# XingqunQi-lab/EmotionGestures

Hardware: AMD Instinct MI355X
Metric: gesture clips/sec (34 frames, 43 joints) (higher is better)
Workload: dtype bf16x3; 1 GPU; TED clips: 4 s 16 kHz audio -> mel(128x124) -> CVAE sample -> generator -> 34x126 pose; global_batch=64, variant=Models_spatial_memory, parallelism=clip-sharded x1, no data-path collective, launch=hipGraph replay, 4 step(s) in flight, branch_streams=False, fold_affine=False

## Files before the change

emotiongestures_amd/_lib.py:

```python
from __future__ import annotations

import ctypes as C
import os

_HERE = os.path.dirname(os.path.abspath(__file__))
LIB_PATH = os.path.join(_HERE, "libemogest_hip.so")

EG_PREC_F32, EG_PREC_BF16X3, EG_PREC_BF16 = 0, 1, 2
PRECISIONS = {"f32": EG_PREC_F32, "fp32": EG_PREC_F32, "bf16x3": EG_PREC_BF16X3, "bf16": EG_PREC_BF16}

(PACK_RAW, PACK_LINEAR, PACK_VEC_PAD, PACK_CONV3X3, PACK_BN_SCALE, PACK_BN_SHIFT, PACK_CONV1X1, PACK_STEM,
 PACK_WN_TAP, PACK_CONV1D, PACK_POS_TABLE, PACK_LINEAR_T, PACK_LINEAR_FOLD, PACK_BIAS_FOLD, PACK_CONV1X1_BF16, PACK_WN_TAPS) = range(16)


class EgError(RuntimeError):
    pass


class EgWeightEntry(C.Structure):
    _fields_ = [("key", C.c_char * 192), ("kind", C.c_int32), ("dims", C.c_int32 * 4),
                ("offset", C.c_int64), ("numel", C.c_int64)]


class EgGeneratorConfig(C.Structure):
    _fields_ = [(n, C.c_int32) for n in (
        "frames", "pose_dim", "prior_frames", "chunk", "d_model", "d_inner", "n_layers", "n_head", "d_k",
        "n_mels", "spec_len", "text_len", "n_words", "embed_dim", "tcn_hidden", "tcn_layers", "variant",
        "precision", "n_position")] + [("reserved", C.c_int32 * 5)]


class EgCvaeConfig(C.Structure):
    _fields_ = [("frames", C.c_int32), ("d_model", C.c_int32), ("latent", C.c_int32), ("n_classes", C.c_int32),
                ("reserved", C.c_int32 * 4)]


_P = C.c_void_p
_I = C.c_int32
_L = C.c_int64


class EgLinearArgs(C.Structure):
    _fields_ = [(n, _P) for n in ("x", "w", "bias", "res1", "res2", "y", "gate_src", "drop_epoch", "partial", "x_images", "y_images")] + \
               [("drop_offset", C.c_uint64)] + \
               [(n, _I) for n in ("lda", "ldw", "ldr", "ldc", "ldg", "m", "n", "k", "relu", "precision", "splits", "k_x", "y_k")] + \
               [("drop_seed", C.c_uint32), ("drop_p", C.c_float)]


class EgResamplePlan(C.Structure):
    _fields_ = [(n, C.c_int32) for n in ("L", "M", "half", "K", "D", "Hs", "pitch", "bank_floats")]


EG_RESAMPLE_TILE, EG_RESAMPLE_MAX_FACTOR = 1024, 640
EG_SKELETON_MAX_BONES, EG_SKELETON_MAX_FACTOR, EG_SKELETON_TILE_FRAMES = 63, 64, 32
EG_SKELETON_SPACE_LOCAL, EG_SKELETON_SPACE_GLOBAL = 0, 1

SIGNATURES = {
    "eg_last_error": (C.c_char_p, []),
    "eg_launch_count": (_L, []),
    "eg_launch_histogram": (_L, [C.c_char_p, _L, C.c_int32]),
    "eg_version": (C.c_char_p, []),
    "eg_set_default_precision": (C.c_int, [C.c_int]),
    "eg_get_default_precision": (C.c_int, []),
    "eg_generator_default_config": (C.c_int, [C.POINTER(EgGeneratorConfig)]),
    "eg_generator_create": (C.c_int, [C.POINTER(EgGeneratorConfig), C.POINTER(_P)]),
    "eg_generator_destroy": (None, [_P]),
    "eg_generator_arena_floats": (_L, [_P]),
    "eg_generator_num_weights": (_I, [_P]),
    "eg_generator_weight_entry": (C.c_int, [_P, _I, C.POINTER(EgWeightEntry)]),
    "eg_generator_workspace_bytes": (_L, [_P, _I]),
    "eg_generator_forward": (C.c_int, [_P, _P, _I, _P, _P, _P, _P, _P, _P, _P, _P, _P, _P, _L, _P]),
    "eg_generator_forward_draws": (C.c_int, [_P, _P, _I, _I, _P, _P, _P, _P, _P, _L, _P]),
    "eg_generator_draws_workspace_bytes": (_L, [_P, _I, _I]),
    "eg_generator_forward_rollout": (C.c_int, [_P, _P, _I, _I, _P, _P, _P, _P, _P, _P, _P, _P, _P, _P, _P, _P, _L, _P]),
    "eg_generator_rollout_workspace_bytes": (_L, [_P, _I, _I]),
    "eg_generator_forward_rollout_draws": (C.c_int, [_P, _P, _I, _I, _I, _P, _P, _P, _P, _P, _P, _P, _P, _P, _P, _P, _P, _L, _P]),
    "eg_generator_rollout_draws_workspace_bytes": (_L, [_P, _I, _I, _I]),
    "eg_rows_by_table": (C.c_int, [_P, _P, _P, _I, _L, _I, _P]),
    "eg_rollout_ragged_plan_ints": (_L, [_I, _L]),
    "eg_rollout_ragged_plan": (C.c_int, [_P, _I, _P, _P, _P, _P]),
    "eg_generator_forward_rollout_ragged": (C.c_int, [_P, _P, _I, _P, _P, _P, _P, _P, _P, _P, _P, _P, _P, _P, _P, _P, _P, _L, _P]),
    "eg_generator_rollout_ragged_workspace_bytes": (_L, [_P, _I, _L]),
    "eg_stream_state_bytes": (_L, [_P, _I, _I, _I]),
    "eg_stream_reset": (C.c_int, [_P, _P, _I, _I, _I, _P, _P, _P]),
    "eg_stream_push": (C.c_int, [_P, _P, _I, _I, _I, _P, _P, _P, _P]),
    "eg_generator_stream_step": (C.c_int, [_P, _P, _P, _I, _I, _I, _P, _P, _P, _P, _P, _P, _P, _P, _P, _L, _P]),
    "eg_stream_tail": (C.c_int, [_P, _P, _I, _I, _I, _P, _P]),
    "eg_generator_tap": (C.c_int, [_P, _I, _P, C.c_char_p, C.POINTER(_P), C.POINTER(_L)]),
    "eg_cvae_default_config": (C.c_int, [C.POINTER(EgCvaeConfig)]),
    "eg_cvae_create": (C.c_int, [C.POINTER(EgCvaeConfig), C.POINTER(_P)]),
    "eg_cvae_destroy": (None, [_P]),
    "eg_cvae_arena_floats": (_L, [_P]),
    "eg_cvae_num_weights": (_I, [_P]),
    "eg_cvae_weight_entry": (C.c_int, [_P, _I, C.POINTER(EgWeightEntry)]),
    "eg_cvae_workspace_bytes": (_L, [_P, _I]),
    "eg_cvae_sample": (C.c_int, [_P, _P, _I, _P, _P, _P, _P, _L, _P]),
    "eg_cvae_forward": (C.c_int, [_P, _P, _I, _P, _P, _P, _P, _P, _P, _P, _L, _P]),
    "eg_mel_tables": (C.c_int, [_P, _P, _P, _P]),
    "eg_mel_workspace_bytes": (_L, [_I, _I]),
    "eg_melspectrogram": (C.c_int, [_P, _I, _I, _P, _P, _P, _P, _P, _I, _P, _L, _P]),
    "eg_window_gather": (C.c_int, [_P, _I, _L, _I, _L, _I, _P, _P]),
    "eg_window_gather_ragged": (C.c_int, [_P, _I, _L, _P, _P, _L, _I, _P, _P]),
    "eg_resample_plan": (C.c_int, [_I, _I, C.POINTER(EgResamplePlan)]),
    "eg_resample_out_length": (_L, [_L, _I, _I]),
    "eg_resample_filter": (C.c_int, [_I, _I, _P, _P]),
    "eg_resample": (C.c_int, [_P, _I, _L, _P, _P, _I, _I, _P, _L, _P, _L, _P]),
    "eg_resample_stream_state_bytes": (_L, [_I, _I, _I]),
    "eg_resample_stream_reset": (C.c_int, [_P, _I, _I, _I, _P, _P]),
    "eg_resample_stream_push": (C.c_int, [_P, _I, _I, _I, _P, _P, _I, _P, _P, _I, _P]),
    "eg_skeleton_check": (C.c_int, [_P, _P, _P, _I]),
    "eg_skeleton_out_frames": (_L, [_L, _I, _I]),
    "eg_skeleton_tile_frames": (_I, []),
    "eg_skeleton_joints": (C.c_int, [_P, _I, _I, _P, _P, _P, _I, _P, _P, _I, _I, _P, _I, _I, _I, _P, _L, _P]),
    "eg_skeleton_dir_vec": (C.c_int, [_P, _I, _I, _P, _P, _P, _I, _P, _P, _I, _I, _P, _P, _P]),
    "eg_skeleton_rest_check": (C.c_int, [_P, _I]),
    "eg_skeleton_levels": (C.c_int, [_P, _P, _P, _I, _P, _P]),
    "eg_skeleton_rotations": (C.c_int, [_P, _I, _I, _P, _P, _P, _I, _P, _P, _P, _I, _I, _P, _I, _I, _I, _P, _L, _P]),
    "eg_beat_tables": (C.c_int, [_P, _P, _P, _P]),
    "eg_beat_workspace_bytes": (_L, [_I, _I]),
    "eg_beat_align": (C.c_int, [_P, _I, _I, _P, _I, _I, _I, _I, _I, C.c_double, _I, _P, _P, _P, _P, _P, _L, _P, _P, _P, _P, _P, _P, _P]),
    "eg_beat_tracks_meta_ints": (_L, [_I]),
    "eg_beat_tracks_meta": (C.c_int, [_P, _P, _P, _I, _I, _P]),
    "eg_beat_tracks_workspace_bytes": (_L, [_P, _P, _I, _I, _I]),
    "eg_beat_align_tracks": (C.c_int, [_P, _I, _L, _P, _P, _P, _I, _I, _I, _P, _I, _I, _P, C.c_double, _I, _P, _P, _P, _P, _P, _L, _P, _P, _P,
                                       _P, _P, _P, _P]),
    "eg_beat_tracks_scan": (C.c_int, [_P, _P, _I, _P, _P, _L, _P, _P, _P]),
    "eg_take_meta_ints": (_L, [_I]),
    "eg_take_meta": (C.c_int, [_P, _I, _P]),
    "eg_track_rows_pack": (C.c_int, [_P, _I, _I, _I, _I, _P, _P, _P, _P]),
    "eg_take_distance_workspace_bytes": (_L, [_P, _I, _I]),
    "eg_take_distance": (C.c_int, [_P, _I, _I, _I, _P, _P, _I, _P, _L, _P, _P, _P]),
    "eg_conv3x3": (C.c_int, [_P, _P, _P, _P, _P, _P, _P, _I, _I, _I, _I, _I, _I, _I, _I, _I, _P]),
    "eg_conv3x3_se": (C.c_int, [_P, _P, _P, _P, _P, _P, _P, _P, _P, _I, _I, _I, _I, _I, _I, _I, _I, _I, _P]),
    "eg_se_gate_pre": (C.c_int, [_P, _P, _I, _P, _P, _P, _P, _P, _P, _P, _P, _I, _I, _I, _I, _P]),
    "eg_se_block_fused": (C.c_int, [_P] * 19 + [_I] * 7 + [_P]),
    "eg_conv3x3_gap_tiles": (_I, [_I, _I, _I, _I, _I]),
    "eg_conv3x3_channel_split": (_I, [_I, _I, _I, _I, _I, _I, _I]),
    "eg_stem_conv": (C.c_int, [_P, _P, _P, _P, _P, _P, _I, _I, _I, _I, _P]),
    "eg_se_gate": (C.c_int, [_P, _I, _P, _P, _P, _P, _P, _I, _I, _I, _P]),
    "eg_se_residual_relu": (C.c_int, [_P, _P, _P, _P, _P, _P, _P, _I, _I, _I, _I, _I, _I, _I, _I, _P]),
    "eg_linear": (C.c_int, [_P, _I, _P, _I, _P, _P, _P, _I, _P, _I, _I, _I, _I, _I, _I, _I, _I, _P]),
    "eg_split_tiles": (C.c_int, [_P, _I, _I, _I, _P, _P]),
    "eg_linear_presplit": (C.c_int, [_P, _I, _P, _I, _P, _P, _P, _I, _P, _I, _I, _I, _I, _I, _I, _P]),
    "eg_linear_presplit_causal": (C.c_int, [_P, _I, _P, _P, _I, _P, _P, _I, _P, _I, _P, _I, _I, _I, _I, _I, _I, _I, _I, _P]),
    "eg_linear_splitk": (C.c_int, [_P, _I, _P, _I, _P, _P, _I, _I, _I, _I, _I, _I, _P, _I, _P]),
    "eg_layernorm": (C.c_int, [_P, _P, _P, _P, _I, _I, C.c_float, _P]),
    "eg_attention": (C.c_int, [_P, _I, _P, _I, _P, _I, _P, _I, _P, _I, _I, _I, _I, _I, _I, _P]),
    "eg_attention_masked": (C.c_int, [_P, _I, _P, _I, _P, _I, _P, _L, _I, _P, _I, _P, _I, _I, _I, _I, _I, _I, _P]),
    "eg_mha_workspace_bytes": (_L, [_I, _I, _I, _I, _I]),
    "eg_multi_head_attention": (C.c_int, [_P, _P, _P, _P, _P, _P, _P, _P, _P, _P, _I, _I, _I, _I, _I, _I, _P, _L, _P]),
    "eg_ffn_workspace_bytes": (_L, [_I, _I, _I]),
    "eg_positionwise_ffn": (C.c_int, [_P, _P, _P, _P, _P, _P, _P, _P, _I, _I, _I, _I, _P, _L, _P]),
    "eg_tcn_forward": (C.c_int, [_P, _P, _P, _I, _I, _I, _I, _I, _P, _L, _P]),
    "eg_add_rows": (C.c_int, [_P, _P, _P, _L, _I, _I, _P]),
    "eg_add_rows_split": (C.c_int, [_P, _P, _P, _P, _L, _I, _I, _P]),
    "eg_conv3x3_packed_floats": (_L, [_I, _I]),
    "eg_profile_enable": (C.c_int, [_I]),
    "eg_profile_disable": (C.c_int, []),
    "eg_profile_read": (_I, [_P, _P, _P, _I]),
    "eg_profile_read_workgroups": (_I, [_P, _I]),
    "eg_reparameterize": (C.c_int, [_P, _P, _P, _P, _L, _P]),
    "eg_conv1d": (C.c_int, [_P, _P, _P, _P, _P, _P, _I, _I, _I, _I, _I, _I, _I, _I, _P]),
    "eg_contrastive_workspace_bytes": (C.c_int64, [_I]),
    "eg_contrastive_loss": (C.c_int, [_P, _P, _I, _I, _P, _P, _P, _P, _L, _P]),
    "eg_contrastive_backward_workspace_bytes": (_L, [_I]),
    "eg_contrastive_loss_backward": (C.c_int, [_P, _P, _I, _I, _P, _P, _P, _L, _P]),
    "eg_transpose": (C.c_int, [_P, _I, _I, _I, _P, _I, _P]),
    "eg_gemm_tn_workspace_floats": (_L, [_I, _I, _L]),
    "eg_gemm_tn": (C.c_int, [_P, _I, _P, _I, _P, _I, _I, _I, _L, _P, _L, _I, _P]),
    "eg_conv3x3_wgrad": (C.c_int, [_P, _P, _P, _I, _I, _I, _I, _I, _I, _P, _L, _P]),
    "eg_im2col3x3": (C.c_int, [_P, _P, _I, _I, _I, _I, _I, _I, _P]),
    "eg_subsample": (C.c_int, [_P, _P, _I, _I, _I, _I, _I, _I, _P]),
    "eg_conv1d_cl_forward": (C.c_int, [_P, _P, _P, _P] + [_I] * 9 + [_P]),
    "eg_conv1d_cl_backward_input": (C.c_int, [_P, _P, _P, _P] + [_I] * 9 + [_P]),
    "eg_conv1d_cl_backward_weight_workspace_floats": (_L, [_I] * 7),
    "eg_conv1d_cl_backward_weight": (C.c_int, [_P, _P, _P, _P, _P] + [_I] * 9 + [_P, _L, _P]),
    "eg_pad_cols": (C.c_int, [_P, _P, _L, _I, _I, _P]),
    "eg_colreduce_workspace_floats": (_L, [_I]),
    "eg_bn_train_forward": (C.c_int, [_P, _P, _P, _P, _P, _P, _P, _P, _L, _I, C.c_float, C.c_float, _P, _P]),
    "eg_bn_train_backward": (C.c_int, [_P, _P, _P, _P, _P, _P, _P, _P, _L, _I, _I, _P, _P]),
    "eg_bn_train_forward_gap": (C.c_int, [_P, _P, _I, _I, _P, _P, _P, _P, _P, _P, _P, _P, _L, _I, C.c_float, C.c_float, _P, _P]),
    "eg_bn_train_forward_sq": (C.c_int, [_P, _P, _P, _I, _I, _P, _P, _P, _P, _P, _P, _P, _P, _L, _I, C.c_float, C.c_float, _P, _P]),
    "eg_conv3x3_sq": (C.c_int, [_P, _P, _P, _P, _P, _P] + [_I] * 8 + [_P]),
    "eg_se_gate_train_forward": (C.c_int, [_P] * 12 + [_I, _I, _I, _P]),
    "eg_se_tail_forward": (C.c_int, [_P] * 9 + [_I, _I, _I, _P]),
    "eg_se_tail_backward_reduce": (C.c_int, [_P] * 7 + [_I, _I, _I, _P, _P]),
    "eg_se_gate_train_backward": (C.c_int, [_P] * 16 + [_I, _I, _I, _P]),
    "eg_se_tail_backward_finish": (C.c_int, [_P] * 14 + [_I, _I, _I, _P]),
    "eg_se_tail_backward_apply": (C.c_int, [_P] * 13 + [_I, _I, _I, _P]),
    "eg_colsum": (C.c_int, [_P, _P, _P, _P, _L, _I, _P, _P]),
    "eg_elementwise": (C.c_int, [_P, _P, _P, _L, _I, C.c_float, _P]),
    "eg_conv3x3_wgrad_mfma_workspace_floats": (_L, [_I, _I, _I, _I, _I]),
    "eg_conv3x3_wgrad_mfma": (C.c_int, [_P, _P, _P, _I, _I, _I, _I, _I, _P, _L, _P]),
    "eg_conv3x3_wgrad_mfma_oihw": (C.c_int, [_P, _P, _P, _I, _I, _I, _I, _I, _P, _L, _P]),
    "eg_conv3x3_wgrad_gather_mfma": (C.c_int, [_P, _P, _P, _I, _I, _I, _I, _I, _I, _P, _L, _P]),
    "eg_conv3x3_dgrad_s2": (C.c_int, [_P, _P, _P, _P, _I, _I, _I, _I, _I, _I, _P]),
    "eg_conv3x3_res_masked": (C.c_int, [_P, _P, _P, _P, _P, _I, _I, _I, _I, _I, _I, _P]),
    "eg_conv3x3_wgrad_mfma_oihw_in_affine": (C.c_int, [_P, _P, _P, _P, _P, _I, _I, _I, _I, _I, _P, _L, _P]),
    "eg_conv3x3_sq_in_affine": (C.c_int, [_P, _P, _P, _P, _P, _P, _P, _P, _I, _I, _I, _I, _I, _I, _I, _I, _P]),
    "eg_bn_train_stats_sq": (C.c_int, [_P, _P, _I, _I, _P, _P, _P, _P, _P, _P, _P, _P, _L, _I, C.c_float, C.c_float, _P, _P]),
    "eg_pack_conv3x3_device": (C.c_int, [_P, _I, _I, _I, _P, _P]),
    "eg_linear_packed_floats": (_L, [_I, _I]),
    "eg_pack_linear_device": (C.c_int, [_P, _I, _I, _I, _I, _P, _P]),
    "eg_pack_table_blocks": (_I, [_I, _I, _I, _I]),
    "eg_pack_table": (C.c_int, [_P, _I, _I, _P]),
    "eg_dropout": (C.c_int, [_P, _P, _L, C.c_float, C.c_uint32, C.c_uint64, _P]),
    "eg_dropout_dev": (C.c_int, [_P, _P, _L, C.c_float, C.c_uint32, C.c_uint64, _P, _P]),
    "eg_seg_mean": (C.c_int, [_P, _P, _I, _I, _I, C.c_float, _P, _P]),
    "eg_seg_dot": (C.c_int, [_P, _P, _P, _I, _I, _I, _P, _P]),
    "eg_se_scale": (C.c_int, [_P, _P, _P, _P, _I, _I, _I, _P]),
    "eg_layernorm_backward": (C.c_int, [_P, _P, _P, _P, _P, _I, _I, C.c_float, _P]),
    "eg_attention_train": (C.c_int, [_P, _I, _P, _I, _P, _I, _P, _I, _P, _I, _I, _I, _I, _I, C.c_float, C.c_uint32, C.c_uint64, _P, _P]),
    "eg_attention_backward_train": (C.c_int, [_P, _I, _P, _I, _P, _I, _P, _P, _I, _P, _I, _P, _I, _P, _I, _I, _I, _I, _I, _I, C.c_float, C.c_uint32,
                                              C.c_uint64, _P, _P]),
    "eg_smooth_l1": (C.c_int, [_P, _P, _P, _P, _L, C.c_float, C.c_float, _P, _P]),
    "eg_cross_entropy": (C.c_int, [_P, _P, _P, C.c_float, C.c_float, _P, _P, _I, _I, _P, _P]),
    "eg_kld": (C.c_int, [_P, _P, _P, _P, _P, _I, _I, C.c_float, _P]),
    "eg_adam_step": (C.c_int, [_P, _P, _P, _P, _L, C.c_float, C.c_float, C.c_float, C.c_float, C.c_float, _I, _P]),
    "eg_adam_step_dev": (C.c_int, [_P, _P, _P, _P, _L, C.c_float, C.c_float, C.c_float, C.c_float, C.c_float, _P, _P]),
    "eg_counter_add": (C.c_int, [_P, _I, _P]),
    "eg_sp_gate_forward": (C.c_int, [_P, _P, _P, _P, _I, _I, _I, _I, _P]),
    "eg_sp_gate_backward": (C.c_int, [_P, _P, _P, _P, _P, _P, _I, _I, _I, _I, _P]),
    "eg_tm_scale_forward": (C.c_int, [_P, _P, _P, _P, _I, _I, _I, _I, _P]),
    "eg_tm_scale_backward": (C.c_int, [_P, _P, _P, _P, _P, _I, _I, _I, _I, _P]),
    "eg_linear_wgrad_mfma_workspace_floats": (_L, [_I, _I, _I]),
    "eg_linear_wgrad_mfma": (C.c_int, [_P, _I, _P, _I, _P, _I, _P, _I, _I, _I, _P, _L, _P]),
# ... 44 lines not shown
```

emotiongestures_amd/csrc/common.h:

```cpp
#pragma once
#include <hip/hip_runtime.h>
#include <stdint.h>
#include <stdio.h>
#include <stdarg.h>
#include <atomic>
#include "emogest.h"


typedef float f4 __attribute__((ext_vector_type(4)));
typedef short bf8 __attribute__((ext_vector_type(8)));

#define EG_WAVE 64

void eg_set_error(const char* fmt, ...);

#define EG_REQUIRE(cond, code, ...)                      \
    do {                                                 \
        if (!(cond)) {                                   \
            eg_set_error(__VA_ARGS__);                   \
            return (code);                               \
        }                                                \
    } while (0)

extern std::atomic<long long> g_eg_launches;
// ... 41 lines not shown
}
__device__ __forceinline__ float row16_sum(float s) {
    s += dpp_move<0xB1>(s);
    s += dpp_move<0x4E>(s);
    s += dpp_move<0x141>(s);
    s += dpp_move<0x140>(s);
    return s;
}
__device__ __forceinline__ float wave_max(float v) {
#pragma unroll
    for (int o = 32; o > 0; o >>= 1) v = fmaxf(v, __shfl_xor(v, o, 64));
    return v;
}

__device__ __forceinline__ unsigned short f32_to_bf16_rne(float x) {
    unsigned int u = __float_as_uint(x);
    u += 0x7FFFu + ((u >> 16) & 1u);
    return (unsigned short)(u >> 16);
}
__device__ __forceinline__ float bf16_to_f32(unsigned short h) { return __uint_as_float(((unsigned int)h) << 16); }

typedef __bf16 bf16x2_t __attribute__((ext_vector_type(2)));
typedef float f32x2_t __attribute__((ext_vector_type(2)));
typedef unsigned int u32x4_t __attribute__((ext_vector_type(4)));
template <bool WANT_LO>
__device__ __forceinline__ void split_octet(const f4& v0, const f4& v1, bf8& hi, bf8& lo) {
    u32x4_t h, l;
#pragma unroll
    for (int p = 0; p < 4; ++p) {
        const f32x2_t x = {p < 2 ? v0[2 * p] : v1[2 * p - 4], p < 2 ? v0[2 * p + 1] : v1[2 * p - 3]};
        const unsigned hu = __builtin_bit_cast(unsigned, __builtin_convertvector(x, bf16x2_t));
        h[p] = hu;
        if (WANT_LO) {
            const f32x2_t r = {x[0] - __uint_as_float(hu << 16), x[1] - __uint_as_float(hu & 0xffff0000u)};
            l[p] = __builtin_bit_cast(unsigned, __builtin_convertvector(r, bf16x2_t));
        }
    }
    hi = __builtin_bit_cast(bf8, h);
    if (WANT_LO) lo = __builtin_bit_cast(bf8, l);
}

__device__ __forceinline__ unsigned int mix32(unsigned int h) {
    h ^= h >> 16; h *= 0x85EBCA6Bu; h ^= h >> 13; h *= 0xC2B2AE35u; h ^= h >> 16;
    return h;
}
__device__ __forceinline__ unsigned int dropout_seed(unsigned int seed, const int* __restrict__ epoch) {
    return epoch ? seed ^ mix32((unsigned int)*epoch * 0x9E3779B9u + 0x7F4A7C15u) : seed;
}
__device__ __forceinline__ bool dropout_keep(unsigned int seed, unsigned long long ctr, unsigned int thr) {
    return mix32(mix32((unsigned int)ctr ^ seed) + (unsigned int)(ctr >> 32) * 0x9E3779B9u + 0x6A09E667u) >= thr;
}
struct EgDropout {
    unsigned int thr = 0, seed = 0;
    float inv_keep = 1.f;
    unsigned long long offset = 0;
    const int* epoch = nullptr;
};

__device__ __forceinline__ void xcd_tile(int& bx, int& by) {
    const int gx = gridDim.x, gy = gridDim.y, total = gx * gy;
    const int lin = blockIdx.y * gx + blockIdx.x;
    const int xcd = lin & 7, idx = lin >> 3;
    const int q = total >> 3, r = total & 7;
    const int log = xcd * q + (xcd < r ? xcd : r) + idx;
    bx = log / gy;
    by = log - bx * gy;
}

template <int N> __device__ __forceinline__ void wait_vmcnt_imm() {
    __builtin_amdgcn_s_waitcnt((N & 15) | 0x70 | 0xF00 | ((N >> 4) << 14));
}
__device__ __forceinline__ void wait_lgkmcnt0() { __builtin_amdgcn_s_waitcnt(0xC07F); }
__device__ __forceinline__ void wg_barrier() {
    asm volatile("" ::: "memory");
    __builtin_amdgcn_s_barrier();
    asm volatile("" ::: "memory");
}

struct EgProfScope {
    int slot;
    hipStream_t st;
    EgProfScope(int64_t tag, double flops, hipStream_t s);
    void workgroups(int n);
    ~EgProfScope();
};

struct EgiCvaeFused {
    const float *y = nullptr, *z = nullptr;
    const float *lin_w[4] = {}, *lin_b[4] = {};
    const float *t_w[2] = {}, *t_b[2] = {}, *t_s[2] = {}, *t_t[2] = {};
    const float *c_w[3] = {}, *c_b[3] = {}, *c_s[2] = {}, *c_t[2] = {};
    float* out = nullptr;
    int F = 0, L = 0, T = 0;
};

struct EgiLinear {
    const float* x = nullptr; int lda = 0;
    const void* ximg = nullptr; int xK = 0, xk0 = 0;
    const float* w = nullptr; int ldw = 0; const float* bias = nullptr;
    const float* res1 = nullptr; const float* res2 = nullptr; int ldr = 0;
    float* y = nullptr; int ldc = 0;
    void* yimg = nullptr; int yK = 0, yk0 = 0;
    int m = 0, n = 0, k = 0, relu = 0, a_shift = 0, a_seq = 1, precision = 0;
    int shared_chip = 0;
    int xs_shift = 0, xs_period = 1; const void* xzero = nullptr;
    int splits = 0; float* partial = nullptr;
};
```

emotiongestures_amd/csrc/gemm.hip:

```cpp
#include "common.h"
#include <stdlib.h>
#include <string.h>

namespace {

struct GemmArgs {
    const float* x; const float* w; const float* bias; const float* res1; const float* res2; float* y;
    const unsigned short* whi; const unsigned short* wlo;
    int lda, ldw, ldr, ldc, M, N, K, relu, a_shift, a_seq, k_per_split;
    float* partial;
    unsigned short* yimg = nullptr;
    int yKO = 0, yoct0 = 0;
    int xoct0 = 0;
    int xs_steps = 0, xs_shift = 0, xs_period = 1;
    const bf8* xzero = nullptr;
    const float* gate = nullptr; int ldg = 0;
    EgDropout drop;
};

__device__ __forceinline__ float epi_masks(const GemmArgs& a, float v, int m, int n, unsigned int dseed) {
    if (a.gate && !(a.gate[(size_t)m * a.ldg + n] > 0.f)) v = 0.f;
    if (a.drop.thr) v = dropout_keep(dseed, a.drop.offset + (unsigned long long)m * a.N + n, a.drop.thr) ? v * a.drop.inv_keep : 0.f;
    return v;
}
// ... 316 lines not shown
        const int k0 = kbeg + step * 32;
        f4* X = lds + slot * SLOT;
#pragma unroll
        for (int p = 0; p < 2; ++p) {
            const int k = min(k0 + xq[p], klast);
            __builtin_amdgcn_global_load_lds((const __attribute__((address_space(1))) void*)(xsrc[p] + k),
                                             (__attribute__((address_space(3))) void*)(X + (p * 4 + wave) * 64), 16, 0, 0);
        }
        bf8* W = reinterpret_cast<bf8*>(X + XS);
#pragma unroll
        for (int t = 0; t < TN; ++t) {
            const size_t gbase = ((size_t)min(by * TN + t, nt_last) * KO + (k0 >> 3)) * 64 + wave * 64 + lane;
            __builtin_amdgcn_global_load_lds((const __attribute__((address_space(1))) void*)(reinterpret_cast<const bf8*>(a.whi) + gbase),
                                             (__attribute__((address_space(3))) void*)(W + t * NIMG * WIMG + wave * 64), 16, 0, 0);
            if (TERMS == 3)
                __builtin_amdgcn_global_load_lds((const __attribute__((address_space(1))) void*)(reinterpret_cast<const bf8*>(a.wlo) + gbase),
                                                 (__attribute__((address_space(3))) void*)(W + t * NIMG * WIMG + WIMG + wave * 64), 16, 0, 0);
        }
    };
    auto wait_groups = [&](int groups_in_flight) {
        if (groups_in_flight >= 2) wait_vmcnt_imm<2 * G>();
        else if (groups_in_flight == 1) wait_vmcnt_imm<G>();
        else wait_vmcnt_imm<0>();
    };

    f4 acc[2][WN];
#pragma unroll
    for (int t = 0; t < 2; ++t)
#pragma unroll
        for (int n = 0; n < WN; ++n) acc[t][n] = (f4){0.f, 0.f, 0.f, 0.f};

    const int pre = min(nsteps, RING - 1);
    for (int s = 0; s < pre; ++s) issue(s, s);
    wait_groups(pre - 1);
    wg_barrier();
    const int fsw = (li ^ (li >> 1)) & 7;
#pragma unroll 1
    for (int s = 0; s < nsteps; ++s) {
        if (s + RING - 1 < nsteps) issue(s + RING - 1, (s + RING - 1) % RING);
        const f4* X = lds + (s % RING) * SLOT;
        const bf8* W = reinterpret_cast<const bf8*>(X + XS);
        bf8 xh[2], xl[2], wh[WN], wl[WN];
#pragma unroll
        for (int t = 0; t < 2; ++t) {
            const f4* xr = X + (wm + t * 16 + li) * 8;
            const f4 q0 = xr[(2 * kq) ^ fsw], q1 = xr[(2 * kq + 1) ^ fsw];
            split_octet<TERMS == 3>(q0, q1, xh[t], xl[t]);
        }
#pragma unroll
        for (int n = 0; n < WN; ++n) {
            const int col = wn + n * 16, tile = col >> 6, r = (col & 63) + li;
            wh[n] = W[tile * NIMG * WIMG + kq * 64 + r];
            if (TERMS == 3) wl[n] = W[tile * NIMG * WIMG + WIMG + kq * 64 + r];
        }
#pragma unroll
        for (int t = 0; t < 2; ++t)
#pragma unroll
            for (int n = 0; n < WN; ++n) {
                if (TERMS == 3) {
                    acc[t][n] = __builtin_amdgcn_mfma_f32_16x16x32_bf16(wl[n], xh[t], acc[t][n], 0, 0, 0);
                    acc[t][n] = __builtin_amdgcn_mfma_f32_16x16x32_bf16(wh[n], xl[t], acc[t][n], 0, 0, 0);
                }
                acc[t][n] = __builtin_amdgcn_mfma_f32_16x16x32_bf16(wh[n], xh[t], acc[t][n], 0, 0, 0);
            }
        const int newest = min(s + RING - 1, nsteps - 1);
        wait_groups(max(0, newest - (s + 1)));
        __builtin_amdgcn_s_waitcnt(0xC07F);
        wg_barrier();
    }
    gemm_epilogue<2, WN, true>(a, acc, m0 + wm + li, n0 + wn + kq * 4);
}

template <int TERMS, int WN>
int launch_glds(const GemmArgs& a, int splits, hipStream_t st) {
    constexpr int NIMG = (TERMS == 3) ? 2 : 1, TN = WN / 2, RING = (WN == 2) ? 4 : 3;
    constexpr size_t LDS_BYTES = (size_t)RING * (64 * 8 + TN * NIMG * 4 * 64) * 16;
    auto kern = gemm_glds_kernel<TERMS, WN>;
    if (int rc = eg_ensure_dynamic_lds(reinterpret_cast<const void*>(kern), LDS_BYTES, "gemm_glds")) return rc;
    dim3 grid(eg_cdiv(a.M, 64), eg_cdiv(a.N, 64 * TN), splits);
    hipLaunchKernelGGL(kern, grid, dim3(256), LDS_BYTES, st, a);
    return eg_check_launch("gemm_glds");
}


template <int TERMS, bool TRAIN = false, bool SHIFT = false>
__global__ __launch_bounds__(256, 2) void gemm_presplit_kernel(GemmArgs a, const bf8* __restrict__ xhi, const bf8* __restrict__ xlo, int xKO) {
    constexpr int BK = 32;
    constexpr int RING = 4;
    constexpr int WM = 2;
    constexpr int NIMG = (TERMS == 3) ? 2 : 1;
    constexpr int IMG = 256;
    constexpr int XO = NIMG * IMG, SLOT = XO + NIMG * IMG;
    constexpr int G = 2 * NIMG;
    extern __shared__ __attribute__((aligned(16))) bf8 lds[];
    const int tid = threadIdx.x, lane = tid & 63, li = lane & 15, kq = lane >> 4;
    const int wave = __builtin_amdgcn_readfirstlane(tid >> 6);
    int bx, by;
    xcd_tile(bx, by);
    const int m0 = bx * 64, n0 = by * 64;
    const int wm = (wave >> 1) * 32, wn = (wave & 1) * 32;
    const int kbeg = blockIdx.z * a.k_per_split;
    const int kend = min(a.K, kbeg + a.k_per_split);
    const int nsteps = (kend - kbeg + BK - 1) / BK;
    const int KO = a.ldw >> 3;
    const bf8 *sxh = nullptr, *sxl = nullptr;
    if constexpr (SHIFT) {
        const int m = bx * 64 + lane, ms = m - a.xs_shift;
        const bool ok = (m % a.xs_period) >= a.xs_shift;
        const size_t gs = ((size_t)(ms >> 6) * xKO + a.xoct0 + wave) * 64 + (ms & 63);
        sxh = ok ? xhi + gs : a.xzero + wave * 64 + lane;
        sxl = ok ? xlo + gs : a.xzero + wave * 64 + lane;
    }
    auto issue = [&](int step, int slot) {
        const int ko = (kbeg + step * BK) >> 3;
        bf8* S = lds + slot * SLOT;
        const int d = wave * 64;
        const int xo = (SHIFT && step >= a.xs_steps) ? ko - a.xs_steps * 4 : ko;
        const size_t gx = ((size_t)bx * xKO + a.xoct0 + xo + wave) * 64 + lane;
        const bf8* ph = xhi + gx;
        const bf8* pl = xlo + gx;
        if (SHIFT && step < a.xs_steps) { ph = sxh + (size_t)step * 256; pl = sxl + (size_t)step * 256; }
        __builtin_amdgcn_global_load_lds((const __attribute__((address_space(1))) void*)ph, (__attribute__((address_space(3))) void*)(S + d), 16, 0, 0);
        if (TERMS == 3)
            __builtin_amdgcn_global_load_lds((const __attribute__((address_space(1))) void*)pl, (__attribute__((address_space(3))) void*)(S + IMG + d), 16, 0, 0);
        const size_t gw = ((size_t)by * KO + ko + wave) * 64 + lane;
        __builtin_amdgcn_global_load_lds((const __attribute__((address_space(1))) void*)(reinterpret_cast<const bf8*>(a.whi) + gw),
                                         (__attribute__((address_space(3))) void*)(S + XO + d), 16, 0, 0);
        if (TERMS == 3)
            __builtin_amdgcn_global_load_lds((const __attribute__((address_space(1))) void*)(reinterpret_cast<const bf8*>(a.wlo) + gw),
                                             (__attribute__((address_space(3))) void*)(S + XO + IMG + d), 16, 0, 0);
    };
    static_assert(RING == 4, "a step group must land within two steps: at most one younger group stays in flight across a barrier");
    auto wait_groups = [&](int n) {
        if (n == 0) wait_vmcnt_imm<0>(); else wait_vmcnt_imm<G>();
    };
    struct Frags { bf8 xh[WM], xl[WM], wh[2], wl[2]; };
    auto read_frags = [&](Frags& f, int slot) {
        const bf8* S = lds + slot * SLOT + li;
        const int o = kq * 64;
#pragma unroll
        for (int t = 0; t < WM; ++t) {
            f.xh[t] = S[o + wm + t * 16];
            if (TERMS == 3) f.xl[t] = S[IMG + o + wm + t * 16];
        }
#pragma unroll
        for (int n = 0; n < 2; ++n) {
            f.wh[n] = S[XO + o + wn + n * 16];
            if (TERMS == 3) f.wl[n] = S[XO + IMG + o + wn + n * 16];
        }
    };
    f4 acc[WM][2];
#pragma unroll
    for (int t = 0; t < WM; ++t)
#pragma unroll
        for (int n = 0; n < 2; ++n) acc[t][n] = (f4){0.f, 0.f, 0.f, 0.f};
    auto mfma_step = [&](const Frags& f) {
#pragma unroll
        for (int t = 0; t < WM; ++t)
#pragma unroll
            for (int n = 0; n < 2; ++n) {
                if (TERMS == 3) {
                    acc[t][n] = __builtin_amdgcn_mfma_f32_16x16x32_bf16(f.wl[n], f.xh[t], acc[t][n], 0, 0, 0);
                    acc[t][n] = __builtin_amdgcn_mfma_f32_16x16x32_bf16(f.wh[n], f.xl[t], acc[t][n], 0, 0, 0);
                }
                acc[t][n] = __builtin_amdgcn_mfma_f32_16x16x32_bf16(f.wh[n], f.xh[t], acc[t][n], 0, 0, 0);
            }
    };

    const int pre = min(nsteps, RING - 1);
    for (int s = 0; s < pre; ++s) issue(s, s);
    wait_groups(max(0, pre - 2));
    wg_barrier();
    Frags fa, fb;
    read_frags(fa, 0);
    __builtin_amdgcn_s_waitcnt(0xC07F);
    auto step = [&](int s, Frags& cur, Frags& nxt) {
        if (s + RING - 1 < nsteps) issue(s + RING - 1, (s + RING - 1) % RING);
        if (s + 1 < nsteps) read_frags(nxt, (s + 1) % RING);
        mfma_step(cur);
        const int newest = min(s + RING - 1, nsteps - 1);
        wait_groups(max(0, min(RING - 3, newest - (s + 2))));
        __builtin_amdgcn_s_waitcnt(0xC07F);
        wg_barrier();
    };
    int s0 = 0;
    if constexpr (!SHIFT) {
        constexpr int AHEAD = (RING - 1) * 4;
        const size_t xoff = (size_t)(a.xoct0 + (kbeg >> 3) + AHEAD + wave) * 64 + lane;
        const bf8* px = xhi + (size_t)bx * xKO * 64 + xoff;
        const bf8* pxl = xlo + (size_t)bx * xKO * 64 + xoff;
        const bf8* pw = reinterpret_cast<const bf8*>(a.whi) + ((size_t)by * KO + (kbeg >> 3) + AHEAD + wave) * 64 + lane;
        const bf8* pwl = reinterpret_cast<const bf8*>(a.wlo) + ((size_t)by * KO + (kbeg >> 3) + AHEAD + wave) * 64 + lane;
        auto fast = [&](const int j, Frags& cur, Frags& nxt) {
            bf8* S = lds + ((j + RING - 1) % RING) * SLOT + wave * 64;
            __builtin_amdgcn_global_load_lds((const __attribute__((address_space(1))) void*)px, (__attribute__((address_space(3))) void*)S, 16, 0, 0);
            if (TERMS == 3)
                __builtin_amdgcn_global_load_lds((const __attribute__((address_space(1))) void*)pxl, (__attribute__((address_space(3))) void*)(S + IMG), 16, 0, 0);
            __builtin_amdgcn_global_load_lds((const __attribute__((address_space(1))) void*)pw, (__attribute__((address_space(3))) void*)(S + XO), 16, 0, 0);
            if (TERMS == 3)
                __builtin_amdgcn_global_load_lds((const __attribute__((address_space(1))) void*)pwl, (__attribute__((address_space(3))) void*)(S + XO + IMG), 16, 0, 0);
            px += 256; pxl += 256; pw += 256; pwl += 256;
            read_frags(nxt, (j + 1) % RING);
            mfma_step(cur);
            wait_vmcnt_imm<(RING - 3) * G>();
            wait_lgkmcnt0();
            wg_barrier();
        };
#pragma unroll 1
        for (; s0 + 2 * RING - 1 <= nsteps; s0 += RING) {
#pragma unroll
            for (int j = 0; j < RING; j += 2) {
                fast(j, fa, fb);
                fast(j + 1, fb, fa);
            }
        }
    }
#pragma unroll 1
    for (int s = s0; s < nsteps; s += 2) {
        step(s, fa, fb);
        if (s + 1 < nsteps) step(s + 1, fb, fa);
    }
    gemm_epilogue<WM, 2, TRAIN>(a, acc, m0 + wm + li, n0 + wn + kq * 4);
}

template <int TERMS, bool TRAIN = false, bool SHIFT = false>
int launch_presplit(const GemmArgs& a, const bf8* xhi, const bf8* xlo, int xko, dim3 grid, hipStream_t st) {
    constexpr int NIMG = (TERMS == 3) ? 2 : 1;
    constexpr size_t LDS_BYTES = (size_t)4 * 2 * NIMG * 4 * 64 * 16;
    auto kern = gemm_presplit_kernel<TERMS, TRAIN, SHIFT>;
    if (int rc = eg_ensure_dynamic_lds(reinterpret_cast<const void*>(kern), LDS_BYTES, "gemm_presplit")) return rc;
    hipLaunchKernelGGL(kern, grid, dim3(256), LDS_BYTES, st, a, xhi, xlo, xko);
    return eg_check_launch("gemm_presplit");
}

template <int TERMS, bool TRAIN = false, bool SHIFT = false>
__global__ __launch_bounds__(512, 1) void gemm_presplit128_kernel(GemmArgs a, const bf8* __restrict__ xhi, const bf8* __restrict__ xlo, int xKO,
                                                                  int m_tiles, int n_tiles) {
    constexpr int RING = 3;
    constexpr int NIMG = (TERMS == 3) ? 2 : 1;
    constexpr int OPI = 8 * 64;
    constexpr int OP = NIMG * OPI, SLOT = 2 * OP;
    constexpr int G = 2 * NIMG;
    extern __shared__ __attribute__((aligned(16))) bf8 lds[];
    const int tid = threadIdx.x, lane = tid & 63, li = lane & 15, kq = lane >> 4;
    const int wave = __builtin_amdgcn_readfirstlane(tid >> 6);
    int bx, by;
    xcd_tile(bx, by);
    const int m0 = bx * 128, n0 = by * 128;
    const int wm = wave >> 2, wn = wave & 3;
    const int nsteps = (a.K + 31) / 32;
    const int KO = a.ldw >> 3;
    const int pt = wave >> 2, po = wave & 3;
    const int xtile = min(bx * 2 + pt, m_tiles - 1);
    const size_t gx = ((size_t)xtile * xKO + a.xoct0 + po) * 64 + lane;
    const bf8 *sxh = nullptr, *sxl = nullptr;
    if constexpr (SHIFT) {
        const int m = xtile * 64 + lane, ms = m - a.xs_shift;
        const bool ok = (m % a.xs_period) >= a.xs_shift;
        const size_t gs = ((size_t)(ms >> 6) * xKO + a.xoct0 + po) * 64 + (ms & 63);
        sxh = ok ? xhi + gs : a.xzero + po * 64 + lane;
        sxl = ok ? xlo + gs : a.xzero + po * 64 + lane;
    }
    const size_t gw = ((size_t)min(by * 2 + pt, n_tiles - 1) * KO + po) * 64 + lane;
    const bf8* whi = reinterpret_cast<const bf8*>(a.whi);
    const bf8* wlo = reinterpret_cast<const bf8*>(a.wlo);
    auto issue = [&](int step, int slot) {
        bf8* S = lds + slot * SLOT + wave * 64;
        const size_t o = (size_t)step * 4 * 64;
        const bf8* ph = xhi + gx + o;
        const bf8* pl = xlo + gx + o;
        if constexpr (SHIFT) {
            if (step < a.xs_steps) { ph = sxh + o; pl = sxl + o; }
            else { ph -= (size_t)a.xs_steps * 256; pl -= (size_t)a.xs_steps * 256; }
        }
        __builtin_amdgcn_global_load_lds((const __attribute__((address_space(1))) void*)ph, (__attribute__((address_space(3))) void*)S, 16, 0, 0);
        if (TERMS == 3)
            __builtin_amdgcn_global_load_lds((const __attribute__((address_space(1))) void*)pl, (__attribute__((address_space(3))) void*)(S + OPI), 16, 0, 0);
        __builtin_amdgcn_global_load_lds((const __attribute__((address_space(1))) void*)(whi + gw + o), (__attribute__((address_space(3))) void*)(S + OP), 16, 0, 0);
        if (TERMS == 3)
            __builtin_amdgcn_global_load_lds((const __attribute__((address_space(1))) void*)(wlo + gw + o), (__attribute__((address_space(3))) void*)(S + OP + OPI), 16, 0, 0);
    };
    struct Frags { bf8 xh[4], xl[4], wh[2], wl[2]; };
    auto read_frags = [&](Frags& f, int slot) {
        const bf8* X = lds + slot * SLOT + (wm * 4 + kq) * 64 + li;
        const bf8* W = lds + slot * SLOT + OP + ((wn >> 1) * 4 + kq) * 64 + (wn & 1) * 32 + li;
#pragma unroll
        for (int t = 0; t < 4; ++t) {
            f.xh[t] = X[t * 16];
            if (TERMS == 3) f.xl[t] = X[OPI + t * 16];
        }
#pragma unroll
        for (int n = 0; n < 2; ++n) {
            f.wh[n] = W[n * 16];
            if (TERMS == 3) f.wl[n] = W[OPI + n * 16];
        }
    };
    f4 acc[4][2];
#pragma unroll
    for (int t = 0; t < 4; ++t)
#pragma unroll
        for (int n = 0; n < 2; ++n) acc[t][n] = (f4){0.f, 0.f, 0.f, 0.f};
    auto mfma_half = [&](const Frags& f, int half) {
#pragma unroll
        for (int t = half * 2; t < half * 2 + 2; ++t)
#pragma unroll
            for (int n = 0; n < 2; ++n) {
                if (TERMS == 3) {
                    acc[t][n] = __builtin_amdgcn_mfma_f32_16x16x32_bf16(f.wl[n], f.xh[t], acc[t][n], 0, 0, 0);
                    acc[t][n] = __builtin_amdgcn_mfma_f32_16x16x32_bf16(f.wh[n], f.xl[t], acc[t][n], 0, 0, 0);
                }
                acc[t][n] = __builtin_amdgcn_mfma_f32_16x16x32_bf16(f.wh[n], f.xh[t], acc[t][n], 0, 0, 0);
            }
    };
    auto wait_younger = [&](int n) {
        if (n <= 0) wait_vmcnt_imm<0>();
        else if (n == 1) wait_vmcnt_imm<G>();
        else wait_vmcnt_imm<2 * G>();
    };
    const int pre = min(nsteps, RING - 1);
    for (int s = 0; s < pre; ++s) issue(s, s);
    wait_younger(pre - 1);
    wg_barrier();
    Frags fa, fb;
    read_frags(fa, 0);
    auto step = [&](int s, Frags& cur, Frags& nxt) {
        if (s + RING - 1 < nsteps) issue(s + RING - 1, (s + RING - 1) % RING);
        mfma_half(cur, 0);
        __builtin_amdgcn_sched_barrier(0);
        wait_younger(min(s + RING - 1, nsteps - 1) - (s + 1));
        wait_lgkmcnt0();
        wg_barrier();
        if (s + 1 < nsteps) read_frags(nxt, (s + 1) % RING);
        mfma_half(cur, 1);
    };
#pragma unroll 1
    for (int s = 0; s < nsteps; s += 2) {
        step(s, fa, fb);
        if (s + 1 < nsteps) step(s + 1, fb, fa);
    }
    gemm_epilogue<4, 2, TRAIN>(a, acc, m0 + wm * 64 + li, n0 + wn * 32 + kq * 4);
}

template <int TERMS, bool TRAIN = false, bool SHIFT = false>
int launch_presplit128(const GemmArgs& a, const bf8* xhi, const bf8* xlo, int xko, int m_tiles, int n_tiles, hipStream_t st) {
    constexpr int NIMG = (TERMS == 3) ? 2 : 1;
    constexpr size_t LDS_BYTES = (size_t)3 * 2 * NIMG * 8 * 64 * 16;
    static_assert(LDS_BYTES <= 160 * 1024, "LDS");
    auto kern = gemm_presplit128_kernel<TERMS, TRAIN, SHIFT>;
    if (int rc = eg_ensure_dynamic_lds(reinterpret_cast<const void*>(kern), LDS_BYTES, "gemm_presplit128")) return rc;
    dim3 grid(eg_cdiv(m_tiles, 2), eg_cdiv(n_tiles, 2), 1);
    hipLaunchKernelGGL(kern, grid, dim3(512), LDS_BYTES, st, a, xhi, xlo, xko, m_tiles, n_tiles);
    return eg_check_launch("gemm_presplit128");
}

enum PresplitTile { TILE_64 = 0, TILE_128 = 1, TILE_AUTO = -1, TILE_BAD = -2 };
int presplit_tile_override() {
    const char* e = getenv("EG_GEMM_TILE");
    if (!e || !e[0]) return TILE_AUTO;
    if (!strcmp(e, "64")) return TILE_64;
    if (!strcmp(e, "128")) return TILE_128;
    return TILE_BAD;
}
int presplit_tile_default(int m, int n, int shared_chip) {
    const long wgs = (long)eg_cdiv(m, 128) * eg_cdiv(n, 128);
    if (wgs >= (shared_chip ? 64 : 1024)) return TILE_128;
    return TILE_64;
}
int dispatch_presplit(const GemmArgs& a, const bf8* xhi, const bf8* xlo, int xko, int precision, hipStream_t st, EgProfScope* prof = nullptr, int shared_chip = 0) {
    const int mt = eg_cdiv(a.M, 64), nt = eg_cdiv(a.N, 64);
    int tile = presplit_tile_override();
    if (tile == TILE_BAD) {
        eg_set_error("EG_GEMM_TILE=\"%s\": accepted values are \"64\" and \"128\" (unset or empty: automatic); the retired tile variants are in tools/experiments/README.md",
                     getenv("EG_GEMM_TILE"));
        return EG_ERR_BAD_ARG;
    }
    if (tile == TILE_AUTO) tile = presplit_tile_default(a.M, a.N, shared_chip);
    if (prof) prof->workgroups(tile == TILE_128 ? eg_cdiv(mt, 2) * eg_cdiv(nt, 2) : mt * nt);
    const bool x3 = precision == EG_PREC_BF16X3;
    dim3 grid(mt, nt, 1);
    if (a.xs_steps) {
        if (a.gate || a.drop.thr) { eg_set_error("shifted pre-split product: no training epilogue"); return EG_ERR_UNSUPPORTED; }
        if (tile == TILE_128)
            return x3 ? launch_presplit128<3, false, true>(a, xhi, xlo, xko, mt, nt, st) : launch_presplit128<1, false, true>(a, xhi, xlo, xko, mt, nt, st);
        return x3 ? launch_presplit<3, false, true>(a, xhi, xlo, xko, grid, st) : launch_presplit<1, false, true>(a, xhi, xlo, xko, grid, st);
    }
    if (a.gate || a.drop.thr) {
        if (!x3) { eg_set_error("pre-split product with a training epilogue: bf16x3 only"); return EG_ERR_UNSUPPORTED; }
        if (tile == TILE_128) return launch_presplit128<3, true>(a, xhi, xlo, xko, mt, nt, st);
        return launch_presplit<3, true>(a, xhi, xlo, xko, grid, st);
    }
    if (tile == TILE_128) return x3 ? launch_presplit128<3>(a, xhi, xlo, xko, mt, nt, st) : launch_presplit128<1>(a, xhi, xlo, xko, mt, nt, st);
    return x3 ? launch_presplit<3>(a, xhi, xlo, xko, grid, st) : launch_presplit<1>(a, xhi, xlo, xko, grid, st);
}

template <int RT, bool XF32, bool TRAIN>
__global__ __launch_bounds__(256) void gemm_skinny_kernel(GemmArgs a, const bf8* __restrict__ xhi, const bf8* __restrict__ xlo, int xKO) {
    constexpr int B = 4;
    __shared__ f4 red[4][RT][64];
    const int tid = threadIdx.x, lane = tid & 63, li = lane & 15, kq = lane >> 4;
    const int wave = __builtin_amdgcn_readfirstlane(tid >> 6);
    const int n0 = blockIdx.x * 16, m0 = blockIdx.y * 64, KO = a.ldw >> 3;
    const int nsteps = (a.K + 31) >> 5;
    const bf8* __restrict__ wh = reinterpret_cast<const bf8*>(a.whi) + ((size_t)(n0 >> 6) * KO) * 64 + (n0 & 63) + li;
    const bf8* __restrict__ wl = reinterpret_cast<const bf8*>(a.wlo) + ((size_t)(n0 >> 6) * KO) * 64 + (n0 & 63) + li;
    const size_t xtile = (size_t)blockIdx.y * xKO * 64;
    struct Frag { bf8 wh, wl, xh[RT], xl[RT]; };
    auto load = [&](Frag& f, int step) {
        const int ko = step * 4 + kq;
        f.wh = wh[(size_t)ko * 64];
        f.wl = wl[(size_t)ko * 64];
#pragma unroll
        for (int t = 0; t < RT; ++t) {
            if constexpr (XF32) {
                const int m = m0 + t * 16 + li, k = ko * 8;
                split_octet<true>(load_x_quad(a, m, k, a.K), load_x_quad(a, m, k + 4, a.K), f.xh[t], f.xl[t]);
            } else {
                const size_t gx = xtile + (size_t)(a.xoct0 + ko) * 64 + t * 16 + li;
                f.xh[t] = xhi[gx];
                f.xl[t] = xlo[gx];
            }
        }
    };
    f4 acc[RT];
#pragma unroll
    for (int t = 0; t < RT; ++t) acc[t] = (f4){0.f, 0.f, 0.f, 0.f};
    auto mfma = [&](const Frag& f) {
#pragma unroll
        for (int t = 0; t < RT; ++t) {
            acc[t] = __builtin_amdgcn_mfma_f32_16x16x32_bf16(f.wl, f.xh[t], acc[t], 0, 0, 0);
            acc[t] = __builtin_amdgcn_mfma_f32_16x16x32_bf16(f.wh, f.xl[t], acc[t], 0, 0, 0);
            acc[t] = __builtin_amdgcn_mfma_f32_16x16x32_bf16(f.wh, f.xh[t], acc[t], 0, 0, 0);
        }
    };
    const int mine = (nsteps - wave + 3) >> 2;
    Frag fa[B], fb[B];
    auto load_batch = [&](Frag (&f)[B], int first) {
#pragma unroll
        for (int j = 0; j < B; ++j)
            if (first + j < mine) load(f[j], wave + 4 * (first + j));
    };
    auto mfma_batch = [&](const Frag (&f)[B], int first) {
#pragma unroll
        for (int j = 0; j < B; ++j)
            if (first + j < mine) mfma(f[j]);
    };
    load_batch(fa, 0);
#pragma unroll 1
    for (int s = 0; s < mine; s += 2 * B) {
        if (s + B < mine) load_batch(fb, s + B);
        mfma_batch(fa, s);
        if (s + 2 * B < mine) load_batch(fa, s + 2 * B);
        mfma_batch(fb, s + B);
    }
#pragma unroll
    for (int t = 0; t < RT; ++t) red[wave][t][lane] = acc[t];
    __syncthreads();
    if (wave < RT) {
        f4 v[1][1];
        v[0][0] = (red[0][wave][lane] + red[1][wave][lane]) + (red[2][wave][lane] + red[3][wave][lane]);
        gemm_epilogue<1, 1, TRAIN>(a, v, m0 + wave * 16 + li, n0 + kq * 4);
    }
}
template <bool XF32, bool TRAIN>
int launch_skinny_t(const GemmArgs& a, const bf8* xhi, const bf8* xlo, int xko, hipStream_t st) {
    const dim3 grid(eg_cdiv(a.N, 16), eg_cdiv(a.M, 64)), block(256);
    switch (a.M > 64 ? 4 : eg_cdiv(a.M, 16)) {
        case 1: hipLaunchKernelGGL((gemm_skinny_kernel<1, XF32, TRAIN>), grid, block, 0, st, a, xhi, xlo, xko); break;
        case 2: hipLaunchKernelGGL((gemm_skinny_kernel<2, XF32, TRAIN>), grid, block, 0, st, a, xhi, xlo, xko); break;
        case 3: hipLaunchKernelGGL((gemm_skinny_kernel<3, XF32, TRAIN>), grid, block, 0, st, a, xhi, xlo, xko); break;
        default: hipLaunchKernelGGL((gemm_skinny_kernel<4, XF32, TRAIN>), grid, block, 0, st, a, xhi, xlo, xko); break;
    }
    return eg_check_launch("gemm (few rows)");
}
template <bool XF32>
int launch_skinny(const GemmArgs& a, const bf8* xhi, const bf8* xlo, int xko, hipStream_t st) {
// ... 2 lines not shown
}
constexpr int SKINNY_ROWS = 64;
bool skinny_ok(const GemmArgs& a, int precision) {
    if (precision != EG_PREC_BF16X3 || a.partial) return false;
    int limit = SKINNY_ROWS;
    if (const char* e = getenv("EG_GEMM_SKINNY")) { if (e[0] == '0') limit = 0; }
    return a.M <= limit;
}

__global__ __launch_bounds__(256) void split_tile_kernel(const float* __restrict__ x, int lda, int M, int K, int KO,
                                                         bf8* __restrict__ hi, bf8* __restrict__ lo) {
    const size_t total = (size_t)gridDim.y * 64 * KO;
    const int mt = blockIdx.y;
    for (int i = blockIdx.x * 256 + threadIdx.x; i < 64 * KO; i += gridDim.x * 256) {
        const int o = i >> 6, r = i & 63, m = mt * 64 + r, k = o * 8;
        f4 v0 = (f4){0.f, 0.f, 0.f, 0.f}, v1 = v0;
        if (m < M) {
            if (k < K) v0 = *reinterpret_cast<const f4*>(x + (size_t)m * lda + k);
            if (k + 4 < K) v1 = *reinterpret_cast<const f4*>(x + (size_t)m * lda + k + 4);
        }
        bf8 h, l;
        split_octet<true>(v0, v1, h, l);
        hi[((size_t)mt * KO + o) * 64 + r] = h;
        lo[((size_t)mt * KO + o) * 64 + r] = l;
    }
    (void)total;
}

__global__ __launch_bounds__(256) void splitk_reduce_kernel(GemmArgs a, int splits) {
    const int i = blockIdx.x * 256 + threadIdx.x;
    if (i >= a.M * a.N) return;
    const int m = i / a.N, n = i - m * a.N;
    float s = a.bias ? a.bias[n] : 0.f;
    for (int z = 0; z < splits; ++z) s += a.partial[(size_t)z * a.M * a.N + i];
    if (a.gate || a.drop.thr) s = epi_masks(a, s, m, n, a.drop.thr ? dropout_seed(a.drop.seed, a.drop.epoch) : 0u);
    if (a.res1) s += a.res1[(size_t)m * a.ldr + n];
    if (a.relu) s = fmaxf(s, 0.f);
    if (a.res2) s = fmaxf(s + a.res2[(size_t)m * a.ldr + n], 0.f);
    a.y[(size_t)m * a.ldc + n] = s;
}

int launch_gemm(GemmArgs& a, int splits, int precision, hipStream_t st) {
    dim3 grid(eg_cdiv(a.M, 64), eg_cdiv(a.N, 64), splits), block(256);
    if (precision == EG_PREC_F32) hipLaunchKernelGGL((gemm_kernel<EG_PREC_F32>), grid, block, 0, st, a);
    else if (a.a_shift) {
        if (precision == EG_PREC_BF16X3) hipLaunchKernelGGL((gemm_bf16_kernel<3>), grid, block, 0, st, a);
        else hipLaunchKernelGGL((gemm_bf16_kernel<1>), grid, block, 0, st, a);
    } else {
        bool wide = (long)eg_cdiv(a.M, 64) * eg_cdiv(a.N, 128) * splits >= 256;
        if (const char* e = getenv("EG_GLDS_TILE")) wide = e[0] == '1';
        if (precision == EG_PREC_BF16X3) return wide ? launch_glds<3, 4>(a, splits, st) : launch_glds<3, 2>(a, splits, st);
        return wide ? launch_glds<1, 4>(a, splits, st) : launch_glds<1, 2>(a, splits, st);
    }
    return eg_check_launch("gemm");
}

int launch_splitk(GemmArgs& a, int splits, int precision, hipStream_t st) {
    a.k_per_split = (int)eg_round_up(eg_cdiv(a.K, splits), 64);
    const int nsplit = eg_cdiv(a.K, a.k_per_split);
    if (int rc = launch_gemm(a, nsplit, precision, st)) return rc;
    hipLaunchKernelGGL(splitk_reduce_kernel, dim3(eg_cdiv(a.M * a.N, 256)), dim3(256), 0, st, a, nsplit);
    return eg_check_launch("splitk_reduce");
}

int fill_common(GemmArgs& a, const float* x, int lda, const float* w, int ldw, int m, int n, int k, int precision,
                const char* who) {
    EG_REQUIRE(x && w && m > 0 && n > 0 && k > 0, EG_ERR_BAD_ARG, "%s: null pointer or empty shape", who);
    EG_REQUIRE(eg_aligned16(x) && eg_aligned16(w), EG_ERR_ALIGN, "%s: X and W must be 16-byte aligned", who);
    EG_REQUIRE((k & 3) == 0 && (lda & 3) == 0 && (ldw & 3) == 0, EG_ERR_ALIGN, "%s: K, lda, ldw must be multiples of 4 (K=%d lda=%d ldw=%d)", who, k, lda, ldw);
    EG_REQUIRE(precision >= 0 && precision <= 2, EG_ERR_BAD_ARG, "%s: precision %d", who, precision);
    a.x = x; a.w = w; a.lda = lda; a.ldw = ldw; a.M = m; a.N = n; a.K = k;
    a.whi = a.wlo = nullptr;
    if (precision != EG_PREC_F32) {
        EG_REQUIRE((ldw & 63) == 0, EG_ERR_ALIGN, "%s: split-bf16 modes need ldw %% 64 == 0 (EG_PACK_LINEAR weights)", who);
        const size_t rows = (size_t)eg_round_up(n, 64);
        a.whi = reinterpret_cast<const unsigned short*>(w + rows * ldw);
        a.wlo = a.whi + rows * ldw;
    }
    return EG_OK;
}

}

int egi_linear(const EgiLinear& p, hipStream_t st) {
    GemmArgs a;
    EG_REQUIRE((p.x || p.ximg) && p.w && (p.y || p.yimg) && p.m > 0 && p.n > 0 && p.k > 0, EG_ERR_BAD_ARG, "egi_linear: null pointer or empty shape");
    EG_REQUIRE((p.k & 3) == 0 && (p.ldw & 3) == 0, EG_ERR_ALIGN, "egi_linear: K, ldw %% 4");
    a.x = p.x; a.w = p.w; a.lda = p.lda; a.ldw = p.ldw; a.M = p.m; a.N = p.n; a.K = p.k;
    a.whi = a.wlo = nullptr;
    if (p.precision != EG_PREC_F32) {
        EG_REQUIRE((p.ldw & 63) == 0, EG_ERR_ALIGN, "egi_linear: packed weights need ldw %% 64 == 0");
        const size_t rows = (size_t)eg_round_up(p.n, 64);
        a.whi = reinterpret_cast<const unsigned short*>(p.w + rows * p.ldw);
        a.wlo = a.whi + rows * p.ldw;
    }
    a.bias = p.bias; a.res1 = p.res1; a.res2 = p.res2; a.ldr = p.ldr; a.y = p.y; a.ldc = p.ldc; a.relu = p.relu;
    a.a_shift = p.a_shift; a.a_seq = p.a_seq > 0 ? p.a_seq : 1; a.k_per_split = (int)eg_round_up(p.k, 64); a.partial = nullptr;
    if (p.yimg) {
        EG_REQUIRE((p.n & 3) == 0 && (p.yK & 63) == 0 && (p.yk0 & 7) == 0, EG_ERR_ALIGN, "egi_linear: image output alignment");
        a.yimg = reinterpret_cast<unsigned short*>(p.yimg); a.yKO = p.yK >> 3; a.yoct0 = p.yk0 >> 3;
    }
    EgProfScope prof(p.precision == EG_PREC_F32 ? 5 : ((p.ximg) ? 3 : (p.a_shift ? 4 : 2)), 2.0 * p.m * (double)p.n * p.k, st);
    if (p.ximg && p.precision != EG_PREC_F32) {
        EG_REQUIRE((p.xK & 63) == 0 && (p.xk0 & 31) == 0 && (p.k & 31) == 0, EG_ERR_ALIGN, "egi_linear: pre-split X needs K %% 32 == 0");
        const int xko = p.xK >> 3, mt = eg_cdiv(p.m, 64);
        const bf8* xhi = reinterpret_cast<const bf8*>(p.ximg);
        const bf8* xlo = xhi + (size_t)mt * xko * 64;
        a.xoct0 = p.xk0 >> 3;
        if (p.xs_shift > 0) {
            EG_REQUIRE((p.k & 63) == 0 && p.xs_period > 0 && p.xzero && p.splits <= 1, EG_ERR_BAD_ARG, "egi_linear: shifted product needs k %% 64 == 0, a period and a zero line");
            a.xs_steps = p.k >> 6; a.xs_shift = p.xs_shift; a.xs_period = p.xs_period; a.xzero = reinterpret_cast<const bf8*>(p.xzero);
            return dispatch_presplit(a, xhi, xlo, xko, p.precision, st, &prof, p.shared_chip);
        }
        if (skinny_ok(a, p.precision)) {
            prof.workgroups(eg_cdiv(a.N, 16) * eg_cdiv(a.M, 64));
            return launch_skinny<false>(a, xhi, xlo, xko, st);
        }
        if (p.splits > 1) {
            EG_REQUIRE(p.partial && !p.yimg && p.y, EG_ERR_BAD_ARG, "egi_linear: split-K needs a partial buffer and an fp32 output (no image output)");
            a.partial = p.partial;
            a.k_per_split = (int)eg_round_up(eg_cdiv(a.K, p.splits), 64);
            const int nsplit = eg_cdiv(a.K, a.k_per_split);
            prof.workgroups(mt * eg_cdiv(a.N, 64) * nsplit);
            dim3 grid(mt, eg_cdiv(a.N, 64), nsplit);
            const int rc = (p.precision == EG_PREC_BF16X3) ? launch_presplit<3>(a, xhi, xlo, xko, grid, st) : launch_presplit<1>(a, xhi, xlo, xko, grid, st);
            if (rc) return rc;
            hipLaunchKernelGGL(splitk_reduce_kernel, dim3(eg_cdiv(a.M * a.N, 256)), dim3(256), 0, st, a, nsplit);
            return eg_check_launch("splitk_reduce");
        }
        return dispatch_presplit(a, xhi, xlo, xko, p.precision, st, &prof, p.shared_chip);
    }
    EG_REQUIRE(p.x && (p.lda & 3) == 0, EG_ERR_BAD_ARG, "egi_linear: fp32 input missing");
    if (skinny_ok(a, p.precision)) {
        prof.workgroups(eg_cdiv(a.N, 16) * eg_cdiv(a.M, 64));
        return launch_skinny<true>(a, nullptr, nullptr, 0, st);
    }
    prof.workgroups(eg_cdiv(p.m, 64) * eg_cdiv(p.n, 64));
    return launch_gemm(a, 1, p.precision, st);
}
int egi_split_tiles(const float* x, int lda, int m, int k, void* images, hipStream_t st) { return eg_split_tiles(x, lda, m, k, images, st); }

extern "C" int eg_linear(const float* x, int32_t lda, const float* w, int32_t ldw, const float* bias,
                         const float* res1, const float* res2, int32_t ldr, float* y, int32_t ldc,
                         int32_t m, int32_t n, int32_t k, int32_t relu, int32_t a_shift, int32_t a_seq,
                         int32_t precision, void* stream) {
    GemmArgs a;
    int rc = fill_common(a, x, lda, w, ldw, m, n, k, precision, "eg_linear");
    if (rc) return rc;
    EG_REQUIRE(y, EG_ERR_BAD_ARG, "eg_linear: null output");
    EG_REQUIRE(a_shift == 0 || a_seq > 0, EG_ERR_BAD_ARG, "eg_linear: a_seq must be positive when a_shift is set");
    a.bias = bias; a.res1 = res1; a.res2 = res2; a.ldr = ldr; a.y = y; a.ldc = ldc; a.relu = relu;
    a.a_shift = a_shift; a.a_seq = a_seq > 0 ? a_seq : 1; a.k_per_split = (int)eg_round_up(k, 64); a.partial = nullptr;
    EgProfScope prof(precision == EG_PREC_F32 ? 5 : (a_shift ? 4 : 2), 2.0 * m * (double)n * k, (hipStream_t)stream);
    if (skinny_ok(a, precision)) return launch_skinny<true>(a, nullptr, nullptr, 0, (hipStream_t)stream);
    return launch_gemm(a, 1, precision, (hipStream_t)stream);
}

extern "C" int eg_linear_splitk(const float* x, int32_t lda, const float* w, int32_t ldw, const float* bias, float* y,
                                int32_t ldc, int32_t m, int32_t n, int32_t k, int32_t relu, int32_t splits,
                                float* partial, int32_t precision, void* stream) {
    GemmArgs a;
    int rc = fill_common(a, x, lda, w, ldw, m, n, k, precision, "eg_linear_splitk");
    if (rc) return rc;
    EG_REQUIRE(y && partial && splits > 0, EG_ERR_BAD_ARG, "eg_linear_splitk: null output/partial");
    a.bias = bias; a.res1 = a.res2 = nullptr; a.ldr = 0; a.y = y; a.ldc = ldc; a.relu = relu;
    a.a_shift = 0; a.a_seq = 1; a.partial = partial;
    return launch_splitk(a, splits, precision, (hipStream_t)stream);
}

extern "C" int eg_linear_ex(const EgLinearArgs* p, void* stream) {
    EG_REQUIRE(p, EG_ERR_BAD_ARG, "eg_linear_ex: null argument block");
    GemmArgs a;
    int rc = fill_common(a, p->x_images ? reinterpret_cast<const float*>(p->x_images) : p->x, p->x_images ? 4 : p->lda, p->w, p->ldw, p->m, p->n, p->k, p->precision,
                         "eg_linear_ex");
    if (rc) return rc;
    if (p->x_images) a.x = nullptr;
    EG_REQUIRE(p->y, EG_ERR_BAD_ARG, "eg_linear_ex: null output");
    EG_REQUIRE(p->drop_p >= 0.f && p->drop_p < 1.f, EG_ERR_BAD_ARG, "eg_linear_ex: drop_p=%f", (double)p->drop_p);
    a.bias = p->bias; a.res1 = p->res1; a.res2 = p->res2; a.ldr = p->ldr; a.y = p->y; a.ldc = p->ldc; a.relu = p->relu;
    a.a_shift = 0; a.a_seq = 1; a.k_per_split = (int)eg_round_up(p->k, 64); a.partial = nullptr;
    a.gate = p->gate_src; a.ldg = p->ldg;
    if (p->drop_p > 0.f) {
        a.drop.thr = (unsigned int)((double)p->drop_p * 4294967296.0);
        a.drop.inv_keep = 1.0f / (1.0f - p->drop_p);
        a.drop.seed = p->drop_seed; a.drop.offset = p->drop_offset; a.drop.epoch = p->drop_epoch;
    }
    if (p->y_images) {
        EG_REQUIRE(p->precision != EG_PREC_F32 && (p->n & 3) == 0 && (p->y_k & 63) == 0 && p->y_k >= p->n && p->splits < 2, EG_ERR_BAD_ARG,
                   "eg_linear_ex: image output needs a bf16 mode, n %% 4 == 0, y_k %% 64 == 0 and no split-K");
        a.yimg = reinterpret_cast<unsigned short*>(p->y_images); a.yKO = p->y_k >> 3; a.yoct0 = 0;
    }
    if (p->splits >= 2) {
        EG_REQUIRE(p->partial && !p->x_images, EG_ERR_BAD_ARG, "eg_linear_ex: split-K needs a partial buffer of splits*M*N floats (and fp32 X)");
        a.partial = p->partial;
        return launch_splitk(a, p->splits, p->precision, (hipStream_t)stream);
    }
    if (p->x_images) {
        EG_REQUIRE(p->precision != EG_PREC_F32 && (p->k_x & 63) == 0 && (p->k & 31) == 0 && p->k <= p->k_x, EG_ERR_BAD_ARG,
                   "eg_linear_ex: pre-split X needs a bf16 mode, k %% 32 == 0 and images of width k_x %% 64 == 0 >= k");
        const int xko = p->k_x >> 3, mt = eg_cdiv(p->m, 64);
        const bf8* xhi = reinterpret_cast<const bf8*>(p->x_images);
        const bf8* xlo = xhi + (size_t)mt * xko * 64;
        a.xoct0 = 0;
        EgProfScope prof(3, 2.0 * p->m * (double)p->n * p->k, (hipStream_t)stream);
        if (skinny_ok(a, p->precision)) return launch_skinny<false>(a, xhi, xlo, xko, (hipStream_t)stream);
        return dispatch_presplit(a, xhi, xlo, xko, p->precision, (hipStream_t)stream, &prof, 0);
    }
    EgProfScope prof(p->precision == EG_PREC_F32 ? 5 : 2, 2.0 * p->m * (double)p->n * p->k, (hipStream_t)stream);
    if (skinny_ok(a, p->precision)) return launch_skinny<true>(a, nullptr, nullptr, 0, (hipStream_t)stream);
    return launch_gemm(a, 1, p->precision, (hipStream_t)stream);
}

extern "C" int eg_split_tiles(const float* x, int32_t lda, int32_t m, int32_t k, void* images, void* stream) {
    EG_REQUIRE(x && images && m > 0 && k > 0 && (k & 3) == 0 && (lda & 3) == 0, EG_ERR_BAD_ARG, "eg_split_tiles: bad argument");
    const int kpad = (int)eg_round_up(k, 64), ko = kpad / 8, mt = eg_cdiv(m, 64);
    bf8* hi = reinterpret_cast<bf8*>(images);
    bf8* lo = hi + (size_t)mt * ko * 64;
    hipLaunchKernelGGL(split_tile_kernel, dim3(eg_cdiv(64 * ko, 256), mt), dim3(256), 0, (hipStream_t)stream, x, lda, m, k, ko, hi, lo);
    return eg_check_launch("split_tiles");
}

extern "C" int eg_linear_presplit(const void* x_images, int32_t k_x, const float* w, int32_t ldw, const float* bias,
                                  const float* res1, const float* res2, int32_t ldr, float* y, int32_t ldc,
                                  int32_t m, int32_t n, int32_t k, int32_t relu, int32_t precision, void* stream) {
    GemmArgs a;
    EG_REQUIRE(x_images && w && y && m > 0 && n > 0 && k > 0, EG_ERR_BAD_ARG, "eg_linear_presplit: null pointer or empty shape");
    EG_REQUIRE(precision == EG_PREC_BF16X3 || precision == EG_PREC_BF16, EG_ERR_BAD_ARG, "eg_linear_presplit: bf16 modes only");
    EG_REQUIRE((ldw & 63) == 0, EG_ERR_ALIGN, "eg_linear_presplit: ldw %% 64");
    a.x = nullptr; a.w = w; a.lda = 0; a.ldw = ldw; a.M = m; a.N = n; a.K = k;
    const size_t rows = (size_t)eg_round_up(n, 64);
    a.whi = reinterpret_cast<const unsigned short*>(w + rows * ldw);
    a.wlo = a.whi + rows * ldw;
    a.bias = bias; a.res1 = res1; a.res2 = res2; a.ldr = ldr; a.y = y; a.ldc = ldc; a.relu = relu;
    a.a_shift = 0; a.a_seq = 1; a.k_per_split = (int)eg_round_up(k, 64); a.partial = nullptr;
    const int xko = (int)eg_round_up(k_x, 64) / 8, mt = eg_cdiv(m, 64);
    const bf8* xhi = reinterpret_cast<const bf8*>(x_images);
    const bf8* xlo = xhi + (size_t)mt * xko * 64;
    EgProfScope prof(3, 2.0 * m * (double)n * k, (hipStream_t)stream);
    return dispatch_presplit(a, xhi, xlo, xko, precision, (hipStream_t)stream, &prof);
}

extern "C" int eg_linear_presplit_causal(const void* x_images, int32_t k_x, const void* zero_line, const float* w, int32_t ldw, const float* bias,
                                         const float* res2, int32_t ldr, float* y, int32_t ldc, void* y_images, int32_t y_k, int32_t m, int32_t n,
                                         int32_t k_tap, int32_t relu, int32_t shift, int32_t period, int32_t precision, void* stream) {
    EG_REQUIRE(x_images && zero_line && w && (y || y_images) && m > 0 && n > 0 && k_tap > 0, EG_ERR_BAD_ARG, "eg_linear_presplit_causal: null pointer or empty shape");
    EG_REQUIRE(precision == EG_PREC_BF16X3 || precision == EG_PREC_BF16, EG_ERR_BAD_ARG, "eg_linear_presplit_causal: bf16 modes only");
    EG_REQUIRE((k_tap & 31) == 0 && ldw == 2 * k_tap && (ldw & 63) == 0 && (k_x & 63) == 0 && k_x >= k_tap, EG_ERR_ALIGN,
               "eg_linear_presplit_causal: k_tap %% 32, ldw == 2 * k_tap, k_x %% 64");
    EG_REQUIRE(shift > 0 && period > 0, EG_ERR_BAD_ARG, "eg_linear_presplit_causal: shift=%d period=%d", shift, period);
    EgiLinear p;
    p.ximg = x_images; p.xK = k_x; p.xk0 = 0; p.w = w; p.ldw = ldw; p.bias = bias; p.res2 = res2; p.ldr = ldr; p.y = y; p.ldc = ldc;
    p.yimg = y_images; p.yK = y_k; p.m = m; p.n = n; p.k = 2 * k_tap; p.relu = relu; p.precision = precision;
    p.xs_shift = shift; p.xs_period = period; p.xzero = zero_line;
    return egi_linear(p, (hipStream_t)stream);
}
```

emotiongestures_amd/csrc/generator.hip:

```cpp
#include "common.h"
#include <string>
#include <vector>
#include <algorithm>
#include <string.h>
#include <map>
#include <mutex>

static thread_local char g_err[512] = "";
void eg_set_error(const char* fmt, ...) {
    va_list ap;
    va_start(ap, fmt);
    vsnprintf(g_err, sizeof(g_err), fmt, ap);
    va_end(ap);
}
extern "C" const char* eg_last_error(void) { return g_err; }
std::atomic<long long> g_eg_launches{0};
extern "C" int64_t eg_launch_count(void) { return (int64_t)g_eg_launches.load(std::memory_order_relaxed); }
bool g_eg_launch_hist = [] { const char* e = getenv("EG_LAUNCH_HIST"); return e && e[0] == '1'; }();
namespace {
std::mutex g_hist_mu;
std::map<std::string, long long> g_hist;
}
void egi_count_launch(const char* what) {
    std::lock_guard<std::mutex> lk(g_hist_mu);
    ++g_hist[what];
}
extern "C" int64_t eg_launch_histogram(char* buf, int64_t cap, int32_t reset) {
    std::lock_guard<std::mutex> lk(g_hist_mu);
    std::string out;
    for (const auto& kv : g_hist) out += kv.first + " " + std::to_string(kv.second) + "\n";
    if (buf && cap > 0) {
        const size_t n = out.size() < (size_t)cap - 1 ? out.size() : (size_t)cap - 1;
        memcpy(buf, out.data(), n);
        buf[n] = 0;
    }
    if (reset) g_hist.clear();
    return (int64_t)out.size() + 1;
}
extern "C" const char* eg_version(void) { return "emogest-hip 0.1 (gfx950)"; }
static int g_default_precision = EG_PREC_F32;
extern "C" int eg_set_default_precision(int p) {
    EG_REQUIRE(p >= 0 && p <= 2, EG_ERR_BAD_ARG, "eg_set_default_precision: %d", p);
    g_default_precision = p;
    return EG_OK;
}
extern "C" int eg_get_default_precision(void) { return g_default_precision; }

int eg_ensure_dynamic_lds(const void* kernel, size_t bytes, const char* who) {
    if (bytes <= 64 * 1024) return EG_OK;
    static std::mutex mu;
    static std::map<std::pair<const void*, int>, size_t> done;
    int dev = 0;
    EG_HIP_TRY(hipGetDevice(&dev), who);
    std::lock_guard<std::mutex> lk(mu);
    size_t& have = done[std::make_pair(kernel, dev)];
    if (have >= bytes) return EG_OK;
    if (bytes > 160 * 1024) { eg_set_error("%s: needs %zu B of LDS (160 KiB per CU)", who, bytes); return EG_ERR_UNSUPPORTED; }
    hipError_t e = hipFuncSetAttribute(kernel, hipFuncAttributeMaxDynamicSharedMemorySize, (int)bytes);
    if (e != hipSuccess) {
        eg_set_error("%s: cannot reserve %zu B of LDS on device %d: %s", who, bytes, dev, hipGetErrorString(e));
        return EG_ERR_HIP;
    }
    have = bytes;
    return EG_OK;
}

namespace {
struct ProfRec { hipEvent_t a, b; int64_t tag; double flops; bool ok; int wgs; };
std::vector<ProfRec> g_prof;
int g_prof_n = 0;
bool g_prof_on = false;
}
EgProfScope::EgProfScope(int64_t tag, double flops, hipStream_t s) : slot(-1), st(s) {
    if (!g_prof_on || g_prof_n >= (int)g_prof.size()) return;
    slot = g_prof_n++;
    g_prof[slot].tag = tag;
    g_prof[slot].flops = flops;
    g_prof[slot].wgs = 0;
    g_prof[slot].ok = hipEventRecord(g_prof[slot].a, st) == hipSuccess;
}
void EgProfScope::workgroups(int n) {
    if (slot >= 0) g_prof[slot].wgs = n;
}
EgProfScope::~EgProfScope() {
    if (slot >= 0 && hipEventRecord(g_prof[slot].b, st) != hipSuccess) g_prof[slot].ok = false;
}
extern "C" int eg_profile_enable(int32_t max_records) {
    EG_REQUIRE(max_records > 0, EG_ERR_BAD_ARG, "eg_profile_enable: max_records=%d", max_records);
    while ((int)g_prof.size() < max_records) {
        ProfRec r;
        if (hipEventCreate(&r.a) != hipSuccess || hipEventCreate(&r.b) != hipSuccess) { eg_set_error("hipEventCreate failed"); return EG_ERR_HIP; }
        r.tag = 0; r.flops = 0; r.ok = false; r.wgs = 0;
        g_prof.push_back(r);
    }
    g_prof_n = 0;
    g_prof_on = true;
    return EG_OK;
}
extern "C" int eg_profile_disable(void) { g_prof_on = false; return EG_OK; }
extern "C" int32_t eg_profile_read_workgroups(int32_t* workgroups, int32_t capacity) {
    const int n = g_prof_n < capacity ? g_prof_n : capacity;
    for (int i = 0; i < n; ++i) workgroups[i] = g_prof[i].wgs;
    return n;
}
extern "C" int32_t eg_profile_read(int64_t* tags, double* flops, float* ms, int32_t capacity) {
    int n = g_prof_n < capacity ? g_prof_n : capacity;
    for (int i = 0; i < n; ++i) {
        float t = 0.f;
        if (!g_prof[i].ok || hipEventSynchronize(g_prof[i].b) != hipSuccess || hipEventElapsedTime(&t, g_prof[i].a, g_prof[i].b) != hipSuccess) {
            eg_set_error("eg_profile_read: event %d was not recorded / cannot be read", i);
            g_prof_n = 0;
            return EG_ERR_HIP;
        }
        tags[i] = g_prof[i].tag; flops[i] = g_prof[i].flops; ms[i] = t;
    }
    g_prof_n = 0;
    return n;
}

struct EgiPriorW {
    const float *w1, *b1, *s1, *t1, *w2, *b2, *s2, *t2;
    const float *sp_w0, *sp_b0, *sp_w1, *sp_b1, *tc_w0, *tc_b0, *tc_w1, *tc_b1, *tm_w0, *tm_b0, *tm_w1, *tm_b1;
};
int egi_embedding(const int64_t* idx, const float* table, float* out, int rows, int dim, int ld, int n_words, hipStream_t st);
int egi_embedding_img(const int64_t* idx, const float* table, float* out, void* img, void* zero_line, int rows, int dim, int ld, int n_words, hipStream_t st);
int egi_add(const float* a, const float* b, float* out, size_t n, int row_len, int period, hipStream_t st);
int egi_add_img(const float* a, const float* b, float* out, void* img, size_t n, int row_len, int period, hipStream_t st);
int egi_time_linear(const float* x, const float* w, const float* bias, float* y, int batch, int L, int C, int ld, hipStream_t st);
int egi_copy2d(const float* src, int lds_, float* dst, int ldd, int rows, int cols, hipStream_t st);
int egi_linear(const EgiLinear& p, hipStream_t st);
int egi_layernorm(const float* x, const float* gamma, const float* beta, float* y, void* img, int rows, int d, float eps, hipStream_t st);
int egi_attention(const float* q, int ldq, const float* k, int ldk, const float* v, int ldv, float* out, int ldo, float* attn,
                  void* oimg, int batch, int heads, int lq, int lk, int dk, int precision, hipStream_t st);
int egi_add_bcast(const float* a, const float* b, float* out, size_t rows, int row_len, int period, int rep, hipStream_t st);
int egi_prior_encoder(const float* prior, const EgiPriorW& w, float* cat, float* tm_mem, float* tm_pe, float* tm_gram, int batch,
                      int P, int F, int D, int Dpad, int chunk, int variant, hipStream_t st);
int egi_conv1d(const float* x, const float* w, const float* bias, const float* scale, const float* shift, float* y, int n, int cin,
               int cout, int lin, int k, int stride, int pad, int act, hipStream_t st);
int egi_convt1d(const float* x, const float* w, const float* bias, const float* scale, const float* shift, float* y, int n, int cin,
                int cout, int lin, hipStream_t st);
int egi_swap01(const void* in, void* out, int A, int B, size_t inner_words, hipStream_t st);
int egi_rows_by_table(const void* in, void* out, const int32_t* table, int rows, size_t inner_words, bool scatter, hipStream_t st);
int egi_rollout_handoff_ragged(const float* pose, const float* prior_in, const float* alpha, float* track, float* windows, float* prior_out,
                               const int32_t* table, int N, int U, int active, int Wmax, int s, int F, int P, int D, hipStream_t st);
int egi_rollout_handoff(const float* pose, const float* prior_in, const float* alpha, float* track, float* windows, float* prior_out, int U,
                        int W, int w, int F, int P, int D, hipStream_t st);
int egi_small_linear(const float* x, int ldx, const float* w, const float* bias, float* y, int ldy, int n, int in, int out,
                     hipStream_t st);
int egi_cvae_sample_fused(EgiCvaeFused a, int n, hipStream_t st, int* taken);

#define EG_TRY(expr)              \
    do {                          \
        int _rc = (expr);         \
        if (_rc) return _rc;      \
    } while (0)

namespace {

struct Layout {
    std::vector<EgWeightEntry> entries;
    int64_t total = 0;
    int64_t add(const std::string& key, int kind, int d0, int d1, int d2, int d3, int64_t numel) {
        total = eg_round_up(total, 16);
        EgWeightEntry e;
        memset(&e, 0, sizeof(e));
        snprintf(e.key, sizeof(e.key), "%s", key.c_str());
        e.kind = kind; e.dims[0] = d0; e.dims[1] = d1; e.dims[2] = d2; e.dims[3] = d3;
        e.offset = total; e.numel = numel;
        entries.push_back(e);
        total += numel;
        return e.offset;
    }
    int64_t raw(const std::string& key, int64_t numel) { return add(key, EG_PACK_RAW, (int)numel, 0, 0, 0, numel); }
    int64_t vec(const std::string& key, int n, int npad) { return add(key, EG_PACK_VEC_PAD, n, npad, 0, 0, npad); }
};

struct LinW { int64_t w = -1, b = -1; int n = 0, k = 0, npad = 0, kpad = 0; };
struct ConvW { int64_t w = -1, bias = -1, scale = -1, shift = -1; int cin = 0, cout = 0, coutp = 0, stride = 1; };
struct BlockW {
    ConvW c1, c2;
    int64_t se_w1, se_b1, se_w2, se_b2;
    bool ds = false;
    int64_t ds_w = -1, ds_scale = -1, ds_shift = -1;
    int64_t ds_wb = -1;
    int cin, cout, stride;
};
struct MhaW { LinW q, kv, qkv, o; int64_t ln_g, ln_b; };
struct FfnW { LinW w1, w2; int64_t ln_g, ln_b; };

LinW add_linear(Layout& L, const std::string& prefix, int n, int k, bool bias, int kpad_force = 0, int npad_force = 0) {
    LinW w;
    w.n = n; w.k = k;
    w.npad = npad_force ? npad_force : (int)eg_round_up(n, 64);
    w.kpad = kpad_force ? kpad_force : (int)eg_round_up(k, 64);
    w.w = L.add(prefix + ".weight", EG_PACK_LINEAR, n, k, w.npad, w.kpad, (int64_t)w.npad * w.kpad * 2);
    if (bias) w.b = L.vec(prefix + ".bias", n, w.npad);
    return w;
}
ConvW add_conv3(Layout& L, const std::string& key, int cin, int cout, int stride) {
    ConvW c;
    c.cin = cin; c.cout = cout; c.coutp = (int)eg_round_up(cout, 16); c.stride = stride;
    c.w = L.add(key + ".weight", EG_PACK_CONV3X3, cout, cin, c.coutp, 0, (int64_t)9 * cin * c.coutp * 2);
    return c;
}
void add_bn(Layout& L, const std::string& prefix, int n, int npad, int64_t& scale, int64_t& shift) {
    scale = L.add(prefix, EG_PACK_BN_SCALE, n, npad, 0, 0, npad);
    shift = L.add(prefix, EG_PACK_BN_SHIFT, n, npad, 0, 0, npad);
}
LinW add_linear_cat(Layout& L, const std::vector<std::string>& prefixes, int n_each, int k, bool bias) {
    LinW w;
    const int n = n_each * (int)prefixes.size();
    w.n = n; w.k = k; w.npad = (int)eg_round_up(n, 64); w.kpad = (int)eg_round_up(k, 64);
    std::string wk, bk;
// ... 19 lines not shown
    if (self_attn) {
        m.qkv = add_linear_cat(L, {p + ".w_qs", p + ".w_ks", p + ".w_vs"}, d, d, false);
    } else {
        m.q = add_linear(L, p + ".w_qs", d, d, false);
        m.kv = add_linear_cat(L, {p + ".w_ks", p + ".w_vs"}, d, d, false);
    }
    m.o = add_linear(L, p + ".fc", d, d, false);
    m.ln_g = L.raw(p + ".layer_norm.weight", d);
    m.ln_b = L.raw(p + ".layer_norm.bias", d);
    return m;
}
FfnW add_ffn(Layout& L, const std::string& p, int d, int di) {
    FfnW f;
    f.w1 = add_linear(L, p + ".w_1", di, d, true);
    f.w2 = add_linear(L, p + ".w_2", d, di, true);
    f.ln_g = L.raw(p + ".layer_norm.weight", d);
    f.ln_b = L.raw(p + ".layer_norm.bias", d);
    return f;
}

struct Carver {
    int64_t off = 0;
    int64_t take(int64_t floats) {
        const int64_t o = off;
        off = eg_round_up(off + floats * (int64_t)sizeof(float), 256);
        return o;
    }
};

}

struct EgGenerator {
    EgGeneratorConfig cfg;
    Layout L;
    int H1, W1, H2, W2, H3, W3, HW3, Dpad, stages[3] = {3, 4, 6}, filters[3] = {32, 64, 128};
    int64_t stem_w, stem_b, stem_scale, stem_shift;
    std::vector<BlockW> blocks;
    ConvW final_conv;
    LinW a_fc1, a_fc2, emosem0, emo2, sem2, fus0, fus2, cls[4], post[4], prior_h0, prior_h2, txt_dec;
    bool fuse_se = true;
    bool fold = false;
    bool shared_chip = false;
    LinW f_audio, f_emo, f_sem, f_post, f_prior;
    int64_t pos_table;
    std::vector<MhaW> enc_attn, dec_attn;
    std::vector<FfnW> enc_ffn, dec_ffn;
    int64_t pc_w1, pc_b1, pc_s1, pc_t1, pc_w2, pc_b2, pc_s2, pc_t2;
    int64_t sp_w0, sp_b0, sp_w1, sp_b1, tc_w0, tc_b0, tc_w1, tc_b1, tm_w0, tm_b0, tm_w1, tm_b1;
    int64_t emb;
    struct TcnConv { LinW tap0, tap1, taps; int64_t bias; };
    std::vector<TcnConv> tcn;
    int64_t txt_fc1_w, txt_fc1_b;
    int Cpad;
    bool keep_taps = false;
    bool concurrent = false;
    mutable hipStream_t side[2] = {nullptr, nullptr};
    mutable hipEvent_t ev_fork = nullptr, ev_join[2] = {nullptr, nullptr};
    int ensure_streams() const {
        if (side[0]) return EG_OK;
        for (int i = 0; i < 2; ++i) {
            if (hipStreamCreateWithFlags(&side[i], hipStreamNonBlocking) != hipSuccess ||
                hipEventCreateWithFlags(&ev_join[i], hipEventDisableTiming) != hipSuccess) {
                eg_set_error("cannot create side stream/event");
                return EG_ERR_HIP;
            }
        }
        if (hipEventCreateWithFlags(&ev_fork, hipEventDisableTiming) != hipSuccess) { eg_set_error("cannot create event"); return EG_ERR_HIP; }
        return EG_OK;
    }
    ~EgGenerator() {
        for (int i = 0; i < 2; ++i) {
            if (side[i]) (void)hipStreamDestroy(side[i]);
            if (ev_join[i]) (void)hipEventDestroy(ev_join[i]);
        }
        if (ev_fork) (void)hipEventDestroy(ev_fork);
    }
};

namespace {

struct GenWs {
    int64_t act[3], gap, gate, scv, amap, afc1, afeat, emo_t, emo, sem_t, sem, cls_part, cls_h[3], cls_out;
    int64_t fus_in, fus_h, fusion, xa, xb, q, qkv, ao, proj, ffn_h, im_x[2], im_enc, im_h, im_a[3], im_p[2];
    int64_t prior_cat, prior_h, prior_enc, prior_rep, tm_mem, tm_pe, tm_gram, post_a, post_b, post_c, pose;
    int64_t t_emb, t_a, t_b, t_c, t_out, im_t[3], t_zero;
    int64_t tap_stem, tap_l[3];
    int64_t total;
};

GenWs carve(const EgGenerator* g, int B, int NB = 0) {
    if (NB <= 0) NB = B;
    const EgGeneratorConfig& c = g->cfg;
    GenWs w;
    Carver cv;
    const int64_t BF = (int64_t)B * c.frames, D = c.d_model, NF = (int64_t)NB * c.frames;
    const int64_t act = (int64_t)B * g->H1 * g->W1 * 32;
    for (int i = 0; i < 3; ++i) w.act[i] = cv.take(act);
    {
        int64_t gap_per_clip = 0;
        int h = g->H1, wd = g->W1;
        for (const BlockW& b : g->blocks) {
            const int ho = (h + 2 - 3) / b.stride + 1, wo = (wd + 2 - 3) / b.stride + 1;
            const int64_t need = (int64_t)eg_conv3x3_gap_tiles(ho, wo, b.cout, b.cout, 1) * b.cout;
            gap_per_clip = need > gap_per_clip ? need : gap_per_clip;
            const int64_t need1 = (int64_t)eg_conv3x3_gap_tiles(h, wd, b.cin, b.cout, b.stride) * b.cout;
            gap_per_clip = need1 > gap_per_clip ? need1 : gap_per_clip;
            h = ho; wd = wo;
        }
        w.gap = cv.take((int64_t)B * gap_per_clip);
    }
    w.gate = cv.take((int64_t)B * 128);
    w.scv = cv.take((int64_t)3 * B * 128);
    w.amap = cv.take(BF * g->HW3);
    w.afc1 = cv.take(BF * D); w.afeat = cv.take(BF * D);
    w.emo_t = cv.take(BF * D * 2); w.emo = cv.take(BF * D); w.sem_t = cv.take(16); w.sem = cv.take(BF * D);
    w.cls_part = cv.take((int64_t)(c.frames > 64 ? c.frames : 64) * B * D);
    w.cls_h[0] = cv.take((int64_t)B * D); w.cls_h[1] = cv.take((int64_t)B * 256); w.cls_h[2] = cv.take((int64_t)B * 64);
    w.cls_out = cv.take((int64_t)B * 16);
    w.fus_in = cv.take(NF * D); w.fus_h = cv.take(NF * D); w.fusion = cv.take(NF * D);
    w.xa = cv.take(NF * D); w.xb = cv.take(NF * D);
    w.q = cv.take(NF * D); w.qkv = cv.take(NF * D * 3); w.ao = cv.take(NF * D); w.proj = cv.take(NF * D);
    w.ffn_h = cv.take(NF * c.d_inner);
    {
        const int64_t N64 = eg_round_up(NF, 64), B64 = eg_round_up(BF, 64), KX = D > g->Dpad ? D : g->Dpad;
        w.im_x[0] = cv.take(N64 * KX); w.im_x[1] = cv.take(N64 * KX); w.im_enc = cv.take(N64 * D); w.im_h = cv.take(N64 * c.d_inner);
        w.im_a[0] = cv.take(B64 * D); w.im_a[1] = cv.take(B64 * D); w.im_a[2] = cv.take(B64 * D * 2);
        w.im_p[0] = cv.take(B64 * D); w.im_p[1] = cv.take(B64 * D);
    }
    w.prior_cat = cv.take(BF * g->Dpad); w.prior_h = cv.take(BF * D); w.prior_enc = cv.take(BF * D);
    w.prior_rep = cv.take(NB > B ? NF * D : 16);
    w.tm_mem = cv.take((int64_t)B * c.pose_dim); w.tm_pe = cv.take((int64_t)B * c.chunk + 16); w.tm_gram = cv.take((int64_t)c.pose_dim * c.chunk);
    w.post_a = cv.take(NF * D * 4); w.post_b = cv.take(NF * D); w.post_c = cv.take(NF * g->Dpad); w.pose = cv.take(NF * c.pose_dim);
    const int64_t BT = (int64_t)B * c.text_len;
    w.t_emb = cv.take(BT * g->Cpad); w.t_a = cv.take(BT * g->Cpad); w.t_b = cv.take(BT * g->Cpad); w.t_c = cv.take(BT * g->Cpad);
    w.t_out = cv.take(BT * 512);
    for (int i = 0; i < 3; ++i) w.im_t[i] = cv.take(eg_round_up(BT, 64) * g->Cpad);
    w.t_zero = cv.take((int64_t)g->Cpad * 32);
    w.tap_stem = w.tap_l[0] = w.tap_l[1] = w.tap_l[2] = -1;
    if (g->keep_taps) {
        w.tap_stem = cv.take(act);
        w.tap_l[0] = cv.take(act);
        w.tap_l[1] = cv.take((int64_t)B * g->H2 * g->W2 * 64);
        w.tap_l[2] = cv.take((int64_t)B * g->H3 * g->W3 * 128);
    }
    w.total = cv.off;
    return w;
}

inline float* P(void* ws, int64_t off) { return reinterpret_cast<float*>(reinterpret_cast<char*>(ws) + off); }

int run_linear(const float* arena, const LinW& w, const float* x, int lda, float* y, int ldc, int m, int relu, const float* res1,
               int ldr, int prec, hipStream_t st, int n_override = 0) {
    return eg_linear(x, lda, arena + w.w, w.kpad, w.b >= 0 ? arena + w.b : nullptr, res1, nullptr, ldr, y, ldc, m,
                     n_override ? n_override : w.n, w.kpad <= lda ? w.kpad : w.k, relu, 0, 0, prec, st);
}

int run_conv(const float* arena, const ConvW& c, const float* x, float* y, float* gap, int B, int h, int w, int relu, int nchw,
             int prec, hipStream_t st) {
    return eg_conv3x3(x, arena + c.w, c.bias >= 0 ? arena + c.bias : nullptr, c.scale >= 0 ? arena + c.scale : nullptr,
                      c.shift >= 0 ? arena + c.shift : nullptr, y, gap, B, h, w, c.cin, c.cout, c.stride, relu, nchw, prec, st);
}

struct Act { float* f = nullptr; int ld = 0; void* img = nullptr; int kimg = 0; };
inline Act act(float* f, int ld, void* img = nullptr, int kimg = 0) { Act a; a.f = f; a.ld = ld; a.img = img; a.kimg = kimg; return a; }

int lin(const EgGenerator* g, const float* arena, const LinW& w, const Act& x, int xk0, const Act& y, bool want_f32, int m, int relu,
        const float* res1, int ldr, hipStream_t st, int n_override = 0, int splits = 0, float* partial = nullptr) {
    const bool img_ok = g->cfg.precision != EG_PREC_F32;
    EgiLinear p;
    p.w = arena + w.w; p.ldw = w.kpad; p.bias = w.b >= 0 ? arena + w.b : nullptr;
    p.res1 = res1; p.ldr = ldr; p.m = m; p.n = n_override ? n_override : w.n; p.relu = relu; p.precision = g->cfg.precision;
    p.shared_chip = g->shared_chip ? 1 : 0;
    if (img_ok && x.img) {
        p.ximg = x.img; p.xK = x.kimg; p.xk0 = xk0; p.k = w.kpad;
    } else {
        p.x = x.f + xk0; p.lda = x.ld; p.k = (w.kpad <= x.ld - xk0 || w.kpad <= x.ld) && (x.ld >= w.kpad) ? w.kpad : w.k;
    }
    const bool yimg = img_ok && y.img;
    if (yimg) { p.yimg = y.img; p.yK = y.kimg; }
    if (want_f32 || !yimg) { p.y = y.f; p.ldc = y.ld; }
    if (splits > 1 && img_ok && x.img && !yimg) { p.splits = splits; p.partial = partial; }
    return egi_linear(p, st);
}

int run_mha(const EgGenerator* g, const float* arena, const MhaW& m, const Act& xq, const Act& xkv, const Act& out, const GenWs& w,
            void* ws, int B, int Lq, int Lk, hipStream_t st) {
    const int D = g->cfg.d_model;
    float *qkv = P(ws, w.qkv), *ao = P(ws, w.ao), *pr = P(ws, w.proj);
    void* aimg = g->cfg.precision != EG_PREC_F32 ? P(ws, w.im_h) : nullptr;
    if (!xkv.f) {
        EG_TRY(lin(g, arena, m.qkv, xq, 0, act(qkv, 3 * D), true, B * Lq, 0, nullptr, 0, st));
        EG_TRY(egi_attention(qkv, 3 * D, qkv + D, 3 * D, qkv + 2 * D, 3 * D, ao, D, nullptr, aimg, B, g->cfg.n_head, Lq, Lk, g->cfg.d_k, g->cfg.precision, st));
    } else {
        float* q = P(ws, w.q);
        EG_TRY(lin(g, arena, m.q, xq, 0, act(q, D), true, B * Lq, 0, nullptr, 0, st));
        EG_TRY(lin(g, arena, m.kv, xkv, 0, act(qkv, 2 * D), true, B * Lk, 0, nullptr, 0, st));
        EG_TRY(egi_attention(q, D, qkv, 2 * D, qkv + D, 2 * D, ao, D, nullptr, aimg, B, g->cfg.n_head, Lq, Lk, g->cfg.d_k, g->cfg.precision, st));
    }
    EG_TRY(lin(g, arena, m.o, act(ao, D, aimg, D), 0, act(pr, D), true, B * Lq, 0, xq.f, D, st));
    return egi_layernorm(pr, arena + m.ln_g, arena + m.ln_b, out.f, g->cfg.precision != EG_PREC_F32 ? out.img : nullptr, B * Lq, D, 1e-6f, st);
}

int run_mha_kv(const EgGenerator* g, const float* arena, const MhaW& m, const Act& xq, const float* kv, const Act& out, const GenWs& w,
               void* ws, int B, int Lq, int Lk, hipStream_t st) {
    const int D = g->cfg.d_model;
    float *q = P(ws, w.q), *ao = P(ws, w.ao), *pr = P(ws, w.proj);
    void* aimg = g->cfg.precision != EG_PREC_F32 ? P(ws, w.im_h) : nullptr;
    EG_TRY(lin(g, arena, m.q, xq, 0, act(q, D), true, B * Lq, 0, nullptr, 0, st));
    EG_TRY(egi_attention(q, D, kv, 2 * D, kv + D, 2 * D, ao, D, nullptr, aimg, B, g->cfg.n_head, Lq, Lk, g->cfg.d_k, g->cfg.precision, st));
    EG_TRY(lin(g, arena, m.o, act(ao, D, aimg, D), 0, act(pr, D), true, B * Lq, 0, xq.f, D, st));
    return egi_layernorm(pr, arena + m.ln_g, arena + m.ln_b, out.f, g->cfg.precision != EG_PREC_F32 ? out.img : nullptr, B * Lq, D, 1e-6f, st);
}

int run_ffn(const EgGenerator* g, const float* arena, const FfnW& f, const Act& x, const Act& out, const GenWs& w, void* ws, int rows,
            hipStream_t st) {
    const int D = g->cfg.d_model, DI = g->cfg.d_inner;
    float *h = P(ws, w.ffn_h), *pr = P(ws, w.proj);
    const Act hid = act(h, DI, P(ws, w.im_h), DI);
    EG_TRY(lin(g, arena, f.w1, x, 0, hid, false, rows, 1, nullptr, 0, st));
    const int sp = (g->cfg.precision != EG_PREC_F32 && rows <= 64 && DI >= 2048 && 4 * D <= DI) ? 4 : 0;
    EG_TRY(lin(g, arena, f.w2, hid, 0, act(pr, D), true, rows, 0, x.f, D, st, 0, sp, h));
    return egi_layernorm(pr, arena + f.ln_g, arena + f.ln_b, out.f, g->cfg.precision != EG_PREC_F32 ? out.img : nullptr, rows, D, 1e-6f, st);
}


int run_audio_tower(const EgGenerator* g, const float* arena, const float* spec, const GenWs& w, void* ws, int B, hipStream_t st) {
    const int prec = g->cfg.precision, F = g->cfg.frames, D = g->cfg.d_model;
    float* bufs[3] = {P(ws, w.act[0]), P(ws, w.act[1]), P(ws, w.act[2])};
    float *gap = P(ws, w.gap), *gate = P(ws, w.gate);
    int xi = 0, h = g->H1, wd = g->W1, bi = 0;
    EG_TRY(eg_stem_conv(spec, arena + g->stem_w, arena + g->stem_b, arena + g->stem_scale, arena + g->stem_shift, bufs[0], B, g->H1,
                        g->W1, 32, st));
    if (g->keep_taps)
        EG_HIP_TRY(hipMemcpyAsync(P(ws, w.tap_stem), bufs[0], sizeof(float) * (size_t)B * g->H1 * g->W1 * 32, hipMemcpyDeviceToDevice, st), "tap copy");
    for (int s = 0; s < 3; ++s) {
        for (int j = 0; j < g->stages[s]; ++j, ++bi) {
            const BlockW& bw = g->blocks[bi];
            const int t1 = (xi + 1) % 3, t2 = (xi + 2) % 3;
            const int ho = (h + 2 - 3) / bw.stride + 1, wo = (wd + 2 - 3) / bw.stride + 1;
            if (g->fuse_se && (!bw.ds || prec != EG_PREC_F32)) {
                EG_TRY(eg_se_block_fused(bufs[xi], arena + bw.c1.w, arena + bw.c1.scale, arena + bw.c1.shift, arena + bw.c2.w, arena + bw.c2.scale,
                                         arena + bw.c2.shift, arena + bw.se_w1, arena + bw.se_b1, arena + bw.se_w2, arena + bw.se_b2,
                                         bw.ds ? arena + bw.ds_wb : nullptr, bw.ds ? arena + bw.ds_scale : nullptr, bw.ds ? arena + bw.ds_shift : nullptr,
                                         bufs[t1], bufs[t2], gap, gate, P(ws, w.scv), B, h, wd, bw.cin, bw.cout, bw.stride, prec, st));
                xi = t2; h = ho; wd = wo;
                continue;
            }
            EG_TRY(run_conv(arena, bw.c1, bufs[xi], bufs[t1], nullptr, B, h, wd, 1, 0, prec, st));
            EG_TRY(run_conv(arena, bw.c2, bufs[t1], bufs[t2], gap, B, ho, wo, 0, 0, prec, st));
            const int tiles = eg_conv3x3_gap_tiles(ho, wo, bw.cout, bw.cout, 1);
            EG_TRY(eg_se_gate(gap, tiles, arena + bw.se_w1, arena + bw.se_b1, arena + bw.se_w2, arena + bw.se_b2, gate, B, bw.cout,
                              ho * wo, st));
            EG_TRY(eg_se_residual_relu(bufs[t2], gate, bufs[xi], bw.ds ? arena + bw.ds_w : nullptr, bw.ds ? arena + bw.ds_scale : nullptr,
                                       bw.ds ? arena + bw.ds_shift : nullptr, bufs[t1], B, ho, wo, bw.cout, h, wd, bw.cin, bw.stride, st));
            xi = t1; h = ho; wd = wo;
        }
        if (g->keep_taps)
            EG_HIP_TRY(hipMemcpyAsync(P(ws, w.tap_l[s]), bufs[xi], sizeof(float) * (size_t)B * h * wd * g->filters[s], hipMemcpyDeviceToDevice, st), "tap copy");
    }
    float* amap = P(ws, w.amap);
    EG_TRY(run_conv(arena, g->final_conv, bufs[xi], amap, nullptr, B, h, wd, 0, 1, prec, st));
    if (g->fold) return lin(g, arena, g->f_audio, act(amap, g->HW3), 0, act(P(ws, w.afeat), D, P(ws, w.im_a[1]), D), true, B * F, 0, nullptr, 0, st);
    const Act h1 = act(P(ws, w.afc1), D, P(ws, w.im_a[0]), D);
    EG_TRY(lin(g, arena, g->a_fc1, act(amap, g->HW3), 0, h1, false, B * F, 0, nullptr, 0, st));
    return lin(g, arena, g->a_fc2, h1, 0, act(P(ws, w.afeat), D, P(ws, w.im_a[1]), D), true, B * F, 0, nullptr, 0, st);
}

int causal_conv(const EgGenerator* g, const float* arena, const EgGenerator::TcnConv& cv, void* ximg, const void* zero, float* y, void* yimg,
                const float* res2, int rows, int d, int L, hipStream_t st) {
    EgiLinear p;
    p.ximg = ximg; p.xK = g->Cpad; p.w = arena + cv.taps.w; p.ldw = cv.taps.kpad; p.bias = arena + cv.bias; p.res2 = res2; p.ldr = g->Cpad;
    p.y = y; p.ldc = g->Cpad; p.yimg = yimg; p.yK = g->Cpad; p.m = rows; p.n = g->Cpad; p.k = cv.taps.kpad; p.relu = 1;
    p.precision = g->cfg.precision; p.shared_chip = g->shared_chip ? 1 : 0;
    p.xs_shift = d; p.xs_period = L; p.xzero = zero;
    return egi_linear(p, st);
}

bool text_one_launch(const EgGenerator* g) {
    if (g->cfg.precision == EG_PREC_F32 || g->cfg.embed_dim != g->cfg.tcn_hidden || g->Cpad != (int)eg_round_up(g->cfg.tcn_hidden, 64)) return false;
    const char* e = getenv("EG_TEXT_TAPS");
    return !(e && e[0] == '2');
}

int run_text(const EgGenerator* g, const float* arena, const int64_t* text, float* out, const GenWs& w, void* ws, int B, hipStream_t st) {
    const EgGeneratorConfig& c = g->cfg;
    const int L = c.text_len, C = c.tcn_hidden, ld = g->Cpad, rows = B * L, prec = c.precision;
    float *x = P(ws, w.t_emb), *h1 = P(ws, w.t_a), *h2 = P(ws, w.t_b), *y = P(ws, w.t_c);
    if (text_one_launch(g)) {
        void *xi = P(ws, w.im_t[0]), *hi = P(ws, w.im_t[1]), *yi = P(ws, w.im_t[2]), *zero = P(ws, w.t_zero);
        EG_TRY(egi_embedding_img(text, arena + g->emb, x, xi, zero, rows, c.embed_dim, ld, c.n_words, st));
        for (int i = 0; i < c.tcn_layers; ++i) {
            const bool last = i + 1 == c.tcn_layers;
            EG_TRY(causal_conv(g, arena, g->tcn[2 * i], xi, zero, nullptr, hi, nullptr, rows, 1 << i, L, st));
            EG_TRY(causal_conv(g, arena, g->tcn[2 * i + 1], hi, zero, y, last ? nullptr : yi, x, rows, 1 << i, L, st));
            float* t = x; x = y; y = t;
            void* ti = xi; xi = yi; yi = ti;
        }
        EG_TRY(egi_time_linear(x, arena + g->txt_fc1_w, arena + g->txt_fc1_b, h1, B, L, C, ld, st));
        return eg_linear(h1, ld, arena + g->txt_dec.w, g->txt_dec.kpad, arena + g->txt_dec.b, nullptr, nullptr, 0, out, 512, rows, 512, C, 0,
                         0, 0, prec, st);
    }
    EG_TRY(egi_embedding(text, arena + g->emb, x, rows, c.embed_dim, ld, c.n_words, st));
    for (int i = 0; i < c.tcn_layers; ++i) {
        const int d = 1 << i;
        const EgGenerator::TcnConv& c1 = g->tcn[2 * i];
        const EgGenerator::TcnConv& c2 = g->tcn[2 * i + 1];
        EG_TRY(eg_linear(x, ld, arena + c1.tap0.w, c1.tap0.kpad, arena + c1.bias, nullptr, nullptr, 0, h1, ld, rows, C, C, 0, d, L, prec, st));
        EG_TRY(eg_linear(x, ld, arena + c1.tap1.w, c1.tap1.kpad, nullptr, h1, nullptr, ld, h1, ld, rows, C, C, 1, 0, 0, prec, st));
        EG_TRY(eg_linear(h1, ld, arena + c2.tap0.w, c2.tap0.kpad, arena + c2.bias, nullptr, nullptr, 0, h2, ld, rows, C, C, 0, d, L, prec, st));
        EG_TRY(eg_linear(h1, ld, arena + c2.tap1.w, c2.tap1.kpad, nullptr, h2, x, ld, y, ld, rows, C, C, 1, 0, 0, prec, st));
        float* t = x; x = y; y = t;
    }
    EG_TRY(egi_time_linear(x, arena + g->txt_fc1_w, arena + g->txt_fc1_b, h1, B, L, C, ld, st));
    return eg_linear(h1, ld, arena + g->txt_dec.w, g->txt_dec.kpad, arena + g->txt_dec.b, nullptr, nullptr, 0, out, 512, rows, 512, C, 0,
                     0, 0, prec, st);
}

int run_prior(const EgGenerator* g, const float* arena, const float* prior, const GenWs& w, void* ws, int B, hipStream_t st) {
    const EgGeneratorConfig& c = g->cfg;
    EgiPriorW pw;
    memset(&pw, 0, sizeof(pw));
    pw.w1 = arena + g->pc_w1; pw.b1 = arena + g->pc_b1; pw.s1 = arena + g->pc_s1; pw.t1 = arena + g->pc_t1;
    pw.w2 = arena + g->pc_w2; pw.b2 = arena + g->pc_b2; pw.s2 = arena + g->pc_s2; pw.t2 = arena + g->pc_t2;
    if (c.variant == 1) {
        pw.sp_w0 = arena + g->sp_w0; pw.sp_b0 = arena + g->sp_b0; pw.sp_w1 = arena + g->sp_w1; pw.sp_b1 = arena + g->sp_b1;
        pw.tc_w0 = arena + g->tc_w0; pw.tc_b0 = arena + g->tc_b0; pw.tc_w1 = arena + g->tc_w1; pw.tc_b1 = arena + g->tc_b1;
        pw.tm_w0 = arena + g->tm_w0; pw.tm_b0 = arena + g->tm_b0; pw.tm_w1 = arena + g->tm_w1; pw.tm_b1 = arena + g->tm_b1;
    }
    EG_TRY(egi_prior_encoder(prior, pw, P(ws, w.prior_cat), P(ws, w.tm_mem), P(ws, w.tm_pe), P(ws, w.tm_gram), B, c.prior_frames, c.frames,
                             c.pose_dim, g->Dpad, c.chunk, c.variant, st));
    const int rows = B * c.frames;
    if (g->fold)
        return lin(g, arena, g->f_prior, act(P(ws, w.prior_cat), g->Dpad), 0, act(P(ws, w.prior_enc), c.d_model, P(ws, w.im_p[1]), c.d_model), true, rows, 0,
                   nullptr, 0, st);
    const Act ph = act(P(ws, w.prior_h), c.d_model, P(ws, w.im_p[0]), c.d_model);
    EG_TRY(lin(g, arena, g->prior_h0, act(P(ws, w.prior_cat), g->Dpad), 0, ph, false, rows, 0, nullptr, 0, st));
    return lin(g, arena, g->prior_h2, ph, 0, act(P(ws, w.prior_enc), c.d_model, P(ws, w.im_p[1]), c.d_model), true, rows, 0, nullptr, 0, st);
}

bool add_images(const EgGenerator* g) {
    if (g->cfg.precision == EG_PREC_F32) return false;
    const char* e = getenv("EG_ADD_IMAGES");
    return !(e && e[0] == '0');
}
Act fusion_act(const EgGenerator* g, const GenWs& w, void* ws) {
    const int D = g->cfg.d_model;
    return act(P(ws, w.fus_in), D, add_images(g) ? P(ws, w.im_x[1]) : nullptr, D);
}

int run_encoder(const EgGenerator* g, const float* arena, const Act& fusion_in, Act& enc_out, const GenWs& w, void* ws, int NB,
                hipStream_t st) {
    const EgGeneratorConfig& c = g->cfg;
    const int F = c.frames, D = c.d_model, rows = NB * F;
    void *im0 = P(ws, w.im_x[0]), *im1 = P(ws, w.im_x[1]), *ime = P(ws, w.im_enc);
    const Act fh = act(P(ws, w.fus_h), D, im0, D);
    EG_TRY(lin(g, arena, g->fus0, fusion_in, 0, fh, false, rows, 1, nullptr, 0, st));
    EG_TRY(lin(g, arena, g->fus2, fh, 0, act(P(ws, w.fusion), D), true, rows, 0, nullptr, 0, st));
    float *xa = P(ws, w.xa), *xb = P(ws, w.xb);
    void* xa_img = add_images(g) ? im1 : nullptr;
    EG_TRY(egi_add_img(P(ws, w.fusion), arena + g->pos_table, xa, xa_img, (size_t)rows * D, D, F, st));
    Act x = act(xa, D, xa_img, D);
    for (int l = 0; l < c.n_layers; ++l) {
        const Act mid = act(xb, D, im0, D);
        const Act nxt = act(xa, D, l + 1 < c.n_layers ? im1 : ime, D);
        EG_TRY(run_mha(g, arena, g->enc_attn[l], x, Act(), mid, w, ws, NB, F, F, st));
        EG_TRY(run_ffn(g, arena, g->enc_ffn[l], mid, nxt, w, ws, rows, st));
        x = nxt;
    }
    enc_out = x;
    return EG_OK;
}

int run_post(const EgGenerator* g, const float* arena, const Act& dx, float* pose, const GenWs& w, void* ws, int rows, hipStream_t st) {
    const EgGeneratorConfig& c = g->cfg;
    const int D = c.d_model;
    void *im0 = P(ws, w.im_x[0]), *im1 = P(ws, w.im_x[1]), *imh = P(ws, w.im_h);
    if (g->fold) return lin(g, arena, g->f_post, dx, 0, act(pose, c.pose_dim), true, rows, 0, nullptr, 0, st);
    const Act pa = act(P(ws, w.post_a), D * 4, imh, D * 4), pb = act(P(ws, w.post_b), D, im0, D), pc = act(P(ws, w.post_c), g->Dpad, im1, g->Dpad);
    EG_TRY(lin(g, arena, g->post[0], dx, 0, pa, false, rows, 0, nullptr, 0, st));
    EG_TRY(lin(g, arena, g->post[1], pa, 0, pb, false, rows, 0, nullptr, 0, st));
    EG_TRY(lin(g, arena, g->post[2], pb, 0, pc, false, rows, 0, nullptr, 0, st, g->Dpad));
    return lin(g, arena, g->post[3], pc, 0, act(pose, c.pose_dim), true, rows, 0, nullptr, 0, st);
}

int run_decoder(const EgGenerator* g, const float* arena, const Act& prior_enc, const Act& enc_out, float* const* kv, float* pose,
                const GenWs& w, void* ws, int NB, hipStream_t st) {
    const EgGeneratorConfig& c = g->cfg;
    const int F = c.frames, D = c.d_model, rows = NB * F;
    void *im0 = P(ws, w.im_x[0]), *im1 = P(ws, w.im_x[1]);
    float *xb = P(ws, w.xb), *da = P(ws, w.fus_h);
    Act dx = prior_enc;
    for (int l = 0; l < c.n_layers; ++l) {
        const Act mid = act(xb, D, im0, D);
        const Act nxt = act(da, D, im1, D);
        if (kv) EG_TRY(run_mha_kv(g, arena, g->dec_attn[l], dx, kv[l], mid, w, ws, NB, F, F, st));
        else EG_TRY(run_mha(g, arena, g->dec_attn[l], dx, enc_out, mid, w, ws, NB, F, F, st));
        EG_TRY(run_ffn(g, arena, g->dec_ffn[l], mid, nxt, w, ws, rows, st));
        dx = nxt;
    }
    return run_post(g, arena, dx, pose, w, ws, rows, st);
}

int run_transformer(const EgGenerator* g, const float* arena, const Act& fusion_in, const Act& prior_enc, float* pose, const GenWs& w,
                    void* ws, int NB, hipStream_t st) {
    Act enc_out;
    EG_TRY(run_encoder(g, arena, fusion_in, enc_out, w, ws, NB, st));
    return run_decoder(g, arena, prior_enc, enc_out, nullptr, pose, w, ws, NB, st);
}

int run_heads(const EgGenerator* g, const float* arena, float* emo, float* sem, float* pred, const GenWs& w, void* ws, int B, hipStream_t st) {
    const EgGeneratorConfig& c = g->cfg;
    const int F = c.frames, D = c.d_model, rows = B * F, prec = c.precision;
    const Act afeat = act(P(ws, w.afeat), D, P(ws, w.im_a[1]), D), es = act(P(ws, w.emo_t), 2 * D, P(ws, w.im_a[2]), 2 * D);
    if (g->fold) {
        EG_TRY(lin(g, arena, g->f_emo, afeat, 0, act(emo, D), true, rows, 0, nullptr, 0, st));
        EG_TRY(lin(g, arena, g->f_sem, afeat, 0, act(sem, D), true, rows, 0, nullptr, 0, st));
    } else {
        EG_TRY(lin(g, arena, g->emosem0, afeat, 0, es, false, rows, 0, nullptr, 0, st));
        EG_TRY(lin(g, arena, g->emo2, es, 0, act(emo, D), true, rows, 0, nullptr, 0, st));
        EG_TRY(lin(g, arena, g->sem2, es, D, act(sem, D), true, rows, 0, nullptr, 0, st));
    }
    const int K0 = F * D;
    EG_TRY(eg_linear_splitk(emo, K0, arena + g->cls[0].w, g->cls[0].kpad, arena + g->cls[0].b, P(ws, w.cls_h[0]), D, B, D, K0, 1,
                            F, P(ws, w.cls_part), prec, st));
    EG_TRY(run_linear(arena, g->cls[1], P(ws, w.cls_h[0]), D, P(ws, w.cls_h[1]), 256, B, 1, nullptr, 0, prec, st));
    EG_TRY(run_linear(arena, g->cls[2], P(ws, w.cls_h[1]), 256, P(ws, w.cls_h[2]), 64, B, 1, nullptr, 0, prec, st));
    return run_linear(arena, g->cls[3], P(ws, w.cls_h[2]), 64, pred, 8, B, 0, nullptr, 0, prec, st);
}

int validate_cfg(const EgGeneratorConfig& c) {
    EG_REQUIRE(c.frames > c.prior_frames && c.prior_frames >= c.chunk && c.chunk > 0, EG_ERR_BAD_ARG, "config: frames/prior/chunk inconsistent");
    EG_REQUIRE(c.d_model % 64 == 0 && c.d_model >= 64 && c.d_model <= 2048, EG_ERR_UNSUPPORTED, "config: d_model=%d", c.d_model);
    EG_REQUIRE(c.d_k == 64 && c.n_head * c.d_k == c.d_model, EG_ERR_UNSUPPORTED, "config: heads*d_k must equal d_model with d_k=64");
    EG_REQUIRE(c.n_mels % 16 == 0 && c.n_mels <= 512 && c.spec_len >= 4, EG_ERR_UNSUPPORTED, "config: spectrogram %dx%d", c.n_mels, c.spec_len);
    EG_REQUIRE(c.frames <= 128, EG_ERR_UNSUPPORTED, "config: frames=%d > 128 (final conv width)", c.frames);
    EG_REQUIRE(c.embed_dim == c.tcn_hidden && c.embed_dim % 4 == 0, EG_ERR_UNSUPPORTED, "config: TCN needs embed_dim == hidden, %%4");
    EG_REQUIRE(c.variant == 0 || c.variant == 1, EG_ERR_BAD_ARG, "config: variant=%d", c.variant);
    EG_REQUIRE(c.precision >= 0 && c.precision <= 2, EG_ERR_BAD_ARG, "config: precision=%d", c.precision);
    EG_REQUIRE(c.n_position >= c.frames, EG_ERR_BAD_ARG, "config: n_position < frames");
    EG_REQUIRE(c.pose_dim > 0 && c.pose_dim <= 1024 && c.n_words > 0 && c.text_len > 0 && c.text_len <= 128, EG_ERR_BAD_ARG, "config: sizes");
    return EG_OK;
}

}

extern "C" int eg_generator_default_config(EgGeneratorConfig* c) {
    EG_REQUIRE(c, EG_ERR_BAD_ARG, "null config");
    memset(c, 0, sizeof(*c));
    c->frames = 34; c->pose_dim = 126; c->prior_frames = 4; c->chunk = 4; c->d_model = 512; c->d_inner = 2048; c->n_layers = 3;
    c->n_head = 8; c->d_k = 64; c->n_mels = 128; c->spec_len = 124; c->text_len = 60; c->n_words = 200; c->embed_dim = 300;
    c->tcn_hidden = 300; c->tcn_layers = 3; c->variant = 0; c->precision = g_default_precision; c->n_position = 60;
    return EG_OK;
}

extern "C" int eg_generator_create(const EgGeneratorConfig* cfg, EgGenerator** out) {
    EG_REQUIRE(cfg && out, EG_ERR_BAD_ARG, "eg_generator_create: null pointer");
    EG_TRY(validate_cfg(*cfg));
    EgGenerator* g = new EgGenerator();
    g->cfg = *cfg;
    g->keep_taps = cfg->reserved[0] != 0;
    g->concurrent = cfg->reserved[1] != 0;
    g->fold = cfg->reserved[2] != 0;
    g->fuse_se = cfg->reserved[3] == 0;
    g->shared_chip = cfg->reserved[4] != 0;
    const EgGeneratorConfig& c = g->cfg;
    g->H1 = c.n_mels; g->W1 = c.spec_len;
    g->H2 = (g->H1 - 1) / 2 + 1; g->W2 = (g->W1 - 1) / 2 + 1;
    g->H3 = (g->H2 - 1) / 2 + 1; g->W3 = (g->W2 - 1) / 2 + 1;
    g->HW3 = g->H3 * g->W3;
    if (g->HW3 % 8 != 0) { delete g; eg_set_error("config: final map %dx%d not a multiple of 8", g->H3, g->W3); return EG_ERR_UNSUPPORTED; }
    g->Dpad = (int)eg_round_up(c.pose_dim, 64);
    g->Cpad = (int)eg_round_up(c.tcn_hidden, 64);
    Layout& L = g->L;
    const int D = c.d_model, F = c.frames, P_ = c.prior_frames, PL = F - P_, PD = c.pose_dim;
    const std::string fe = "audio_encoder.feat_extractor";
    g->stem_w = L.add(fe + ".conv1.weight", EG_PACK_STEM, 32, 0, 0, 0, 9 * 32);
    g->stem_b = L.raw(fe + ".conv1.bias", 32);
    add_bn(L, fe + ".bn1", 32, 32, g->stem_scale, g->stem_shift);
    int inpl = 32;
    for (int s = 0; s < 3; ++s) {
        const int planes = g->filters[s];
        for (int j = 0; j < g->stages[s]; ++j) {
            BlockW b;
            const std::string p = fe + ".layer" + std::to_string(s + 1) + "." + std::to_string(j);
            b.stride = (s > 0 && j == 0) ? 2 : 1;
            b.cin = inpl; b.cout = planes;
            b.c1 = add_conv3(L, p + ".conv1", inpl, planes, b.stride);
            add_bn(L, p + ".bn1", planes, planes, b.c1.scale, b.c1.shift);
            b.c2 = add_conv3(L, p + ".conv2", planes, planes, 1);
            add_bn(L, p + ".bn2", planes, planes, b.c2.scale, b.c2.shift);
            b.se_w1 = L.raw(p + ".se.fc.0.weight", planes / 8 * planes);
            b.se_b1 = L.raw(p + ".se.fc.0.bias", planes / 8);
            b.se_w2 = L.raw(p + ".se.fc.2.weight", planes * (planes / 8));
            b.se_b2 = L.raw(p + ".se.fc.2.bias", planes);
            b.ds = (b.stride != 1 || inpl != planes);
            if (b.ds) {
                b.ds_w = L.add(p + ".downsample.0.weight", EG_PACK_CONV1X1, planes, inpl, 0, 0, (int64_t)inpl * planes);
                b.ds_wb = L.add(p + ".downsample.0.weight", EG_PACK_CONV1X1_BF16, planes, inpl, 0, 0, (int64_t)inpl * planes);
                add_bn(L, p + ".downsample.1", planes, planes, b.ds_scale, b.ds_shift);
            }
            g->blocks.push_back(b);
            inpl = planes;
        }
// ... 39 lines not shown
    g->pc_w1 = L.raw(pp + ".pred_conv.0.weight", (int64_t)PL * P_ * 3); g->pc_b1 = L.raw(pp + ".pred_conv.0.bias", PL);
    add_bn(L, pp + ".pred_conv.2", PL, PL, g->pc_s1, g->pc_t1);
    g->pc_w2 = L.raw(pp + ".pred_conv.3.weight", (int64_t)PL * PL * 3); g->pc_b2 = L.raw(pp + ".pred_conv.3.bias", PL);
    add_bn(L, pp + ".pred_conv.5", PL, PL, g->pc_s2, g->pc_t2);
    if (c.variant == 1) {
        const int CD = c.chunk * PD;
        const std::string sp = pp + ".spatial_memory.spatial_chunk_encoder", tm = pp + ".temporal_memory";
        g->sp_w0 = L.raw(sp + ".0.weight", (int64_t)PD * CD); g->sp_b0 = L.raw(sp + ".0.bias", PD);
        g->sp_w1 = L.raw(sp + ".2.weight", (int64_t)PD * PD); g->sp_b1 = L.raw(sp + ".2.bias", PD);
        g->tc_w0 = L.raw(tm + ".temporal_chunk_encoder.0.weight", (int64_t)PD * CD); g->tc_b0 = L.raw(tm + ".temporal_chunk_encoder.0.bias", PD);
        g->tc_w1 = L.raw(tm + ".temporal_chunk_encoder.2.weight", (int64_t)PD * PD); g->tc_b1 = L.raw(tm + ".temporal_chunk_encoder.2.bias", PD);
        g->tm_w0 = L.raw(tm + ".temporal_memory_encoder.0.weight", (int64_t)c.chunk * CD); g->tm_b0 = L.raw(tm + ".temporal_memory_encoder.0.bias", c.chunk);
        g->tm_w1 = L.raw(tm + ".temporal_memory_encoder.2.weight", (int64_t)c.chunk * c.chunk); g->tm_b1 = L.raw(tm + ".temporal_memory_encoder.2.bias", c.chunk);
    }
    g->pos_table = L.add("encoder.position_enc.pos_table", EG_PACK_POS_TABLE, F, D, 0, 0, (int64_t)F * D);
    for (int l = 0; l < c.n_layers; ++l) {
        const std::string e = "encoder.layer_stack." + std::to_string(l), d = "decoder.layer_stack." + std::to_string(l);
        g->enc_attn.push_back(add_mha(L, e + ".slf_attn", D, true));
        g->enc_ffn.push_back(add_ffn(L, e + ".pos_ffn", D, c.d_inner));
        g->dec_attn.push_back(add_mha(L, d + ".enc_attn", D, false));
        g->dec_ffn.push_back(add_ffn(L, d + ".pos_ffn", D, c.d_inner));
    }
    g->emb = L.raw("text_encoder.embedding.weight", (int64_t)c.n_words * c.embed_dim);
    for (int i = 0; i < c.tcn_layers; ++i)
        for (int j = 1; j <= 2; ++j) {
            EgGenerator::TcnConv tc;
            const std::string p = "text_encoder.tcn.network." + std::to_string(i) + ".conv" + std::to_string(j);
            const int C = c.tcn_hidden, npad = (int)eg_round_up(C, 64);
            for (int tap = 0; tap < 2; ++tap) {
                LinW w;
                w.n = C; w.k = C; w.npad = npad; w.kpad = g->Cpad;
                w.w = L.add(p, EG_PACK_WN_TAP, C, C, tap, g->Cpad, (int64_t)npad * g->Cpad * 2);
                (tap == 0 ? tc.tap0 : tc.tap1) = w;
            }
            tc.taps.n = C; tc.taps.k = 2 * g->Cpad; tc.taps.npad = npad; tc.taps.kpad = 2 * g->Cpad;
            tc.taps.w = L.add(p + ".weight_g|" + p + ".weight_v", EG_PACK_WN_TAPS, C, C, npad, g->Cpad, (int64_t)npad * g->Cpad * 4);
            tc.bias = L.vec(p + ".bias", C, npad);
            g->tcn.push_back(tc);
        }
    g->txt_fc1_w = L.raw("text_encoder.fc1.0.weight", (int64_t)c.text_len * c.text_len);
    g->txt_fc1_b = L.raw("text_encoder.fc1.0.bias", c.text_len);
    g->txt_dec = add_linear(L, "text_encoder.decoder", 512, c.tcn_hidden, true, g->Cpad, 0);
    L.total = eg_round_up(L.total, 16);
    *out = g;
    return EG_OK;
}

extern "C" void eg_generator_destroy(EgGenerator* g) { delete g; }
extern "C" int64_t eg_generator_arena_floats(const EgGenerator* g) { return g ? g->L.total : 0; }
extern "C" int32_t eg_generator_num_weights(const EgGenerator* g) { return g ? (int32_t)g->L.entries.size() : 0; }
extern "C" int eg_generator_weight_entry(const EgGenerator* g, int32_t i, EgWeightEntry* out) {
    EG_REQUIRE(g && out && i >= 0 && i < (int)g->L.entries.size(), EG_ERR_BAD_ARG, "eg_generator_weight_entry: index %d", i);
    *out = g->L.entries[i];
    return EG_OK;
}
extern "C" int64_t eg_generator_workspace_bytes(const EgGenerator* g, int32_t batch) {
    if (!g || batch <= 0) return 0;
    return carve(g, batch).total;
}

extern "C" int eg_generator_forward(const EgGenerator* g, const float* arena, int32_t B, const float* spec, const int64_t* text,
                                    const float* prior, const float* sampled, float* pose, float* emotion_feature,
                                    float* semantic_feature, float* emotion_prediction, float* text_embedding, void* ws,
                                    int64_t ws_bytes, void* stream) {
    EG_REQUIRE(g && arena && spec && text && prior && ws, EG_ERR_BAD_ARG, "eg_generator_forward: null pointer");
    EG_REQUIRE(B > 0, EG_ERR_BAD_ARG, "eg_generator_forward: batch=%d", B);
    const GenWs w = carve(g, B);
    EG_REQUIRE(ws_bytes >= w.total, EG_ERR_WORKSPACE, "eg_generator_forward: workspace %lld < %lld bytes", (long long)ws_bytes, (long long)w.total);
    EG_REQUIRE(eg_aligned16(ws) && eg_aligned16(arena) && eg_aligned16(spec), EG_ERR_ALIGN, "eg_generator_forward: 16-byte alignment");
    hipStream_t st = (hipStream_t)stream;
    const EgGeneratorConfig& c = g->cfg;
    const int F = c.frames, D = c.d_model, rows = B * F;

    float* txt = text_embedding ? text_embedding : P(ws, w.t_out);
    hipStream_t s_text = st, s_prior = st;
    if (g->concurrent) {
        EG_TRY(g->ensure_streams());
        s_text = g->side[0]; s_prior = g->side[1];
        EG_HIP_TRY(hipEventRecord(g->ev_fork, st), "branch fork");
        EG_HIP_TRY(hipStreamWaitEvent(s_text, g->ev_fork, 0), "branch fork");
        EG_HIP_TRY(hipStreamWaitEvent(s_prior, g->ev_fork, 0), "branch fork");
    }
    EG_TRY(run_text(g, arena, text, txt, w, ws, B, s_text));
    EG_TRY(run_prior(g, arena, prior, w, ws, B, s_prior));
    if (g->concurrent) {
        EG_HIP_TRY(hipEventRecord(g->ev_join[0], s_text), "branch join");
        EG_HIP_TRY(hipEventRecord(g->ev_join[1], s_prior), "branch join");
    }
    EG_TRY(run_audio_tower(g, arena, spec, w, ws, B, st));
    float* emo = emotion_feature ? emotion_feature : P(ws, w.emo);
    float* sem = semantic_feature ? semantic_feature : P(ws, w.sem);
    EG_TRY(run_heads(g, arena, emo, sem, emotion_prediction ? emotion_prediction : P(ws, w.cls_out), w, ws, B, st));
    const Act fus_in = fusion_act(g, w, ws);
    EG_TRY(egi_add_img(sampled ? sampled : emo, sem, fus_in.f, fus_in.img, (size_t)rows * D, D, 0, st));
    float* pose_out = pose ? pose : P(ws, w.pose);
    if (g->concurrent) {
        EG_HIP_TRY(hipStreamWaitEvent(st, g->ev_join[1], 0), "branch join");
        EG_HIP_TRY(hipStreamWaitEvent(st, g->ev_join[0], 0), "branch join");
    }
    return run_transformer(g, arena, fus_in, act(P(ws, w.prior_enc), D, P(ws, w.im_p[1]), D), pose_out, w, ws, B, st);
}

extern "C" int64_t eg_generator_draws_workspace_bytes(const EgGenerator* g, int32_t batch, int32_t draws) {
    if (!g || batch <= 0 || draws <= 0) return 0;
    return carve(g, batch, batch * draws).total;
}

extern "C" int eg_generator_forward_draws(const EgGenerator* g, const float* arena, int32_t B, int32_t R, const float* spec,
                                          const float* prior, const float* sampled, float* pose, void* ws, int64_t ws_bytes,
                                          void* stream) {
    EG_REQUIRE(g && arena && spec && prior && sampled && pose && ws, EG_ERR_BAD_ARG, "eg_generator_forward_draws: null pointer");
    EG_REQUIRE(B > 0 && R > 0, EG_ERR_BAD_ARG, "eg_generator_forward_draws: batch=%d draws=%d", B, R);
    const GenWs w = carve(g, B, B * R);
    EG_REQUIRE(ws_bytes >= w.total, EG_ERR_WORKSPACE, "eg_generator_forward_draws: workspace %lld < %lld bytes", (long long)ws_bytes, (long long)w.total);
    hipStream_t st = (hipStream_t)stream;
    const EgGeneratorConfig& c = g->cfg;
    const int F = c.frames, D = c.d_model, rows = B * F, prec = c.precision;
    EG_TRY(run_audio_tower(g, arena, spec, w, ws, B, st));
    EG_TRY(run_prior(g, arena, prior, w, ws, B, st));
    const Act afeat = act(P(ws, w.afeat), D, P(ws, w.im_a[1]), D), es = act(P(ws, w.emo_t), 2 * D, P(ws, w.im_a[2]), 2 * D);
    if (g->fold) {
        EG_TRY(lin(g, arena, g->f_sem, afeat, 0, act(P(ws, w.sem), D), true, rows, 0, nullptr, 0, st));
    } else {
        EG_TRY(lin(g, arena, g->emosem0, afeat, 0, es, false, rows, 0, nullptr, 0, st));
        EG_TRY(lin(g, arena, g->sem2, es, D, act(P(ws, w.sem), D), true, rows, 0, nullptr, 0, st));
    }
    EG_TRY(egi_add_bcast(sampled, P(ws, w.sem), P(ws, w.fus_in), (size_t)B * R * F, D, F, R, st));
    EG_TRY(egi_add_bcast(nullptr, P(ws, w.prior_enc), P(ws, w.prior_rep), (size_t)B * R * F, D, F, R, st));
    return run_transformer(g, arena, act(P(ws, w.fus_in), D), act(P(ws, w.prior_rep), D), pose, w, ws, B * R, st);
}

int egi_draws_fusion(const float* sampled, const float* semantic, float* fus_in, int U, int W, int R, size_t clip_floats, hipStream_t st);
int egi_draws_seed(const float* seed, float* prior, int U, int R, int PD, hipStream_t st);
namespace {
struct RollPlan {
    int U, R, N, steps;
    const int32_t* plan;
    const int32_t* windows_per;
    const int32_t* order;
    bool same_order;
    bool seed_in_order;
};

struct RollWs { GenWs a; int64_t kv[8], prior[2], spec, text, sampled, total; };
RollWs carve_rollout(const EgGenerator* g, int U, int64_t N, int R) {
    const EgGeneratorConfig& c = g->cfg;
    RollWs r;
    r.a = carve(g, (int)N, (int)(N * R));
    GenWs& w = r.a;
    Carver cv;
    cv.off = w.total;
    const int64_t UR = (int64_t)U * R, D = c.d_model;
    if (UR > N) {
        const int64_t BF = UR * c.frames, B64 = eg_round_up(BF, 64);
        w.prior_cat = cv.take(BF * g->Dpad); w.prior_h = cv.take(BF * D); w.prior_enc = cv.take(BF * D);
        w.im_p[0] = cv.take(B64 * D); w.im_p[1] = cv.take(B64 * D);
        w.tm_mem = cv.take(UR * c.pose_dim); w.tm_pe = cv.take(UR * c.chunk + 16);
    }
    for (int l = 0; l < c.n_layers; ++l) r.kv[l] = cv.take(N * R * c.frames * 2 * D);
    r.prior[0] = cv.take(UR * c.prior_frames * c.pose_dim);
    r.prior[1] = cv.take(UR * c.prior_frames * c.pose_dim);
    r.spec = cv.take(N * c.n_mels * c.spec_len);
    r.text = cv.take(N * c.text_len * 2);
    r.sampled = R == 1 ? cv.take(N * c.frames * D) : -1;
    r.total = cv.off;
    return r;
}

int roll_rows(const RollPlan& p, const void* in, void* out, size_t words, bool back, hipStream_t st) {
    if (p.plan) return egi_rows_by_table(in, out, p.plan, p.N, words, back, st);
    return back ? egi_swap01(in, out, p.steps, p.U, words, st) : egi_swap01(in, out, p.U, p.steps, words, st);
}

int rollout_phase_a(const EgGenerator* g, const float* arena, const RollPlan& p, const RollWs& r, void* ws, const float* spec,
                    const int64_t* text, const float* sampled, float* emotion_prediction, float* emotion_feature, float* semantic_feature,
                    float* text_embedding, float** kv, hipStream_t st) {
    const EgGeneratorConfig& c = g->cfg;
    const GenWs& w = r.a;
    const int F = c.frames, D = c.d_model, N = p.N, NR = p.N * p.R;
    const bool move = !p.same_order;
    if (move) {
        EG_TRY(roll_rows(p, spec, P(ws, r.spec), (size_t)c.n_mels * c.spec_len, false, st));
        spec = P(ws, r.spec);
        if (text_embedding) {
            EG_TRY(roll_rows(p, text, P(ws, r.text), (size_t)c.text_len * 2, false, st));
            text = reinterpret_cast<const int64_t*>(P(ws, r.text));
        }
        if (sampled && p.R == 1) {
            EG_TRY(roll_rows(p, sampled, P(ws, r.sampled), (size_t)F * D, false, st));
            sampled = P(ws, r.sampled);
        }
    }
    float* txt = move ? P(ws, w.t_out) : text_embedding;
    float* emo = move || !emotion_feature ? P(ws, w.emo) : emotion_feature;
    float* sem = move || !semantic_feature ? P(ws, w.sem) : semantic_feature;
    float* pred = move || !emotion_prediction ? P(ws, w.cls_out) : emotion_prediction;
    if (text_embedding) EG_TRY(run_text(g, arena, text, txt, w, ws, N, st));
    EG_TRY(run_audio_tower(g, arena, spec, w, ws, N, st));
    EG_TRY(run_heads(g, arena, emo, sem, pred, w, ws, N, st));
    Act fus_in = act(P(ws, w.fus_in), D);
    if (p.R == 1) {
        fus_in = fusion_act(g, w, ws);
        EG_TRY(egi_add_img(sampled ? sampled : emo, sem, fus_in.f, fus_in.img, (size_t)N * F * D, D, 0, st));
    } else EG_TRY(egi_draws_fusion(sampled, sem, fus_in.f, p.U, p.steps, p.R, (size_t)F * D, st));
    Act enc_out;
    EG_TRY(run_encoder(g, arena, fus_in, enc_out, w, ws, NR, st));
    for (int l = 0; l < c.n_layers; ++l) {
        kv[l] = P(ws, r.kv[l]);
        EG_TRY(lin(g, arena, g->dec_attn[l].kv, enc_out, 0, act(kv[l], 2 * D), true, NR * F, 0, nullptr, 0, st));
    }
    if (move) {
        if (text_embedding) EG_TRY(roll_rows(p, txt, text_embedding, (size_t)c.text_len * 512, true, st));
        if (emotion_feature) EG_TRY(roll_rows(p, emo, emotion_feature, (size_t)F * D, true, st));
        if (semantic_feature) EG_TRY(roll_rows(p, sem, semantic_feature, (size_t)F * D, true, st));
        if (emotion_prediction) EG_TRY(roll_rows(p, pred, emotion_prediction, 8, true, st));
    }
    return EG_OK;
}

int rollout_phase_b(const EgGenerator* g, const float* arena, const RollPlan& p, const RollWs& r, void* ws, float* const* kv,
                    const float* seed_pose, const float* alpha, float* track, float* windows, hipStream_t st) {
    const EgGeneratorConfig& c = g->cfg;
    const GenWs& w = r.a;
    const int F = c.frames, D = c.d_model, P_ = c.prior_frames, PD = c.pose_dim;
    const float* prior = seed_pose;
    if (p.R > 1) {
        EG_TRY(egi_draws_seed(seed_pose, P(ws, r.prior[1]), p.U, p.R, P_ * PD, st));
        prior = P(ws, r.prior[1]);
    } else if (!p.seed_in_order) {
        EG_TRY(egi_rows_by_table(seed_pose, P(ws, r.prior[1]), p.plan + p.N, p.U, (size_t)P_ * PD, false, st));
        prior = P(ws, r.prior[1]);
    }
    const Act prior_enc = act(P(ws, w.prior_enc), D, P(ws, w.im_p[1]), D);
    int batch = p.U * p.R;
    size_t slot = 0;
    for (int s = 0; s < p.steps; ++s) {
        if (p.plan)
            while (batch > 0 && p.windows_per[p.order[batch - 1]] <= s) --batch;
        EG_TRY(run_prior(g, arena, prior, w, ws, batch, st));
        float* step_kv[8];
        for (int l = 0; l < c.n_layers; ++l) step_kv[l] = kv[l] + slot * F * 2 * D;
        EG_TRY(run_decoder(g, arena, prior_enc, Act(), step_kv, P(ws, w.pose), w, ws, batch, st));
        float* next = P(ws, r.prior[s & 1]);
        if (p.plan)
            EG_TRY(egi_rollout_handoff_ragged(P(ws, w.pose), prior, alpha, track, windows, next, p.plan, p.N, p.U, batch, p.steps, s, F, P_, PD, st));
        else
            EG_TRY(egi_rollout_handoff(P(ws, w.pose), prior, alpha, track, windows, next, batch, p.steps, s, F, P_, PD, st));
        prior = next;
        slot += (size_t)batch;
    }
    return EG_OK;
}
}

extern "C" int64_t eg_generator_rollout_workspace_bytes(const EgGenerator* g, int32_t utterances, int32_t windows) {
    if (!g || utterances <= 0 || windows <= 0 || g->cfg.n_layers > 8 || (int64_t)utterances * windows > (1 << 20)) return 0;
    return carve_rollout(g, utterances, (int64_t)utterances * windows, 1).total;
}

extern "C" int eg_generator_forward_rollout(const EgGenerator* g, const float* arena, int32_t U, int32_t W, const float* spec,
                                            const int64_t* text, const float* seed_pose, const float* sampled, const float* alpha,
                                            float* track, float* windows, float* emotion_prediction, float* emotion_feature,
                                            float* semantic_feature, float* text_embedding, void* ws, int64_t ws_bytes, void* stream) {
    EG_REQUIRE(g && arena && spec && seed_pose && track && ws, EG_ERR_BAD_ARG, "eg_generator_forward_rollout: null pointer");
    EG_REQUIRE(U >= 1, EG_ERR_BAD_ARG, "eg_generator_forward_rollout: utterances=%d (need >= 1)", U);
    EG_REQUIRE(W >= 1, EG_ERR_BAD_ARG, "eg_generator_forward_rollout: windows=%d (need >= 1)", W);
    EG_REQUIRE((int64_t)U * W <= (1 << 20), EG_ERR_UNSUPPORTED, "eg_generator_forward_rollout: utterances*windows=%lld", (long long)U * W);
    EG_REQUIRE(text || !text_embedding, EG_ERR_BAD_ARG, "eg_generator_forward_rollout: text_embedding wanted without text");
    EG_REQUIRE(g->cfg.n_layers <= 8, EG_ERR_UNSUPPORTED, "eg_generator_forward_rollout: n_layers=%d > 8", g->cfg.n_layers);
    const RollWs r = carve_rollout(g, U, (int64_t)U * W, 1);
    EG_REQUIRE(ws_bytes >= r.total, EG_ERR_WORKSPACE, "eg_generator_forward_rollout: workspace %lld < %lld bytes", (long long)ws_bytes, (long long)r.total);
    EG_REQUIRE(eg_aligned16(ws) && eg_aligned16(arena) && eg_aligned16(spec), EG_ERR_ALIGN, "eg_generator_forward_rollout: 16-byte alignment");
    const bool same = U == 1 || W == 1;
    const RollPlan p = {U, 1, U * W, W, nullptr, nullptr, nullptr, same, true};
    hipStream_t st = (hipStream_t)stream;
    float* kv[8];
    EG_TRY(rollout_phase_a(g, arena, p, r, ws, spec, text, sampled, emotion_prediction, emotion_feature, semantic_feature, text_embedding, kv, st));
    return rollout_phase_b(g, arena, p, r, ws, kv, seed_pose, alpha, track, windows, st);
}

extern "C" int64_t eg_generator_rollout_draws_workspace_bytes(const EgGenerator* g, int32_t utterances, int32_t windows, int32_t draws) {
    if (!g || utterances <= 0 || windows <= 0 || draws <= 0 || g->cfg.n_layers > 8) return 0;
    const int64_t N = (int64_t)utterances * windows;
    if (N > (1 << 20) || N * draws > (1 << 20)) return 0;
    return carve_rollout(g, utterances, N, draws).total;
}

extern "C" int eg_generator_forward_rollout_draws(const EgGenerator* g, const float* arena, int32_t U, int32_t W, int32_t R, const float* spec,
                                                  const int64_t* text, const float* seed_pose, const float* sampled, const float* alpha,
                                                  float* track, float* windows, float* emotion_prediction, float* emotion_feature,
                                                  float* semantic_feature, float* text_embedding, void* ws, int64_t ws_bytes, void* stream) {
    EG_REQUIRE(g && arena && spec && seed_pose && sampled && track && ws, EG_ERR_BAD_ARG, "eg_generator_forward_rollout_draws: null pointer");
    EG_REQUIRE(U >= 1, EG_ERR_BAD_ARG, "eg_generator_forward_rollout_draws: utterances=%d (need >= 1)", U);
// ... 58 lines not shown
}

int egi_stream_reset(float* ring, float* prior, int64_t* ctr, const int32_t* mask, const float* seed, int U, int64_t ring_len, int PD,
                     hipStream_t st);
int egi_stream_push(float* ring, int64_t* ctr, const float* chunk, const int32_t* ends, float* clips, int U, int64_t hop, int n, int lag,
                    hipStream_t st);
int egi_stream_handoff(const float* pose, float* prior, int64_t* ctr, const float* alpha, float* rows_out, int32_t* valid_out,
                       float* window_out, int U, int F, int P, int D, hipStream_t st);
namespace {
struct StreamState { int64_t ring, prior, ctr, total, ring_len; int lag; };
int64_t stream_lag(int hop, int n) { return ((int64_t)n + hop - 1) / hop; }
bool stream_geometry_ok(const EgGenerator* g, int U, int hop, int n) {
    if (!g || U < 1 || U > (1 << 20) || hop < 1 || n < 1) return false;
    const int64_t per = stream_lag(hop, n) * hop + n;
    return per < ((int64_t)1 << 31) && (int64_t)U * per < ((int64_t)1 << 40);
}
StreamState carve_stream(const EgGenerator* g, int U, int hop, int n) {
    StreamState s;
    s.lag = (int)stream_lag(hop, n);
    s.ring_len = (int64_t)s.lag * hop;
    Carver cv;
    s.ring = cv.take((int64_t)U * s.ring_len);
    s.prior = cv.take((int64_t)U * g->cfg.prior_frames * g->cfg.pose_dim);
    s.ctr = cv.take((int64_t)U * 4 * 2);
    s.total = cv.off;
    return s;
}
inline int64_t* stream_ctr(void* state, const StreamState& s) { return reinterpret_cast<int64_t*>(reinterpret_cast<char*>(state) + s.ctr); }
}

extern "C" int64_t eg_stream_state_bytes(const EgGenerator* g, int32_t rows, int32_t hop_samples, int32_t n_samples) {
    if (!stream_geometry_ok(g, rows, hop_samples, n_samples)) return 0;
    return carve_stream(g, rows, hop_samples, n_samples).total;
}

extern "C" int eg_stream_reset(const EgGenerator* g, void* state, int32_t rows, int32_t hop_samples, int32_t n_samples,
                               const int32_t* row_mask, const float* seed_pose, void* stream) {
    EG_REQUIRE(g && state && seed_pose, EG_ERR_BAD_ARG, "eg_stream_reset: null pointer");
    EG_REQUIRE(stream_geometry_ok(g, rows, hop_samples, n_samples), EG_ERR_BAD_ARG, "eg_stream_reset: rows=%d hop_samples=%d n_samples=%d", rows,
               hop_samples, n_samples);
    EG_REQUIRE(eg_aligned16(state), EG_ERR_ALIGN, "eg_stream_reset: 16-byte alignment");
    const StreamState s = carve_stream(g, rows, hop_samples, n_samples);
    return egi_stream_reset(P(state, s.ring), P(state, s.prior), stream_ctr(state, s), row_mask, seed_pose, rows, s.ring_len,
                            g->cfg.prior_frames * g->cfg.pose_dim, (hipStream_t)stream);
}

extern "C" int eg_stream_push(const EgGenerator* g, void* state, int32_t rows, int32_t hop_samples, int32_t n_samples, const float* chunk,
                              const int32_t* ends, float* clips, void* stream) {
    EG_REQUIRE(g && state && chunk && clips, EG_ERR_BAD_ARG, "eg_stream_push: null pointer");
    EG_REQUIRE(stream_geometry_ok(g, rows, hop_samples, n_samples), EG_ERR_BAD_ARG, "eg_stream_push: rows=%d hop_samples=%d n_samples=%d", rows,
               hop_samples, n_samples);
    EG_REQUIRE(eg_aligned16(state), EG_ERR_ALIGN, "eg_stream_push: 16-byte alignment");
    const StreamState s = carve_stream(g, rows, hop_samples, n_samples);
    return egi_stream_push(P(state, s.ring), stream_ctr(state, s), chunk, ends, clips, rows, hop_samples, n_samples, s.lag, (hipStream_t)stream);
}

extern "C" int eg_stream_tail(const EgGenerator* g, const void* state, int32_t rows, int32_t hop_samples, int32_t n_samples, float* out,
                              void* stream) {
    EG_REQUIRE(g && state && out, EG_ERR_BAD_ARG, "eg_stream_tail: null pointer");
    EG_REQUIRE(stream_geometry_ok(g, rows, hop_samples, n_samples), EG_ERR_BAD_ARG, "eg_stream_tail: rows=%d hop_samples=%d n_samples=%d", rows,
               hop_samples, n_samples);
    const StreamState s = carve_stream(g, rows, hop_samples, n_samples);
    const int PD = g->cfg.prior_frames * g->cfg.pose_dim;
    return egi_copy2d(P(const_cast<void*>(state), s.prior), PD, out, PD, rows, PD, (hipStream_t)stream);
}

extern "C" int eg_generator_stream_step(const EgGenerator* g, const float* arena, void* state, int32_t U, int32_t hop_samples,
                                        int32_t n_samples, const float* spec, const int64_t* text, const float* sampled, const float* alpha,
                                        float* rows_out, int32_t* valid_out, float* window_out, float* emotion_prediction, void* ws,
                                        int64_t ws_bytes, void* stream) {
    EG_REQUIRE(g && arena && state && spec && rows_out && valid_out && ws, EG_ERR_BAD_ARG, "eg_generator_stream_step: null pointer");
    EG_REQUIRE(stream_geometry_ok(g, U, hop_samples, n_samples), EG_ERR_BAD_ARG, "eg_generator_stream_step: rows=%d hop_samples=%d n_samples=%d", U,
               hop_samples, n_samples);
    const GenWs w = carve(g, U);
    EG_REQUIRE(ws_bytes >= w.total, EG_ERR_WORKSPACE, "eg_generator_stream_step: workspace %lld < %lld bytes", (long long)ws_bytes, (long long)w.total);
    EG_REQUIRE(eg_aligned16(ws) && eg_aligned16(arena) && eg_aligned16(spec) && eg_aligned16(state), EG_ERR_ALIGN,
               "eg_generator_stream_step: 16-byte alignment");
    const StreamState s = carve_stream(g, U, hop_samples, n_samples);
    hipStream_t st = (hipStream_t)stream;
    const EgGeneratorConfig& c = g->cfg;
    const int F = c.frames, D = c.d_model, rows = U * F;
    float* prior = P(state, s.prior);
    if (text) EG_TRY(run_text(g, arena, text, P(ws, w.t_out), w, ws, U, st));
    EG_TRY(run_prior(g, arena, prior, w, ws, U, st));
    EG_TRY(run_audio_tower(g, arena, spec, w, ws, U, st));
    EG_TRY(run_heads(g, arena, P(ws, w.emo), P(ws, w.sem), emotion_prediction ? emotion_prediction : P(ws, w.cls_out), w, ws, U, st));
    const Act fus_in = fusion_act(g, w, ws);
    EG_TRY(egi_add_img(sampled ? sampled : P(ws, w.emo), P(ws, w.sem), fus_in.f, fus_in.img, (size_t)rows * D, D, 0, st));
    EG_TRY(run_transformer(g, arena, fus_in, act(P(ws, w.prior_enc), D, P(ws, w.im_p[1]), D), P(ws, w.pose), w, ws, U, st));
    return egi_stream_handoff(P(ws, w.pose), prior, stream_ctr(state, s), alpha, rows_out, valid_out, window_out, U, F, c.prior_frames, c.pose_dim,
                              st);
}

extern "C" int eg_generator_tap(const EgGenerator* g, int32_t batch, void* ws, const char* name, float** d_ptr, int64_t* numel) {
    EG_REQUIRE(g && ws && name && d_ptr && numel && batch > 0, EG_ERR_BAD_ARG, "eg_generator_tap: null pointer");
    const GenWs w = carve(g, batch);
    const EgGeneratorConfig& c = g->cfg;
    const int64_t BFD = (int64_t)batch * c.frames * c.d_model;
    const std::string n(name);
    int64_t off = -1, cnt = 0;
    if (n == "audio_feat") { off = w.afeat; cnt = BFD; }
    else if (n == "prior_enc") { off = w.prior_enc; cnt = BFD; }
    else if (n == "fusion") { off = w.fusion; cnt = BFD; }
    else if (n == "enc_out") { off = w.xa; cnt = BFD; }
    else if (n == "audio_map") { off = w.amap; cnt = (int64_t)batch * c.frames * g->HW3; }
    else if (n == "mha_out") { off = w.xb; cnt = BFD; }
    else if (n == "attn_q") { off = w.q; cnt = BFD; }
    else if (n == "attn_qkv") { off = w.qkv; cnt = 3 * BFD; }
    else if (n == "attn_out") { off = w.ao; cnt = BFD; }
    else if (n == "proj") { off = w.proj; cnt = BFD; }
    else if (n == "dec_out") { off = w.fus_h; cnt = BFD; }
    else if (g->keep_taps && n == "stem") { off = w.tap_stem; cnt = (int64_t)batch * g->H1 * g->W1 * 32; }
    else if (g->keep_taps && n == "layer1") { off = w.tap_l[0]; cnt = (int64_t)batch * g->H1 * g->W1 * 32; }
    else if (g->keep_taps && n == "layer2") { off = w.tap_l[1]; cnt = (int64_t)batch * g->H2 * g->W2 * 64; }
    else if (g->keep_taps && n == "layer3") { off = w.tap_l[2]; cnt = (int64_t)batch * g->H3 * g->W3 * 128; }
    EG_REQUIRE(off >= 0, EG_ERR_BAD_ARG, "eg_generator_tap: unknown or disabled tap '%s'", name);
    *d_ptr = P(ws, off);
    *numel = cnt;
    return EG_OK;
}

struct EgCvae {
    EgCvaeConfig cfg;
    Layout L;
    struct Conv { int64_t w, b, s, t; int cin, cout, k, stride, pad; bool act; };
    Conv enc[4], dec_conv[3];
    struct ConvT { int64_t w, b, s, t; int cin, cout; } dec_t[2];
    struct Lin { int64_t w, b; int in, out; } py0, py2, mu0, mu2, var0, var2, fz0, fz2;
};

namespace {
EgCvae::Lin cvae_lin(Layout& L, const std::string& p, int out, int in) {
    EgCvae::Lin l;
    l.in = in; l.out = out;
    l.w = L.raw(p + ".weight", (int64_t)out * in);
    l.b = L.raw(p + ".bias", out);
    return l;
}
EgCvae::Conv cvae_conv(Layout& L, const std::string& seq, int idx, int cout, int cin, int k, int stride, int pad, bool act) {
    EgCvae::Conv c;
    c.cin = cin; c.cout = cout; c.k = k; c.stride = stride; c.pad = pad; c.act = act; c.s = c.t = -1;
    const std::string p = seq + "." + std::to_string(idx);
    c.w = L.raw(p + ".weight", (int64_t)cout * cin * k);
    c.b = L.raw(p + ".bias", cout);
    if (act) add_bn(L, seq + "." + std::to_string(idx + 2), cout, cout, c.s, c.t);
    return c;
}
struct CvaeWs { int64_t py_h, zy, fz_h, z0, d1, d2, d3, d4, e1, e2, e3, e4, mu_h, var_h, z, total; };
CvaeWs cvae_carve(const EgCvae* c, int n) {
    CvaeWs w;
    Carver cv;
    const int F = c->cfg.frames, D = c->cfg.d_model, Q = D / 4;
    w.py_h = cv.take((int64_t)n * 16); w.zy = cv.take((int64_t)n * 64); w.fz_h = cv.take((int64_t)n * 128); w.z0 = cv.take((int64_t)n * 4 * Q);
    w.d1 = cv.take((int64_t)n * 8 * Q * 2); w.d2 = cv.take((int64_t)n * 16 * D); w.d3 = cv.take((int64_t)n * 32 * D); w.d4 = cv.take((int64_t)n * F * D);
    w.e1 = cv.take((int64_t)n * 32 * D); w.e2 = cv.take((int64_t)n * 16 * D); w.e3 = cv.take((int64_t)n * 8 * D / 2); w.e4 = cv.take((int64_t)n * 4 * Q);
    w.mu_h = cv.take((int64_t)n * 128); w.var_h = cv.take((int64_t)n * 128); w.z = cv.take((int64_t)n * 32);
    w.total = cv.off;
    return w;
}
int cvae_decode(const EgCvae* c, const float* A, const CvaeWs& w, void* ws, int n, float* out, hipStream_t st) {
    const int F = c->cfg.frames, D = c->cfg.d_model, Q = D / 4;
    EG_TRY(egi_small_linear(P(ws, w.zy), 64, A + c->fz0.w, A + c->fz0.b, P(ws, w.fz_h), 128, n, 64, 128, st));
    EG_TRY(egi_small_linear(P(ws, w.fz_h), 128, A + c->fz2.w, A + c->fz2.b, P(ws, w.z0), 4 * Q, n, 128, 4 * Q, st));
    EG_TRY(egi_convt1d(P(ws, w.z0), A + c->dec_t[0].w, A + c->dec_t[0].b, A + c->dec_t[0].s, A + c->dec_t[0].t, P(ws, w.d1), n, 4, 8, Q, st));
    EG_TRY(egi_convt1d(P(ws, w.d1), A + c->dec_t[1].w, A + c->dec_t[1].b, A + c->dec_t[1].s, A + c->dec_t[1].t, P(ws, w.d2), n, 8, 16, 2 * Q, st));
    const EgCvae::Conv* dc = c->dec_conv;
    EG_TRY(egi_conv1d(P(ws, w.d2), A + dc[0].w, A + dc[0].b, A + dc[0].s, A + dc[0].t, P(ws, w.d3), n, 16, 32, D, 3, 1, 1, 1, st));
    EG_TRY(egi_conv1d(P(ws, w.d3), A + dc[1].w, A + dc[1].b, A + dc[1].s, A + dc[1].t, P(ws, w.d4), n, 32, F, D, 3, 1, 1, 1, st));
// ... 103 lines not shown
```

include/emogest.h:

```cpp
#ifndef EMOGEST_H
#define EMOGEST_H

#include <stddef.h>
#include <stdint.h>

#ifdef __cplusplus
extern "C" {
#endif

typedef enum EgStatus {
    EG_OK = 0,
    EG_ERR_BAD_ARG = -1,
    EG_ERR_UNSUPPORTED = -2,
    EG_ERR_WORKSPACE = -3,
    EG_ERR_HIP = -4,
    EG_ERR_ALIGN = -5
} EgStatus;

typedef enum EgPrecision {
    EG_PREC_F32 = 0,
    EG_PREC_BF16X3 = 1,
    EG_PREC_BF16 = 2
} EgPrecision;

// ... 194 lines not shown
                          int32_t bones, const double* rest, const void* d_levels, const int32_t* d_frames, int32_t draws, int32_t frame_unit,
                          const float* d_mean, int32_t space, int32_t L, int32_t M, float* rotations, int64_t out_stride, void* stream);

#define EG_BEAT_MAX_FRAMES 1024
int eg_beat_tables(float* h_melfb_t , float* h_window , float* h_twiddle ,
                   int32_t* h_band );
int64_t eg_beat_workspace_bytes(int32_t batch, int32_t n_samples);
int eg_beat_align(const float* audio, int32_t batch, int32_t n_samples, const float* pose, int32_t frames, int32_t pose_dim,
                  int32_t pose_fps, int32_t t_start, int32_t t_end, double sigma, int32_t order, const float* d_melfb_t,
                  const float* d_window, const float* d_twiddle, const int32_t* d_band, void* workspace, int64_t workspace_bytes,
                  double* score, int32_t* n_audio_beats, float* oenv, float* rms, uint8_t* audio_beats, uint8_t* pose_beats,
                  void* stream);

int64_t eg_beat_tracks_meta_ints(int32_t recordings);
int eg_beat_tracks_meta(const int32_t* lengths, const int32_t* frames , const int32_t* t_end ,
                        int32_t pose_fps, int32_t recordings, int32_t* meta);
int64_t eg_beat_tracks_workspace_bytes(const int32_t* lengths, const int32_t* frames , int32_t recordings, int32_t draws,
                                       int32_t Tmax);
int eg_beat_align_tracks(const float* audio, int32_t recordings, int64_t stride, const int32_t* lengths, const int32_t* d_meta,
                         const float* pose, int32_t draws, int32_t Tmax, int32_t pose_dim, const int32_t* frames, int32_t pose_fps,
                         int32_t t_start, const int32_t* t_end, double sigma, int32_t order, const float* d_melfb_t, const float* d_window,
                         const float* d_twiddle, const int32_t* d_band, void* workspace, int64_t workspace_bytes, double* score,
                         int32_t* n_audio_beats, float* oenv, float* rms, uint8_t* audio_beats, uint8_t* pose_beats, void* stream);
int eg_beat_tracks_scan(const uint8_t* d_cand, const int32_t* lengths, int32_t recordings, const int32_t* d_meta, void* workspace,
                        int64_t workspace_bytes, int32_t* events, int32_t* counts, void* stream);

#define EG_TAKE_CHUNK_FRAMES 16
#define EG_TAKE_MAX_DRAWS 64
int64_t eg_take_meta_ints(int32_t recordings);
int eg_take_meta(const int32_t* frames, int32_t recordings, int32_t* meta);
int eg_track_rows_pack(const float* track, int32_t recordings, int32_t draws, int32_t Tmax, int32_t pose_dim, const int32_t* frames,
                       const int32_t* d_meta, float* rows, void* stream);
int64_t eg_take_distance_workspace_bytes(const int32_t* frames, int32_t recordings, int32_t draws);
int eg_take_distance(const float* feat, int32_t recordings, int32_t draws, int32_t feat_dim, const int32_t* frames, const int32_t* d_meta,
                     int32_t span , void* workspace, int64_t workspace_bytes, double* distance, double* diversity,
                     void* stream);


int eg_conv3x3(const float* x, const float* w, const float* bias, const float* scale, const float* shift,
               float* y, float* gap_partial, int32_t batch, int32_t h, int32_t wdt, int32_t cin, int32_t cout,
               int32_t stride, int32_t relu, int32_t nchw_out, int32_t precision, void* stream);
int32_t eg_conv3x3_gap_tiles(int32_t h, int32_t wdt, int32_t cin, int32_t cout, int32_t stride);
int32_t eg_conv3x3_channel_split(int32_t batch, int32_t h, int32_t wdt, int32_t cin, int32_t cout, int32_t stride, int32_t precision);
int eg_conv3x3_se(const float* x, const float* w_packed, const float* bias, const float* scale, const float* shift, const float* gate,
                  const float* residual, float* y, float* gap_partial, int32_t batch, int32_t h, int32_t wdt, int32_t cin, int32_t cout,
                  int32_t stride, int32_t relu, int32_t nchw_out, int32_t precision, void* stream);
int eg_conv3x3_res_masked(const float* x, const float* w_packed, const float* residual, const uint32_t* res_bits, float* y, int32_t batch, int32_t h,
                          int32_t wdt, int32_t cin, int32_t cout, int32_t precision, void* stream);
int eg_conv3x3_sq(const float* x, const float* w_packed, const float* bias, float* y, float* gap_partial, float* gap_sq_partial, int32_t batch,
                  int32_t h, int32_t wdt, int32_t cin, int32_t cout, int32_t stride, int32_t relu, int32_t precision, void* stream);
int eg_conv3x3_sq_in_affine(const float* x, const float* in_scale, const float* in_shift, const float* w_packed, const float* bias, float* y,
                            float* gap_partial, float* gap_sq_partial, int32_t batch, int32_t h, int32_t wdt, int32_t cin, int32_t cout, int32_t stride,
                            int32_t relu, int32_t precision, void* stream);
int eg_se_gate_pre(const float* t1, const float* gap_partial, int32_t tiles, const float* conv2_w_packed, const float* scale2,
                   const float* shift2, const float* w1, const float* b1, const float* w2, const float* b2, float* gate,
                   int32_t batch, int32_t h, int32_t wdt, int32_t c, void* stream);
int eg_se_block_fused(const float* x, const float* conv1_w, const float* scale1, const float* shift1, const float* conv2_w, const float* scale2,
                      const float* shift2, const float* se_w1, const float* se_b1, const float* se_w2, const float* se_b2, const float* ds_w,
                      const float* ds_scale, const float* ds_shift, float* t1, float* out, float* gap_partial, float* gate, float* sc_vec,
                      int32_t batch, int32_t h, int32_t wdt, int32_t cin, int32_t cout, int32_t stride, int32_t precision, void* stream);
int64_t eg_conv3x3_packed_floats(int32_t cin, int32_t cout_pad);

int eg_stem_conv(const float* x, const float* w9xc, const float* bias, const float* scale, const float* shift,
                 float* y, int32_t batch, int32_t h, int32_t wdt, int32_t c, void* stream);

int eg_se_gate(const float* gap_partial, int32_t tiles, const float* w1, const float* b1, const float* w2,
               const float* b2, float* gate, int32_t batch, int32_t c, int32_t hw, void* stream);

int eg_se_residual_relu(const float* y, const float* gate, const float* x_in, const float* ds_w,
                        const float* ds_scale, const float* ds_shift, float* out, int32_t batch, int32_t ho,
                        int32_t wo, int32_t c, int32_t h_in, int32_t w_in, int32_t cin, int32_t stride, void* stream);

int eg_linear(const float* x, int32_t lda, const float* w, int32_t ldw, const float* bias,
              const float* res1, const float* res2, int32_t ldr, float* y, int32_t ldc,
              int32_t m, int32_t n, int32_t k, int32_t relu, int32_t a_shift, int32_t a_seq,
              int32_t precision, void* stream);
int eg_split_tiles(const float* x, int32_t lda, int32_t m, int32_t k, void* images, void* stream);
int eg_linear_presplit(const void* x_images, int32_t k_x, const float* w, int32_t ldw, const float* bias,
                       const float* res1, const float* res2, int32_t ldr, float* y, int32_t ldc,
                       int32_t m, int32_t n, int32_t k, int32_t relu, int32_t precision, void* stream);
int eg_linear_presplit_causal(const void* x_images, int32_t k_x, const void* zero_line, const float* w, int32_t ldw, const float* bias,
                              const float* res2, int32_t ldr, float* y, int32_t ldc, void* y_images, int32_t y_k, int32_t m, int32_t n,
                              int32_t k_tap, int32_t relu, int32_t shift, int32_t period, int32_t precision, void* stream);

int eg_linear_splitk(const float* x, int32_t lda, const float* w, int32_t ldw, const float* bias, float* y,
                     int32_t ldc, int32_t m, int32_t n, int32_t k, int32_t relu, int32_t splits,
                     float* partial, int32_t precision, void* stream);

typedef struct EgLinearArgs {
    const float* x; const float* w; const float* bias; const float* res1; const float* res2; float* y;
    const float* gate_src;
    const int32_t* drop_epoch;
    float* partial;
    const void* x_images;
    void* y_images;
    uint64_t drop_offset;
    int32_t lda, ldw, ldr, ldc, ldg;
    int32_t m, n, k, relu, precision, splits;
    int32_t k_x, y_k;
    uint32_t drop_seed;
    float drop_p;
} EgLinearArgs;
int eg_linear_ex(const EgLinearArgs* args, void* stream);

int eg_layernorm(const float* x, const float* gamma, const float* beta, float* y, int32_t rows, int32_t d,
                 float eps, void* stream);
int eg_layernorm_img(const float* x, const float* gamma, const float* beta, float* y, void* y_images, int32_t rows, int32_t d, float eps,
                     void* stream);

int eg_attention(const float* q, int32_t ldq, const float* k, int32_t ldk, const float* v, int32_t ldv,
                 float* out, int32_t ldo, float* attn, int32_t batch, int32_t heads, int32_t lq, int32_t lk,
                 int32_t dk, int32_t precision, void* stream);
int eg_attention_masked(const float* q, int32_t ldq, const float* k, int32_t ldk, const float* v, int32_t ldv, const uint8_t* mask,
                        int64_t mask_batch_stride, int32_t mask_query_stride, float* out, int32_t ldo, float* attn, int32_t batch,
                        int32_t heads, int32_t lq, int32_t lk, int32_t dk, int32_t precision, void* stream);

int64_t eg_mha_workspace_bytes(int32_t batch, int32_t lq, int32_t lk, int32_t d_model, int32_t heads);
int eg_multi_head_attention(const float* xq, const float* xkv, const float* wq, const float* wk, const float* wv,
                            const float* wo, const float* ln_g, const float* ln_b, float* out, float* attn,
                            int32_t batch, int32_t lq, int32_t lk, int32_t d_model, int32_t heads,
                            int32_t precision, void* workspace, int64_t workspace_bytes, void* stream);

int64_t eg_ffn_workspace_bytes(int32_t rows, int32_t d_model, int32_t d_inner);
int eg_positionwise_ffn(const float* x, const float* w1, const float* b1, const float* w2, const float* b2,
                        const float* ln_g, const float* ln_b, float* out, int32_t rows, int32_t d_model,
                        int32_t d_inner, int32_t precision, void* workspace, int64_t workspace_bytes, void* stream);

int eg_tcn_forward(const float* x, const float* w, float* y, int32_t batch, int32_t len, int32_t c,
                   int32_t levels, int32_t precision, void* workspace, int64_t workspace_bytes, void* stream);

int eg_add_rows_split(const float* a, const float* table, float* out, void* images, int64_t rows, int32_t d, int32_t period, void* stream);
int eg_add_rows(const float* a, const float* table, float* out, int64_t rows, int32_t d, int32_t period, void* stream);

int eg_reparameterize(const float* mu, const float* logvar, const float* eps, float* z, int64_t n, void* stream);

int eg_conv1d(const float* x, const float* w, const float* bias, const float* scale, const float* shift, float* y, int32_t n,
              int32_t cin, int32_t cout, int32_t lin, int32_t k, int32_t stride, int32_t pad, int32_t act, void* stream);

int64_t eg_contrastive_workspace_bytes(int32_t n);
int eg_contrastive_loss(const float* face, const float* audio, int32_t n, int32_t d, float* cross, float* loss, float* acc,
                        void* workspace, int64_t workspace_bytes, void* stream);
int64_t eg_contrastive_backward_workspace_bytes(int32_t n);
int eg_contrastive_loss_backward(const float* face, const float* audio, int32_t n, int32_t d, float* gface, float* gaudio, void* workspace,
                                 int64_t workspace_bytes, void* stream);



int eg_transpose(const float* x, int32_t ldx, int32_t rows, int32_t cols, float* y, int32_t ldy, void* stream);
int64_t eg_gemm_tn_workspace_floats(int32_t m, int32_t n, int64_t k);
int eg_gemm_tn(const float* a, int32_t lda, const float* b, int32_t ldb, float* c, int32_t ldc, int32_t m, int32_t n, int64_t k,
               float* workspace, int64_t workspace_floats, int32_t accumulate, void* stream);
int eg_conv3x3_wgrad(const float* x, const float* dy, float* dw_mat, int32_t batch, int32_t h, int32_t w, int32_t cin, int32_t cout,
                     int32_t stride, float* workspace, int64_t workspace_floats, void* stream);
int eg_im2col3x3(const float* x, float* col, int32_t batch, int32_t h, int32_t w, int32_t c, int32_t stride, int32_t backward, void* stream);
int eg_subsample(const float* x, float* y, int32_t batch, int32_t h, int32_t w, int32_t c, int32_t stride, int32_t backward, void* stream);
int eg_conv1d_cl_forward(const float* x, const float* w, const float* bias, float* y, int32_t batch, int32_t len, int32_t cin, int32_t len_out,
                         int32_t cout, int32_t k, int32_t stride, int32_t pad, int32_t dilation, void* stream);
int eg_conv1d_cl_backward_input(const float* dy, const float* w, const float* bias, float* dx, int32_t batch, int32_t len, int32_t cin,
                                int32_t len_out, int32_t cout, int32_t k, int32_t stride, int32_t pad, int32_t dilation, void* stream);
int64_t eg_conv1d_cl_backward_weight_workspace_floats(int32_t batch, int32_t cin, int32_t len_out, int32_t cout, int32_t k, int32_t stride,
                                                      int32_t dilation);
int eg_conv1d_cl_backward_weight(const float* x, const float* dy, float* dw, float* db_dy, float* db_x, int32_t batch, int32_t len, int32_t cin,
                                 int32_t len_out, int32_t cout, int32_t k, int32_t stride, int32_t pad, int32_t dilation, float* workspace,
                                 int64_t workspace_floats, void* stream);
int eg_pad_cols(const float* x, float* y, int64_t rows, int32_t k, int32_t k_padded, void* stream);
int64_t eg_colreduce_workspace_floats(int32_t c);
// ... 93 lines not shown
```

Before: 26930 clips/s.

## Group independent presplit GEMMs into single grouped-kernel launches

Adds a grouped variant of the presplit GEMM kernels that packs up to four independent linear layers into one launch, with each workgroup picking its member from a start-offset table. The grouping is applied at several sites: the audio fc2 together with the prior h2 tail, the emo2/sem2 heads, and the decoder KV projections, which are hoisted out of the layer loop. The aim is fewer kernel launches and better CU fill for small-M GEMMs at batch 64. The cost is a larger kernel argument struct, some per-block branching, and an extra KV workspace buffer. Profiling is extended so grouped launches split their time across members.

```diff
diff --git a/emotiongestures_amd/_lib.py b/emotiongestures_amd/_lib.py
--- a/emotiongestures_amd/_lib.py
+++ b/emotiongestures_amd/_lib.py
@@ -44,6 +44,11 @@
                [("drop_offset", C.c_uint64)] + \
                [(n, _I) for n in ("lda", "ldw", "ldr", "ldc", "ldg", "m", "n", "k", "relu", "precision", "splits", "k_x", "y_k")] + \
                [("drop_seed", C.c_uint32), ("drop_p", C.c_float)]
+
+
+class EgLinearGroupMember(C.Structure):
+    _fields_ = [(n, _P) for n in ("x_images", "w", "bias", "res1", "y", "y_images", "partial")] + \
+               [(n, _I) for n in ("k_x", "k0", "ldw", "ldr", "ldc", "y_k", "m", "n", "k", "relu", "splits", "shared_chip")]
 
 
 class EgResamplePlan(C.Structure):
@@ -141,6 +146,7 @@
     "eg_linear": (C.c_int, [_P, _I, _P, _I, _P, _P, _P, _I, _P, _I, _I, _I, _I, _I, _I, _I, _I, _P]),
     "eg_split_tiles": (C.c_int, [_P, _I, _I, _I, _P, _P]),
     "eg_linear_presplit": (C.c_int, [_P, _I, _P, _I, _P, _P, _P, _I, _P, _I, _I, _I, _I, _I, _I, _P]),
+    "eg_linear_presplit_group": (C.c_int, [C.POINTER(EgLinearGroupMember), _I, _I, _I, _P]),
     "eg_linear_presplit_causal": (C.c_int, [_P, _I, _P, _P, _I, _P, _P, _I, _P, _I, _P, _I, _I, _I, _I, _I, _I, _I, _I, _P]),
     "eg_linear_splitk": (C.c_int, [_P, _I, _P, _I, _P, _P, _I, _I, _I, _I, _I, _I, _P, _I, _P]),
     "eg_layernorm": (C.c_int, [_P, _P, _P, _P, _I, _I, C.c_float, _P]),
diff --git a/emotiongestures_amd/csrc/common.h b/emotiongestures_amd/csrc/common.h
--- a/emotiongestures_amd/csrc/common.h
+++ b/emotiongestures_amd/csrc/common.h
@@ -147,6 +147,7 @@
     hipStream_t st;
     EgProfScope(int64_t tag, double flops, hipStream_t s);
     void workgroups(int n);
+    void share(int64_t tag, double flops, int workgroups);
     ~EgProfScope();
 };
 
@@ -171,3 +172,5 @@
     int xs_shift = 0, xs_period = 1; const void* xzero = nullptr;
     int splits = 0; float* partial = nullptr;
 };
+int egi_linear(const EgiLinear& p, hipStream_t st);
+int egi_linear_group(const EgiLinear* p, int n, hipStream_t st);
diff --git a/emotiongestures_amd/csrc/gemm.hip b/emotiongestures_amd/csrc/gemm.hip
--- a/emotiongestures_amd/csrc/gemm.hip
+++ b/emotiongestures_amd/csrc/gemm.hip
@@ -422,9 +422,46 @@
     return eg_check_launch("gemm_glds");
 }
 
-
-template <int TERMS, bool TRAIN = false, bool SHIFT = false>
-__global__ __launch_bounds__(256, 2) void gemm_presplit_kernel(GemmArgs a, const bf8* __restrict__ xhi, const bf8* __restrict__ xlo, int xKO) {
+constexpr int GROUP_MAX = 4;
+struct GroupMember {
+    GemmArgs a;
+    const bf8 *xhi, *xlo;
+    int xKO, m_tiles, n_tiles;
+    int gx, gy, start;
+};
+struct GroupArgs { GroupMember m[GROUP_MAX]; int n; };
+
+__device__ __forceinline__ void xcd_tile_sub(int lin, int gx, int gy, int& bx, int& by) {
+    const int total = gx * gy;
+    const int xcd = lin & 7, idx = lin >> 3;
+    const int q = total >> 3, r = total & 7;
+    const int log = xcd * q + (xcd < r ? xcd : r) + idx;
+    bx = log / gy;
+    by = log - bx * gy;
+}
+__device__ __forceinline__ int group_member_of(const GroupArgs& g) {
+    int i = 0;
+#pragma unroll
+    for (int j = 1; j < GROUP_MAX; ++j)
+        if (j < g.n && (int)blockIdx.x >= g.m[j].start) i = j;
+    return i;
+}
+template <bool GROUP> struct PresplitOperand { typedef GemmArgs type; };
+template <> struct PresplitOperand<true> { typedef GroupArgs type; };
+
+
+template <int TERMS, bool TRAIN = false, bool SHIFT = false, bool GROUP = false>
+__global__ __launch_bounds__(256, 2) void gemm_presplit_kernel(typename PresplitOperand<GROUP>::type ga, const bf8* __restrict__ xhi, const bf8* __restrict__ xlo, int xKO) {
+    int glin = 0, ggx = 0, ggy = 0;
+    const GemmArgs* ap;
+    if constexpr (GROUP) {
+        const GroupMember& mb = ga.m[group_member_of(ga)];
+        glin = (int)blockIdx.x - mb.start; ggx = mb.gx; ggy = mb.gy;
+        if (glin >= ggx * ggy) return;
+        xhi = mb.xhi; xlo = mb.xlo; xKO = mb.xKO;
+        ap = &mb.a;
+    } else ap = &ga;
+    const GemmArgs& a = *ap;
     constexpr int BK = 32;
     constexpr int RING = 4;
     constexpr int WM = 2;
@@ -436,7 +473,7 @@
     const int tid = threadIdx.x, lane = tid & 63, li = lane & 15, kq = lane >> 4;
     const int wave = __builtin_amdgcn_readfirstlane(tid >> 6);
     int bx, by;
-    xcd_tile(bx, by);
+    if constexpr (GROUP) xcd_tile_sub(glin, ggx, ggy, bx, by); else xcd_tile(bx, by);
     const int m0 = bx * 64, n0 = by * 64;
     const int wm = (wave >> 1) * 32, wn = (wave & 1) * 32;
     const int kbeg = blockIdx.z * a.k_per_split;
@@ -573,9 +610,19 @@
     return eg_check_launch("gemm_presplit");
 }
 
-template <int TERMS, bool TRAIN = false, bool SHIFT = false>
-__global__ __launch_bounds__(512, 1) void gemm_presplit128_kernel(GemmArgs a, const bf8* __restrict__ xhi, const bf8* __restrict__ xlo, int xKO,
+template <int TERMS, bool TRAIN = false, bool SHIFT = false, bool GROUP = false>
+__global__ __launch_bounds__(512, 1) void gemm_presplit128_kernel(typename PresplitOperand<GROUP>::type ga, const bf8* __restrict__ xhi, const bf8* __restrict__ xlo, int xKO,
                                                                   int m_tiles, int n_tiles) {
+    int glin = 0, ggx = 0, ggy = 0;
+    const GemmArgs* ap;
+    if constexpr (GROUP) {
+        const GroupMember& mb = ga.m[group_member_of(ga)];
+        glin = (int)blockIdx.x - mb.start; ggx = mb.gx; ggy = mb.gy;
+        if (glin >= ggx * ggy) return;
+        xhi = mb.xhi; xlo = mb.xlo; xKO = mb.xKO; m_tiles = mb.m_tiles; n_tiles = mb.n_tiles;
+        ap = &mb.a;
+    } else ap = &ga;
+    const GemmArgs& a = *ap;
     constexpr int RING = 3;
     constexpr int NIMG = (TERMS == 3) ? 2 : 1;
     constexpr int OPI = 8 * 64;
@@ -585,7 +632,7 @@
     const int tid = threadIdx.x, lane = tid & 63, li = lane & 15, kq = lane >> 4;
     const int wave = __builtin_amdgcn_readfirstlane(tid >> 6);
     int bx, by;
-    xcd_tile(bx, by);
+    if constexpr (GROUP) xcd_tile_sub(glin, ggx, ggy, bx, by); else xcd_tile(bx, by);
     const int m0 = bx * 128, n0 = by * 128;
     const int wm = wave >> 2, wn = wave & 3;
     const int nsteps = (a.K + 31) / 32;
@@ -731,6 +778,31 @@
     }
     if (tile == TILE_128) return x3 ? launch_presplit128<3>(a, xhi, xlo, xko, mt, nt, st) : launch_presplit128<1>(a, xhi, xlo, xko, mt, nt, st);
     return x3 ? launch_presplit<3>(a, xhi, xlo, xko, grid, st) : launch_presplit<1>(a, xhi, xlo, xko, grid, st);
+}
+
+template <int TERMS>
+int launch_presplit_group(GroupArgs& g, int tile, hipStream_t st) {
+    constexpr int NIMG = (TERMS == 3) ? 2 : 1;
+    int total = 0;
+    for (int i = 0; i < g.n; ++i) {
+        GroupMember& m = g.m[i];
+        m.gx = tile == TILE_128 ? eg_cdiv(m.m_tiles, 2) : m.m_tiles;
+        m.gy = tile == TILE_128 ? eg_cdiv(m.n_tiles, 2) : m.n_tiles;
+        m.start = (int)eg_round_up(total, 8);
+        total = m.start + m.gx * m.gy;
+    }
+    if (tile == TILE_128) {
+        constexpr size_t LDS_BYTES = (size_t)3 * 2 * NIMG * 8 * 64 * 16;
+        auto kern = gemm_presplit128_kernel<TERMS, false, false, true>;
+        if (int rc = eg_ensure_dynamic_lds(reinterpret_cast<const void*>(kern), LDS_BYTES, "gemm_presplit128_group")) return rc;
+        hipLaunchKernelGGL(kern, dim3(total), dim3(512), LDS_BYTES, st, g, (const bf8*)nullptr, (const bf8*)nullptr, 0, 0, 0);
+        return eg_check_launch("gemm_presplit128_group");
+    }
+    constexpr size_t LDS_BYTES = (size_t)4 * 2 * NIMG * 4 * 64 * 16;
+    auto kern = gemm_presplit_kernel<TERMS, false, false, true>;
+    if (int rc = eg_ensure_dynamic_lds(reinterpret_cast<const void*>(kern), LDS_BYTES, "gemm_presplit_group")) return rc;
+    hipLaunchKernelGGL(kern, dim3(total), dim3(256), LDS_BYTES, st, g, (const bf8*)nullptr, (const bf8*)nullptr, 0);
+    return eg_check_launch("gemm_presplit_group");
 }
 
 template <int RT, bool XF32, bool TRAIN>
@@ -899,8 +971,8 @@
 
 }
 
-int egi_linear(const EgiLinear& p, hipStream_t st) {
-    GemmArgs a;
+namespace {
+int egi_fill(const EgiLinear& p, GemmArgs& a) {
     EG_REQUIRE((p.x || p.ximg) && p.w && (p.y || p.yimg) && p.m > 0 && p.n > 0 && p.k > 0, EG_ERR_BAD_ARG, "egi_linear: null pointer or empty shape");
     EG_REQUIRE((p.k & 3) == 0 && (p.ldw & 3) == 0, EG_ERR_ALIGN, "egi_linear: K, ldw %% 4");
     a.x = p.x; a.w = p.w; a.lda = p.lda; a.ldw = p.ldw; a.M = p.m; a.N = p.n; a.K = p.k;
@@ -917,6 +989,12 @@
         EG_REQUIRE((p.n & 3) == 0 && (p.yK & 63) == 0 && (p.yk0 & 7) == 0, EG_ERR_ALIGN, "egi_linear: image output alignment");
         a.yimg = reinterpret_cast<unsigned short*>(p.yimg); a.yKO = p.yK >> 3; a.yoct0 = p.yk0 >> 3;
     }
+    return EG_OK;
+}
+}
+int egi_linear(const EgiLinear& p, hipStream_t st) {
+    GemmArgs a;
+    if (int rc = egi_fill(p, a)) return rc;
     EgProfScope prof(p.precision == EG_PREC_F32 ? 5 : ((p.ximg) ? 3 : (p.a_shift ? 4 : 2)), 2.0 * p.m * (double)p.n * p.k, st);
     if (p.ximg && p.precision != EG_PREC_F32) {
         EG_REQUIRE((p.xK & 63) == 0 && (p.xk0 & 31) == 0 && (p.k & 31) == 0, EG_ERR_ALIGN, "egi_linear: pre-split X needs K %% 32 == 0");
@@ -954,6 +1032,52 @@
     }
     prof.workgroups(eg_cdiv(p.m, 64) * eg_cdiv(p.n, 64));
     return launch_gemm(a, 1, p.precision, st);
+}
+
+namespace {
+bool group_products_on() {
+    const char* e = getenv("EG_GROUP_PRODUCTS");
+    return !(e && e[0] && strtol(e, nullptr, 0) == 0);
+}
+}
+int egi_linear_group(const EgiLinear* p, int n, hipStream_t st) {
+    EG_REQUIRE(p && n >= 1 && n <= GROUP_MAX, EG_ERR_BAD_ARG, "egi_linear_group: %d members (1..%d)", n, GROUP_MAX);
+    bool group = n >= 2 && group_products_on();
+    int tile = presplit_tile_override();
+    if (tile == TILE_BAD) group = false;
+    const bool auto_tile = tile == TILE_AUTO;
+    for (int i = 0; group && i < n; ++i) {
+        const EgiLinear& q = p[i];
+        const bool plain = q.ximg && q.w && (q.y || q.yimg) && q.precision != EG_PREC_F32 && q.precision == p[0].precision && q.m > 64 && q.n > 0 &&
+                           q.k > 0 && q.xs_shift == 0 && q.splits <= 1 && (q.ldw & 63) == 0 && (q.xK & 63) == 0 && (q.xk0 & 31) == 0 && (q.k & 31) == 0;
+        if (!plain) { group = false; break; }
+        const int t = auto_tile ? presplit_tile_default(q.m, q.n, q.shared_chip) : tile;
+        if (i == 0) tile = t;
+        else if (t != tile) group = false;
+    }
+    if (!group) {
+        for (int i = 0; i < n; ++i)
+            if (int rc = egi_linear(p[i], st)) return rc;
+        return EG_OK;
+    }
+    GroupArgs g;
+    g.n = n;
+    for (int i = 0; i < n; ++i) {
+        GroupMember& m = g.m[i];
+        if (int rc = egi_fill(p[i], m.a)) return rc;
+        m.xKO = p[i].xK >> 3; m.m_tiles = eg_cdiv(p[i].m, 64); m.n_tiles = eg_cdiv(p[i].n, 64);
+        m.xhi = reinterpret_cast<const bf8*>(p[i].ximg);
+        m.xlo = m.xhi + (size_t)m.m_tiles * m.xKO * 64;
+        m.a.xoct0 = p[i].xk0 >> 3;
+    }
+    for (int i = n; i < GROUP_MAX; ++i) g.m[i] = g.m[0];
+    EgProfScope prof(3, 2.0 * p[0].m * (double)p[0].n * p[0].k, st);
+    for (int i = 0; i < n; ++i) {
+        const int wgs = tile == TILE_128 ? eg_cdiv(g.m[i].m_tiles, 2) * eg_cdiv(g.m[i].n_tiles, 2) : g.m[i].m_tiles * g.m[i].n_tiles;
+        if (i == 0) prof.workgroups(wgs);
+        else prof.share(3, 2.0 * p[i].m * (double)p[i].n * p[i].k, wgs);
+    }
+    return p[0].precision == EG_PREC_BF16X3 ? launch_presplit_group<3>(g, tile, st) : launch_presplit_group<1>(g, tile, st);
 }
 int egi_split_tiles(const float* x, int lda, int m, int k, void* images, hipStream_t st) { return eg_split_tiles(x, lda, m, k, images, st); }
 
@@ -1071,3 +1195,21 @@
     p.xs_shift = shift; p.xs_period = period; p.xzero = zero_line;
     return egi_linear(p, (hipStream_t)stream);
 }
+
+extern "C" int eg_linear_presplit_group(const EgLinearGroupMember* members, int32_t n, int32_t precision, int32_t grouped, void* stream) {
+    EG_REQUIRE(members && n >= 1 && n <= GROUP_MAX, EG_ERR_BAD_ARG, "eg_linear_presplit_group: %d members (1..%d)", n, GROUP_MAX);
+    EG_REQUIRE(precision == EG_PREC_BF16X3 || precision == EG_PREC_BF16, EG_ERR_BAD_ARG, "eg_linear_presplit_group: bf16 modes only");
+    EgiLinear p[GROUP_MAX];
+    for (int i = 0; i < n; ++i) {
+        const EgLinearGroupMember& m = members[i];
+        EG_REQUIRE(m.x_images && m.w && (m.y || m.y_images), EG_ERR_BAD_ARG, "eg_linear_presplit_group: member %d: null pointer", i);
+        p[i].ximg = m.x_images; p[i].xK = m.k_x; p[i].xk0 = m.k0; p[i].w = m.w; p[i].ldw = m.ldw; p[i].bias = m.bias;
+        p[i].res1 = m.res1; p[i].ldr = m.ldr; p[i].y = m.y; p[i].ldc = m.ldc; p[i].yimg = m.y_images; p[i].yK = m.y_k;
+        p[i].m = m.m; p[i].n = m.n; p[i].k = m.k; p[i].relu = m.relu; p[i].precision = precision; p[i].shared_chip = m.shared_chip;
+        p[i].splits = m.splits; p[i].partial = m.partial;
+    }
+    if (grouped) return egi_linear_group(p, n, (hipStream_t)stream);
+    for (int i = 0; i < n; ++i)
+        if (int rc = egi_linear(p[i], (hipStream_t)stream)) return rc;
+    return EG_OK;
+}
diff --git a/emotiongestures_amd/csrc/generator.hip b/emotiongestures_amd/csrc/generator.hip
--- a/emotiongestures_amd/csrc/generator.hip
+++ b/emotiongestures_amd/csrc/generator.hip
@@ -66,7 +66,7 @@
 }
 
 namespace {
-struct ProfRec { hipEvent_t a, b; int64_t tag; double flops; bool ok; int wgs; };
+struct ProfRec { hipEvent_t a, b; int64_t tag; double flops; bool ok; int wgs; int head, parts; };
 std::vector<ProfRec> g_prof;
 int g_prof_n = 0;
 bool g_prof_on = false;
@@ -77,10 +77,17 @@
     g_prof[slot].tag = tag;
     g_prof[slot].flops = flops;
     g_prof[slot].wgs = 0;
+    g_prof[slot].head = -1; g_prof[slot].parts = 1;
     g_prof[slot].ok = hipEventRecord(g_prof[slot].a, st) == hipSuccess;
 }
 void EgProfScope::workgroups(int n) {
     if (slot >= 0) g_prof[slot].wgs = n;
+}
+void EgProfScope::share(int64_t tag, double flops, int workgroups) {
+    if (slot < 0 || g_prof_n >= (int)g_prof.size()) return;
+    ProfRec& r = g_prof[g_prof_n++];
+    r.tag = tag; r.flops = flops; r.wgs = workgroups; r.head = slot; r.parts = 1; r.ok = true;
+    ++g_prof[slot].parts;
 }
 EgProfScope::~EgProfScope() {
     if (slot >= 0 && hipEventRecord(g_prof[slot].b, st) != hipSuccess) g_prof[slot].ok = false;
@@ -90,7 +97,7 @@
     while ((int)g_prof.size() < max_records) {
         ProfRec r;
         if (hipEventCreate(&r.a) != hipSuccess || hipEventCreate(&r.b) != hipSuccess) { eg_set_error("hipEventCreate failed"); return EG_ERR_HIP; }
-        r.tag = 0; r.flops = 0; r.ok = false; r.wgs = 0;
+        r.tag = 0; r.flops = 0; r.ok = false; r.wgs = 0; r.head = -1; r.parts = 1;
         g_prof.push_back(r);
     }
     g_prof_n = 0;
@@ -107,12 +114,13 @@
     int n = g_prof_n < capacity ? g_prof_n : capacity;
     for (int i = 0; i < n; ++i) {
         float t = 0.f;
-        if (!g_prof[i].ok || hipEventSynchronize(g_prof[i].b) != hipSuccess || hipEventElapsedTime(&t, g_prof[i].a, g_prof[i].b) != hipSuccess) {
+        const ProfRec& h = g_prof[i].head >= 0 ? g_prof[g_prof[i].head] : g_prof[i];
+        if (!g_prof[i].ok || !h.ok || hipEventSynchronize(h.b) != hipSuccess || hipEventElapsedTime(&t, h.a, h.b) != hipSuccess) {
             eg_set_error("eg_profile_read: event %d was not recorded / cannot be read", i);
             g_prof_n = 0;
             return EG_ERR_HIP;
         }
-        tags[i] = g_prof[i].tag; flops[i] = g_prof[i].flops; ms[i] = t;
+        tags[i] = g_prof[i].tag; flops[i] = g_prof[i].flops; ms[i] = t / (float)h.parts;
     }
     g_prof_n = 0;
     return n;
@@ -128,7 +136,6 @@
 int egi_add_img(const float* a, const float* b, float* out, void* img, size_t n, int row_len, int period, hipStream_t st);
 int egi_time_linear(const float* x, const float* w, const float* bias, float* y, int batch, int L, int C, int ld, hipStream_t st);
 int egi_copy2d(const float* src, int lds_, float* dst, int ldd, int rows, int cols, hipStream_t st);
-int egi_linear(const EgiLinear& p, hipStream_t st);
 int egi_layernorm(const float* x, const float* gamma, const float* beta, float* y, void* img, int rows, int d, float eps, hipStream_t st);
 int egi_attention(const float* q, int ldq, const float* k, int ldk, const float* v, int ldv, float* out, int ldo, float* attn,
                   void* oimg, int batch, int heads, int lq, int lk, int dk, int precision, hipStream_t st);
@@ -314,6 +321,7 @@
 struct GenWs {
     int64_t act[3], gap, gate, scv, amap, afc1, afeat, emo_t, emo, sem_t, sem, cls_part, cls_h[3], cls_out;
     int64_t fus_in, fus_h, fusion, xa, xb, q, qkv, ao, proj, ffn_h, im_x[2], im_enc, im_h, im_a[3], im_p[2];
+    int64_t dkv;
     int64_t prior_cat, prior_h, prior_enc, prior_rep, tm_mem, tm_pe, tm_gram, post_a, post_b, post_c, pose;
     int64_t t_emb, t_a, t_b, t_c, t_out, im_t[3], t_zero;
     int64_t tap_stem, tap_l[3];
@@ -353,6 +361,7 @@
     w.xa = cv.take(NF * D); w.xb = cv.take(NF * D);
     w.q = cv.take(NF * D); w.qkv = cv.take(NF * D * 3); w.ao = cv.take(NF * D); w.proj = cv.take(NF * D);
     w.ffn_h = cv.take(NF * c.d_inner);
+    w.dkv = NB == B ? cv.take((int64_t)c.n_layers * NF * D * 2) : -1;
     {
         const int64_t N64 = eg_round_up(NF, 64), B64 = eg_round_up(BF, 64), KX = D > g->Dpad ? D : g->Dpad;
         w.im_x[0] = cv.take(N64 * KX); w.im_x[1] = cv.take(N64 * KX); w.im_enc = cv.take(N64 * D); w.im_h = cv.take(N64 * c.d_inner);
@@ -396,8 +405,8 @@
 struct Act { float* f = nullptr; int ld = 0; void* img = nullptr; int kimg = 0; };
 inline Act act(float* f, int ld, void* img = nullptr, int kimg = 0) { Act a; a.f = f; a.ld = ld; a.img = img; a.kimg = kimg; return a; }
 
-int lin(const EgGenerator* g, const float* arena, const LinW& w, const Act& x, int xk0, const Act& y, bool want_f32, int m, int relu,
-        const float* res1, int ldr, hipStream_t st, int n_override = 0, int splits = 0, float* partial = nullptr) {
+EgiLinear lin_desc(const EgGenerator* g, const float* arena, const LinW& w, const Act& x, int xk0, const Act& y, bool want_f32, int m, int relu,
+                   const float* res1, int ldr, int n_override = 0, int splits = 0, float* partial = nullptr) {
     const bool img_ok = g->cfg.precision != EG_PREC_F32;
     EgiLinear p;
     p.w = arena + w.w; p.ldw = w.kpad; p.bias = w.b >= 0 ? arena + w.b : nullptr;
@@ -412,7 +421,18 @@
     if (yimg) { p.yimg = y.img; p.yK = y.kimg; }
     if (want_f32 || !yimg) { p.y = y.f; p.ldc = y.ld; }
     if (splits > 1 && img_ok && x.img && !yimg) { p.splits = splits; p.partial = partial; }
-    return egi_linear(p, st);
+    return p;
+}
+int lin(const EgGenerator* g, const float* arena, const LinW& w, const Act& x, int xk0, const Act& y, bool want_f32, int m, int relu,
+        const float* res1, int ldr, hipStream_t st, int n_override = 0, int splits = 0, float* partial = nullptr) {
+    return egi_linear(lin_desc(g, arena, w, x, xk0, y, want_f32, m, relu, res1, ldr, n_override, splits, partial), st);
+}
+
+enum GroupSite { GROUP_HEADS = 1, GROUP_DEC_KV = 2, GROUP_TAILS = 4 };
+bool group_site(const EgGenerator* g, int site, int rows) {
+    if (g->cfg.precision == EG_PREC_F32 || rows <= 64) return false;
+    const char* e = getenv("EG_GROUP_PRODUCTS");
+    return !(e && e[0]) || (strtol(e, nullptr, 0) & site) != 0;
 }
 
 int run_mha(const EgGenerator* g, const float* arena, const MhaW& m, const Act& xq, const Act& xkv, const Act& out, const GenWs& w,
@@ -433,12 +453,24 @@
     return egi_layernorm(pr, arena + m.ln_g, arena + m.ln_b, out.f, g->cfg.precision != EG_PREC_F32 ? out.img : nullptr, B * Lq, D, 1e-6f, st);
 }
 
+int run_dec_kv(const EgGenerator* g, const float* arena, const Act& enc_out, float* const* kv, const Act* prior_enc, float* q0, int rows,
+               hipStream_t st) {
+    const int D = g->cfg.d_model, L = g->cfg.n_layers;
+    EgiLinear p[9];
+    int n = 0;
+    for (int l = 0; l < L && l < 8; ++l) p[n++] = lin_desc(g, arena, g->dec_attn[l].kv, enc_out, 0, act(kv[l], 2 * D), true, rows, 0, nullptr, 0);
+    if (prior_enc) p[n++] = lin_desc(g, arena, g->dec_attn[0].q, *prior_enc, 0, act(q0, D), true, rows, 0, nullptr, 0);
+    const bool group = group_site(g, GROUP_DEC_KV, rows);
+    for (int i = 0; i < n; i += group ? 4 : 1) EG_TRY(egi_linear_group(p + i, group ? (n - i < 4 ? n - i : 4) : 1, st));
+    return EG_OK;
+}
+
 int run_mha_kv(const EgGenerator* g, const float* arena, const MhaW& m, const Act& xq, const float* kv, const Act& out, const GenWs& w,
-               void* ws, int B, int Lq, int Lk, hipStream_t st) {
+               void* ws, int B, int Lq, int Lk, hipStream_t st, bool have_q = false) {
     const int D = g->cfg.d_model;
     float *q = P(ws, w.q), *ao = P(ws, w.ao), *pr = P(ws, w.proj);
     void* aimg = g->cfg.precision != EG_PREC_F32 ? P(ws, w.im_h) : nullptr;
-    EG_TRY(lin(g, arena, m.q, xq, 0, act(q, D), true, B * Lq, 0, nullptr, 0, st));
+    if (!have_q) EG_TRY(lin(g, arena, m.q, xq, 0, act(q, D), true, B * Lq, 0, nullptr, 0, st));
     EG_TRY(egi_attention(q, D, kv, 2 * D, kv + D, 2 * D, ao, D, nullptr, aimg, B, g->cfg.n_head, Lq, Lk, g->cfg.d_k, g->cfg.precision, st));
     EG_TRY(lin(g, arena, m.o, act(ao, D, aimg, D), 0, act(pr, D), true, B * Lq, 0, xq.f, D, st));
     return egi_layernorm(pr, arena + m.ln_g, arena + m.ln_b, out.f, g->cfg.precision != EG_PREC_F32 ? out.img : nullptr, B * Lq, D, 1e-6f, st);
@@ -456,7 +488,15 @@
 }
 
 
-int run_audio_tower(const EgGenerator* g, const float* arena, const float* spec, const GenWs& w, void* ws, int B, hipStream_t st) {
+bool group_tails(const EgGenerator* g, int rows) { return !g->concurrent && !g->fold && group_site(g, GROUP_TAILS, rows); }
+EgiLinear prior_h2_desc(const EgGenerator* g, const float* arena, const GenWs& w, void* ws, int rows) {
+    const int D = g->cfg.d_model;
+    return lin_desc(g, arena, g->prior_h2, act(P(ws, w.prior_h), D, P(ws, w.im_p[0]), D), 0, act(P(ws, w.prior_enc), D, P(ws, w.im_p[1]), D), true, rows, 0,
+                    nullptr, 0);
+}
+
+int run_audio_tower(const EgGenerator* g, const float* arena, const float* spec, const GenWs& w, void* ws, int B, hipStream_t st,
+                    bool with_prior_h2 = false) {
     const int prec = g->cfg.precision, F = g->cfg.frames, D = g->cfg.d_model;
     float* bufs[3] = {P(ws, w.act[0]), P(ws, w.act[1]), P(ws, w.act[2])};
     float *gap = P(ws, w.gap), *gate = P(ws, w.gate);
@@ -495,7 +535,9 @@
     if (g->fold) return lin(g, arena, g->f_audio, act(amap, g->HW3), 0, act(P(ws, w.afeat), D, P(ws, w.im_a[1]), D), true, B * F, 0, nullptr, 0, st);
     const Act h1 = act(P(ws, w.afc1), D, P(ws, w.im_a[0]), D);
     EG_TRY(lin(g, arena, g->a_fc1, act(amap, g->HW3), 0, h1, false, B * F, 0, nullptr, 0, st));
-    return lin(g, arena, g->a_fc2, h1, 0, act(P(ws, w.afeat), D, P(ws, w.im_a[1]), D), true, B * F, 0, nullptr, 0, st);
+    const EgiLinear p[2] = {lin_desc(g, arena, g->a_fc2, h1, 0, act(P(ws, w.afeat), D, P(ws, w.im_a[1]), D), true, B * F, 0, nullptr, 0),
+                            prior_h2_desc(g, arena, w, ws, B * F)};
+    return egi_linear_group(p, with_prior_h2 ? 2 : 1, st);
 }
 
 int causal_conv(const EgGenerator* g, const float* arena, const EgGenerator::TcnConv& cv, void* ximg, const void* zero, float* y, void* yimg,
@@ -548,7 +590,7 @@
                      0, 0, prec, st);
 }
 
-int run_prior(const EgGenerator* g, const float* arena, const float* prior, const GenWs& w, void* ws, int B, hipStream_t st) {
+int run_prior(const EgGenerator* g, const float* arena, const float* prior, const GenWs& w, void* ws, int B, hipStream_t st, bool defer_h2 = false) {
     const EgGeneratorConfig& c = g->cfg;
     EgiPriorW pw;
     memset(&pw, 0, sizeof(pw));
@@ -567,7 +609,8 @@
                    nullptr, 0, st);
     const Act ph = act(P(ws, w.prior_h), c.d_model, P(ws, w.im_p[0]), c.d_model);
     EG_TRY(lin(g, arena, g->prior_h0, act(P(ws, w.prior_cat), g->Dpad), 0, ph, false, rows, 0, nullptr, 0, st));
-    return lin(g, arena, g->prior_h2, ph, 0, act(P(ws, w.prior_enc), c.d_model, P(ws, w.im_p[1]), c.d_model), true, rows, 0, nullptr, 0, st);
+    if (defer_h2) return EG_OK;
+    return egi_linear(prior_h2_desc(g, arena, w, ws, rows), st);
 }
 
 bool add_images(const EgGenerator* g) {
@@ -622,10 +665,17 @@
     void *im0 = P(ws, w.im_x[0]), *im1 = P(ws, w.im_x[1]);
     float *xb = P(ws, w.xb), *da = P(ws, w.fus_h);
     Act dx = prior_enc;
+    float* own[8];
+    const bool hoist = !kv && w.dkv >= 0 && c.n_layers <= 8 && group_site(g, GROUP_DEC_KV, rows);
+    if (hoist) {
+        for (int l = 0; l < c.n_layers; ++l) own[l] = P(ws, w.dkv) + (size_t)l * rows * 2 * D;
+        EG_TRY(run_dec_kv(g, arena, enc_out, own, &prior_enc, P(ws, w.q), rows, st));
+        kv = own;
+    }
     for (int l = 0; l < c.n_layers; ++l) {
         const Act mid = act(xb, D, im0, D);
         const Act nxt = act(da, D, im1, D);
-        if (kv) EG_TRY(run_mha_kv(g, arena, g->dec_attn[l], dx, kv[l], mid, w, ws, NB, F, F, st));
+        if (kv) EG_TRY(run_mha_kv(g, arena, g->dec_attn[l], dx, kv[l], mid, w, ws, NB, F, F, st, hoist && l == 0));
         else EG_TRY(run_mha(g, arena, g->dec_attn[l], dx, enc_out, mid, w, ws, NB, F, F, st));
         EG_TRY(run_ffn(g, arena, g->dec_ffn[l], mid, nxt, w, ws, rows, st));
         dx = nxt;
@@ -649,8 +699,10 @@
         EG_TRY(lin(g, arena, g->f_sem, afeat, 0, act(sem, D), true, rows, 0, nullptr, 0, st));
     } else {
         EG_TRY(lin(g, arena, g->emosem0, afeat, 0, es, false, rows, 0, nullptr, 0, st));
-        EG_TRY(lin(g, arena, g->emo2, es, 0, act(emo, D), true, rows, 0, nullptr, 0, st));
-        EG_TRY(lin(g, arena, g->sem2, es, D, act(sem, D), true, rows, 0, nullptr, 0, st));
+        const EgiLinear p[2] = {lin_desc(g, arena, g->emo2, es, 0, act(emo, D), true, rows, 0, nullptr, 0),
+                                lin_desc(g, arena, g->sem2, es, D, act(sem, D), true, rows, 0, nullptr, 0)};
+        if (group_site(g, GROUP_HEADS, rows)) EG_TRY(egi_linear_group(p, 2, st));
+        else { EG_TRY(egi_linear(p[0], st)); EG_TRY(egi_linear(p[1], st)); }
     }
     const int K0 = F * D;
     EG_TRY(eg_linear_splitk(emo, K0, arena + g->cls[0].w, g->cls[0].kpad, arena + g->cls[0].b, P(ws, w.cls_h[0]), D, B, D, K0, 1,
@@ -856,12 +908,13 @@
         EG_HIP_TRY(hipStreamWaitEvent(s_prior, g->ev_fork, 0), "branch fork");
     }
     EG_TRY(run_text(g, arena, text, txt, w, ws, B, s_text));
-    EG_TRY(run_prior(g, arena, prior, w, ws, B, s_prior));
+    const bool tails = group_tails(g, rows);
+    EG_TRY(run_prior(g, arena, prior, w, ws, B, s_prior, tails));
     if (g->concurrent) {
         EG_HIP_TRY(hipEventRecord(g->ev_join[0], s_text), "branch join");
         EG_HIP_TRY(hipEventRecord(g->ev_join[1], s_prior), "branch join");
     }
-    EG_TRY(run_audio_tower(g, arena, spec, w, ws, B, st));
+    EG_TRY(run_audio_tower(g, arena, spec, w, ws, B, st, tails));
     float* emo = emotion_feature ? emotion_feature : P(ws, w.emo);
     float* sem = semantic_feature ? semantic_feature : P(ws, w.sem);
     EG_TRY(run_heads(g, arena, emo, sem, emotion_prediction ? emotion_prediction : P(ws, w.cls_out), w, ws, B, st));
@@ -890,8 +943,13 @@
     hipStream_t st = (hipStream_t)stream;
     const EgGeneratorConfig& c = g->cfg;
     const int F = c.frames, D = c.d_model, rows = B * F, prec = c.precision;
-    EG_TRY(run_audio_tower(g, arena, spec, w, ws, B, st));
-    EG_TRY(run_prior(g, arena, prior, w, ws, B, st));
+    if (group_tails(g, rows)) {
+        EG_TRY(run_prior(g, arena, prior, w, ws, B, st, true));
+        EG_TRY(run_audio_tower(g, arena, spec, w, ws, B, st, true));
+    } else {
+        EG_TRY(run_audio_tower(g, arena, spec, w, ws, B, st));
+        EG_TRY(run_prior(g, arena, prior, w, ws, B, st));
+    }
     const Act afeat = act(P(ws, w.afeat), D, P(ws, w.im_a[1]), D), es = act(P(ws, w.emo_t), 2 * D, P(ws, w.im_a[2]), 2 * D);
     if (g->fold) {
         EG_TRY(lin(g, arena, g->f_sem, afeat, 0, act(P(ws, w.sem), D), true, rows, 0, nullptr, 0, st));
@@ -931,7 +989,8 @@
         w.im_p[0] = cv.take(B64 * D); w.im_p[1] = cv.take(B64 * D);
         w.tm_mem = cv.take(UR * c.pose_dim); w.tm_pe = cv.take(UR * c.chunk + 16);
     }
-    for (int l = 0; l < c.n_layers; ++l) r.kv[l] = cv.take(N * R * c.frames * 2 * D);
+    for (int l = 0; l < c.n_layers; ++l)
+        r.kv[l] = w.dkv >= 0 ? w.dkv + (int64_t)l * N * c.frames * 2 * D * (int64_t)sizeof(float) : cv.take(N * R * c.frames * 2 * D);
     r.prior[0] = cv.take(UR * c.prior_frames * c.pose_dim);
     r.prior[1] = cv.take(UR * c.prior_frames * c.pose_dim);
     r.spec = cv.take(N * c.n_mels * c.spec_len);
@@ -979,10 +1038,8 @@
     } else EG_TRY(egi_draws_fusion(sampled, sem, fus_in.f, p.U, p.steps, p.R, (size_t)F * D, st));
     Act enc_out;
     EG_TRY(run_encoder(g, arena, fus_in, enc_out, w, ws, NR, st));
-    for (int l = 0; l < c.n_layers; ++l) {
-        kv[l] = P(ws, r.kv[l]);
-        EG_TRY(lin(g, arena, g->dec_attn[l].kv, enc_out, 0, act(kv[l], 2 * D), true, NR * F, 0, nullptr, 0, st));
-    }
+    for (int l = 0; l < c.n_layers; ++l) kv[l] = P(ws, r.kv[l]);
+    EG_TRY(run_dec_kv(g, arena, enc_out, kv, nullptr, nullptr, NR * F, st));
     if (move) {
         if (text_embedding) EG_TRY(roll_rows(p, txt, text_embedding, (size_t)c.text_len * 512, true, st));
         if (emotion_feature) EG_TRY(roll_rows(p, emo, emotion_feature, (size_t)F * D, true, st));
@@ -1207,8 +1264,9 @@
     const int F = c.frames, D = c.d_model, rows = U * F;
     float* prior = P(state, s.prior);
     if (text) EG_TRY(run_text(g, arena, text, P(ws, w.t_out), w, ws, U, st));
-    EG_TRY(run_prior(g, arena, prior, w, ws, U, st));
-    EG_TRY(run_audio_tower(g, arena, spec, w, ws, U, st));
+    const bool tails = !g->fold && group_site(g, GROUP_TAILS, U * c.frames);
+    EG_TRY(run_prior(g, arena, prior, w, ws, U, st, tails));
+    EG_TRY(run_audio_tower(g, arena, spec, w, ws, U, st, tails));
     EG_TRY(run_heads(g, arena, P(ws, w.emo), P(ws, w.sem), emotion_prediction ? emotion_prediction : P(ws, w.cls_out), w, ws, U, st));
     const Act fus_in = fusion_act(g, w, ws);
     EG_TRY(egi_add_img(sampled ? sampled : P(ws, w.emo), P(ws, w.sem), fus_in.f, fus_in.img, (size_t)rows * D, D, 0, st));
diff --git a/include/emogest.h b/include/emogest.h
--- a/include/emogest.h
+++ b/include/emogest.h
@@ -300,6 +300,16 @@
 int eg_linear_presplit_causal(const void* x_images, int32_t k_x, const void* zero_line, const float* w, int32_t ldw, const float* bias,
                               const float* res2, int32_t ldr, float* y, int32_t ldc, void* y_images, int32_t y_k, int32_t m, int32_t n,
                               int32_t k_tap, int32_t relu, int32_t shift, int32_t period, int32_t precision, void* stream);
+typedef struct EgLinearGroupMember {
+    const void* x_images;
+    const float* w; const float* bias; const float* res1;
+    float* y;
+    void* y_images;
+    float* partial;
+    int32_t k_x, k0, ldw, ldr, ldc, y_k;
+    int32_t m, n, k, relu, splits, shared_chip;
+} EgLinearGroupMember;
+int eg_linear_presplit_group(const EgLinearGroupMember* members, int32_t n, int32_t precision, int32_t grouped, void* stream);
 
 int eg_linear_splitk(const float* x, int32_t lda, const float* w, int32_t ldw, const float* bias, float* y,
                      int32_t ldc, int32_t m, int32_t n, int32_t k, int32_t relu, int32_t splits,
```

Result: no change. 27120 clips/s, median of 6 (+0.7%).
